# peekxc/primate

Measured on AMD Instinct MI355X. Metric: probe-matvecs/sec, higher is better.
Workload: dtype f64

## Files before the change

include/slq.h:

```cpp
#ifndef SLQ_H
#define SLQ_H

#include <stddef.h>
#include <stdint.h>

#ifdef __cplusplus
extern "C" {
#endif

#define SLQ_VERSION 100

enum {
  SLQ_OK = 0,
  SLQ_EINVAL = -1,
  SLQ_ENOMEM = -2,
  SLQ_EHIP = -3,
  SLQ_ENODEV = -4,
  SLQ_ECALLBACK = -5,
  SLQ_ENOTCONV = -6
};

enum { SLQ_F32 = 0, SLQ_F64 = 1 };

enum {
// ... 20 lines not shown
typedef struct slq_diag slq_diag;
typedef struct slq_dmat slq_dmat;
typedef struct slq_density slq_density;
typedef struct slq_sddmm slq_sddmm;

typedef int (*slq_matvec_fn)(void *user, const void *x, void *y);
typedef int (*slq_matmat_device_fn)(void *user, const void *d_X, void *d_Y, int64_t n, int ncols, void *stream);

const char *slq_last_error(void);
int slq_version(void);
int slq_device_count(int *count);
int slq_context_create(int device, void *hip_stream, slq_context **out);
int slq_context_destroy(slq_context *ctx);
int slq_context_synchronize(slq_context *ctx);
int slq_context_meminfo(slq_context *ctx, size_t *free_bytes, size_t *total_bytes);
int slq_context_device(slq_context *ctx, int *device);

int slq_csr_create(slq_context *ctx, int dtype, int64_t n, int64_t nnz, const int32_t *rowptr,
                   const int32_t *colind, const void *vals, slq_operator **out);
int slq_csr_create_device(slq_context *ctx, int dtype, int64_t n, int64_t nnz,
                          const int32_t *d_rowptr, const int32_t *d_colind, const void *d_vals,
                          slq_operator **out);
int slq_csr_gram_create(slq_context *ctx, int dtype, int64_t mrows, int64_t ncols, int64_t nnz, const int32_t *rowptr,
                        const int32_t *colind, const void *vals, slq_operator **out);
int slq_csr_affine_create(slq_context *ctx, int dtype, int64_t n, int64_t nnz_a, const int32_t *rowptr_a, const int32_t *colind_a,
                          const void *vals_a, int64_t nnz_b, const int32_t *rowptr_b, const int32_t *colind_b, const void *vals_b,
                          slq_operator **out);
int slq_operator_set_parameter(slq_operator *op, double t);
enum { SLQ_KERNEL_RBF = 0, SLQ_KERNEL_MATERN12 = 1, SLQ_KERNEL_MATERN32 = 2, SLQ_KERNEL_MATERN52 = 3 };
int slq_kernel_create(slq_context *ctx, int dtype, int64_t n, int d, const void *points, int64_t ldp, int profile,
                      const double *lengthscales, int nls, double outputscale, double noise, slq_operator **out);
int slq_kernel_create_device(slq_context *ctx, int dtype, int64_t n, int d, const void *d_points, int64_t ldp, int profile,
                             const double *lengthscales, int nls, double outputscale, double noise, slq_operator **out);
int slq_kernel_set_parameters(slq_operator *op, const double *lengthscales, int nls, double outputscale, double noise);
int slq_kernel_get_parameters(const slq_operator *op, int *d, int *profile, double *lengthscales, int nls, double *outputscale, double *noise);
int slq_debug_kernel_points(slq_operator *op, void *zt, void *nrm, void *params);
int slq_debug_kernel_schedule(int64_t n, int panel_width, int panels, int num_cus, int64_t *out, int nout);
int slq_debug_operator_device_bytes(int64_t *live);
int slq_dense_create(slq_context *ctx, int dtype, int64_t n, const void *A, int64_t lda,
                     slq_operator **out);
int slq_device_callback_create(slq_context *ctx, int dtype, int64_t n, slq_matmat_device_fn fn, void *user,
                               slq_operator **out);
int slq_callback_create(slq_context *ctx, int dtype, int64_t n, slq_matvec_fn fn, void *user,
                        slq_operator **out);
int slq_operator_destroy(slq_operator *op);
int slq_operator_shape(const slq_operator *op, int64_t *nrows, int64_t *ncols, int64_t *nnz,
                       int *dtype);
int slq_operator_matmat(slq_operator *op, const void *X, int64_t ldx, void *Y, int64_t ldy,
                        int b);

int slq_plan_create(slq_context *ctx, slq_operator *op, int nprobes, int deg, int orth,
                    int keep_basis, slq_plan **out);
int slq_plan_create_recompute(slq_context *ctx, slq_operator *op, int nprobes, int deg, int orth, slq_plan **out);
int slq_plan_basis_mode(const slq_plan *plan, int *mode, int *ring_slots, int *acc_cols);
int slq_plan_action_columns(slq_plan *plan, uint64_t *read, uint64_t *offered, int reset);
int slq_plan_destroy(slq_plan *plan);
int slq_plan_workspace_bytes(const slq_plan *plan, size_t *bytes);
int slq_plan_query_bytes(int dtype, int64_t n, int nprobes, int deg, int orth, int keep_basis,
                         size_t *bytes);
int slq_plan_query_bytes_recompute(int dtype, int64_t n, int nprobes, int deg, int orth, size_t *bytes);
typedef struct {
  int panel_width;
  int panels;
  int ring_slots;
  int sequence;
  int pipelined;
  int reordered;
  int upper_alpha;
  double far_per_row;
  int tiles;
  int fused_alpha;
} slq_plan_info;
int slq_plan_describe(const slq_plan *plan, slq_plan_info *out);

int slq_plan_set_probes(slq_plan *plan, const void *X, int64_t ldx);
int slq_plan_set_probes_device(slq_plan *plan, const void *d_X, int64_t ldx);
int slq_plan_generate_probes(slq_plan *plan, int pdf, uint64_t seed, uint64_t probe_offset);
int slq_plan_get_probes(slq_plan *plan, void *X, int64_t ldx);

int slq_plan_run(slq_plan *plan, double rtol);
int slq_plan_run_steps(slq_plan *plan, double rtol, int upto);
int slq_plan_steps_done(const slq_plan *plan, int *cur);
int slq_plan_get_tridiag(slq_plan *plan, void *alpha, void *beta, int32_t *steps);
int slq_plan_quadrature(slq_plan *plan, int fun_id, const double *fun_params, double *quad,
                        double *nodes, double *weights);
int slq_plan_quadrature_at(slq_plan *plan, int m, int rule, double endpoint, int fun_id, const double *fun_params,
                           double *quad, double *nodes, double *weights, double *stage);
int slq_plan_get_basis(slq_plan *plan, int probe, void *Q, int64_t ldq);
int slq_plan_fun_action(slq_plan *plan, int fun_id, const double *fun_params, void *Y,
                        int64_t ldy);

int slq_quadrature_batch(slq_context *ctx, int nb, int deg, const double *d, const double *e,
                         int fun_id, const double *fun_params, double *quad, double *nodes,
                         double *weights);

int slq_quadrature_radau_batch(slq_context *ctx, int nb, int m, const double *d, const double *e, const double *beta_m,
                               double endpoint, int fun_id, const double *fun_params, double *quad, double *nodes,
                               double *weights);

int slq_eigh_tridiag_batch(slq_context *ctx, int nb, int deg, const double *d, const double *e, double *w, double *Z);

int slq_dmat_create(slq_context *ctx, int64_t n, int cols, slq_dmat **out);
int slq_dmat_destroy(slq_dmat *m);
int slq_dmat_set(slq_dmat *m, int c0, int nc, const double *host, int64_t ld);
int slq_dmat_get(slq_dmat *m, int c0, int nc, double *host, int64_t ld);
int slq_dmat_ptr(slq_dmat *m, int c0, void **dptr);
int slq_dmat_generate(slq_dmat *m, int c0, int nc, int pdf, uint64_t seed, uint64_t probe_offset);
int slq_dmat_copy(slq_dmat *dst, int d0, slq_dmat *src, int s0, int nc);
int slq_dmat_copy_rows(slq_dmat *dst, int d0, int64_t dr0, slq_dmat *src, int s0, int64_t sr0, int64_t nrows, int nc);
int slq_dmat_gemm_tn(slq_dmat *A, int a0, int ma, slq_dmat *B, int b0, int mb, double *C_host);
int slq_dmat_gemm_nn(slq_dmat *OUT, int o0, slq_dmat *A, int a0, int ma, const double *C_host, int mb,
                     double alpha, double beta);
int slq_plan_fun_action_dmat(slq_plan *plan, int fun_id, const double *fun_params, slq_dmat *OUT, int o0);
int slq_plan_get_probes_dmat(slq_plan *plan, slq_dmat *OUT, int o0);

int slq_measure_stream(slq_context *ctx, int mode, size_t bytes_per_stream, int reps, double *gbps);

int slq_fttr_batch(slq_context *ctx, int nb, int n, int k, const double *theta, const double *alpha,
                   const double *beta, double *weights);

int slq_diag_create(slq_context *ctx, int64_t n, slq_diag **out);
int slq_diag_destroy(slq_diag *d);
int slq_diag_update(slq_diag *d, slq_plan *plan, int fun_id, const double *fun_params);
int slq_diag_get(slq_diag *d, double *numer, double *denom, double *running_mean, int64_t *count);

int slq_density_create(slq_context *ctx, int kind, int ngrid, const double *grid, double bw, slq_density **out);
int slq_density_update(slq_density *d, slq_plan *plan);
int slq_density_get(slq_density *d, double *mean, double *m2, double *outside, int64_t *count);
int slq_density_destroy(slq_density *d);

int slq_plan_create_chebyshev(slq_context *ctx, slq_operator *op, int nprobes, int nsteps, slq_plan **out);
int slq_plan_run_chebyshev(slq_plan *plan, double center, double halfwidth, double outside_tol);
int slq_plan_get_moments(slq_plan *plan, double *mu, int *outside);
int slq_plan_moment_sum(slq_plan *plan, int ncoef, const double *coef, double *quad, double *stage);
int slq_density_update_moments(slq_density *d, slq_plan *plan, int nweights, const double *damp);

int slq_plan_create_chebyshev_action(slq_context *ctx, slq_operator *op, int nprobes, int nsteps, slq_plan **out);
int slq_plan_chebyshev_action(slq_plan *plan, double center, double halfwidth, double outside_tol, int ncoef, const double *coef,
                              void *Y, int64_t ldy);
int slq_plan_chebyshev_action_dmat(slq_plan *plan, double center, double halfwidth, double outside_tol, int ncoef, const double *coef,
                                   slq_dmat *OUT, int o0);

int slq_sddmm_create(slq_context *ctx, int64_t n, int64_t nnz, const int32_t *rowptr, const int32_t *colind, slq_sddmm **out);
int slq_sddmm_create_device(slq_context *ctx, int64_t n, int64_t nnz, const int32_t *d_rowptr, const int32_t *d_colind, slq_sddmm **out);
int slq_sddmm_update(slq_sddmm *s, slq_dmat *W, int w0, slq_dmat *Z, int z0, int m, double alpha, double beta, int symmetric);
int slq_sddmm_get(slq_sddmm *s, double *vals, int64_t *count);
int slq_sddmm_ptr(slq_sddmm *s, void **d_vals);
int slq_sddmm_reset(slq_sddmm *s);
int slq_sddmm_destroy(slq_sddmm *s);
int slq_debug_sddmm_schedule(int64_t n, const int32_t *rowptr, int32_t *row0, int32_t *nrows, int32_t *kind, int64_t *e0, int64_t *e1,
                             int64_t cap, int64_t *nitems, int64_t *info);

typedef struct slq_kernel_grad slq_kernel_grad;
int slq_kernel_grad_create(slq_context *ctx, slq_operator *op, slq_kernel_grad **out);
int slq_kernel_grad_update(slq_kernel_grad *g, slq_dmat *Z, int z0, slq_dmat *W, int w0, int m, double alpha, double beta);
int slq_kernel_grad_get(slq_kernel_grad *g, double *vals, int nvals, int64_t *count);
int slq_kernel_grad_reset(slq_kernel_grad *g);
int slq_kernel_grad_destroy(slq_kernel_grad *g);
int slq_debug_kernel_grad_schedule(int64_t n, int m, int num_cus, int64_t *out, int nout);

typedef struct slq_kernel_cross slq_kernel_cross;
int slq_kernel_cross_create(slq_context *ctx, slq_operator *op, int64_t m, const void *points, int64_t ldp, slq_kernel_cross **out);
int slq_kernel_cross_create_device(slq_context *ctx, slq_operator *op, int64_t m, const void *d_points, int64_t ldp, slq_kernel_cross **out);
int slq_kernel_cross_matmat(slq_kernel_cross *cross, int trans, const void *X, int64_t ldx, void *Y, int64_t ldy, int b);
int slq_kernel_cross_dmat(slq_kernel_cross *cross, int trans, slq_dmat *IN, int i0, slq_dmat *OUT, int o0, int b);
int slq_kernel_cross_destroy(slq_kernel_cross *cross);
int slq_debug_kernel_cross_points(slq_kernel_cross *cross, void *zt, void *nrm);
int slq_debug_kernel_cross_schedule(int64_t nrows, int64_t nsum, int64_t b, int num_cus, int64_t *out, int nout);

typedef struct slq_kernel_feature slq_kernel_feature;
int slq_kernel_feature_create(slq_context *ctx, slq_operator *op, int64_t F2, const void *omega, int64_t ld, slq_kernel_feature **out);
int slq_kernel_feature_matmat(slq_kernel_feature *feat, slq_kernel_cross *cross, const void *W, int64_t ldw, void *Y, int64_t ldy, int b);
int slq_kernel_feature_dmat(slq_kernel_feature *feat, slq_kernel_cross *cross, slq_dmat *IN, int i0, slq_dmat *OUT, int o0, int b);
int slq_kernel_feature_destroy(slq_kernel_feature *feat);
int slq_debug_kernel_feature_frequencies(slq_kernel_feature *feat, void *omega_t);
int slq_debug_kernel_feature_schedule(int64_t nrows, int64_t F2, int64_t b, int num_cus, int is_f64, int64_t *out, int nout);
int slq_kernel_feature_rmatmat(slq_kernel_feature *feat, slq_kernel_cross *cross, const void *U, int64_t ldu, void *Z, int64_t ldz, int b);
int slq_kernel_feature_rdmat(slq_kernel_feature *feat, slq_kernel_cross *cross, slq_dmat *IN, int i0, slq_dmat *OUT, int o0, int b);
int slq_debug_kernel_feature_adjoint_schedule(int64_t F2, int64_t nrows, int64_t b, int num_cus, int is_f64, int64_t *out, int nout);

int slq_kernel_precond_create(slq_context *ctx, slq_operator *kernel_op, int rank_max, double tol, slq_operator **out);
int slq_kernel_precond_refresh(slq_operator *pre);
int slq_kernel_precond_info(const slq_operator *pre, int *rank_max, int *rank, double *logdet_p, double *residual_trace, double *t_max);
int slq_kernel_precond_get(slq_operator *pre, int32_t *pivots, double *L, int64_t ldl, double *G, double *eig);
int slq_kernel_precond_apply(slq_operator *pre, const void *X, int64_t ldx, void *Y, int64_t ldy, int b);
int slq_kernel_precond_apply_dmat(slq_operator *pre, slq_dmat *IN, int i0, slq_dmat *OUT, int o0, int b);
int slq_debug_kernel_precond_addresses(const slq_operator *pre, uint64_t *out4);
int slq_debug_kernel_precond_h(slq_operator *pre, double *H);
int slq_kernel_precond_columns(slq_operator *pre, int which, int c0, int nc, slq_dmat *OUT, int o0);
int slq_kernel_precond_trace_grad(slq_operator *pre, slq_kernel_grad *grad, double alpha, double beta);
int slq_debug_kernel_precond_timing(const slq_operator *pre, double *out2);

typedef struct slq_kernel_pointgrad slq_kernel_pointgrad;
int slq_kernel_pointgrad_create(slq_context *ctx, slq_operator *op, slq_kernel_pointgrad **out);
int slq_kernel_pointgrad_create_cross(slq_context *ctx, slq_kernel_cross *cross, slq_kernel_pointgrad **out);
int slq_kernel_pointgrad_update(slq_kernel_pointgrad *g, slq_dmat *Z_or_U, int c0, slq_dmat *W, int w0, int m, double alpha, double beta);
int slq_kernel_pointgrad_get(slq_kernel_pointgrad *g, double *vals, int64_t ld, int64_t *count);
int slq_kernel_pointgrad_reset(slq_kernel_pointgrad *g);
int slq_kernel_pointgrad_destroy(slq_kernel_pointgrad *g);
int slq_kernel_precond_trace_pointgrad(slq_operator *pre, slq_kernel_pointgrad *grad, double alpha, double beta);
int slq_debug_kernel_pointgrad_schedule(int64_t nrows, int64_t nsum, int num_cus, int64_t *out, int nout);

enum {
  SLQ_K_SPMM = 0,
  SLQ_K_AXPY_NORM,
  SLQ_K_REORTH_DOT,
  SLQ_K_REORTH_UPD,
  SLQ_K_FINALIZE,
  SLQ_K_PROBES,
  SLQ_K_QUADRATURE,
  SLQ_K_COMBINE,
  SLQ_K_COUNT
};
typedef struct {
  double ms[SLQ_K_COUNT];
  int64_t launches[SLQ_K_COUNT];
} slq_profile;
int slq_plan_profile_enable(slq_plan *plan, int enable);
int slq_plan_sweep_columns(slq_plan *plan, uint64_t *read, uint64_t *offered, int reset);
int slq_plan_window_columns(slq_plan *plan, int64_t out[5], int reset);
int slq_plan_dense_path(slq_plan *plan, int *kernel, int *ksplit);
int slq_plan_window_verify(slq_plan *plan, int *mode, double out[5]);
int slq_plan_window_census(slq_plan *plan, int32_t *out, int64_t len);
int slq_plan_window_flags(slq_plan *plan, int32_t *read, int32_t *rescue, int64_t len);
int slq_plan_profile_read(slq_plan *plan, slq_profile *out, int reset);

int slq_debug_ring_flag_status(int flag);
int slq_debug_plan_poke_ring_flag(slq_plan *plan, int value);
int slq_debug_plan_mark_stale(slq_plan *plan, int nstale);
int slq_debug_step_shape(const int *facts, int nfacts, int j, int prev_xt, int *out, int nout);
int slq_debug_cheb_step_shape(const int *facts, int nfacts, int j, int *out, int nout);
int slq_debug_cheb_action_schedule(int nsteps, int *t0, int *nc, int cap, int *npieces, int *ring_slots, int *acc_cols);
int slq_debug_csr_layout(int64_t n, int64_t nnz, const int32_t *rowptr, const int32_t *colind, int plain, int32_t *perm_out,
                         int32_t *tile_row_out, int64_t ntile_cap, int32_t *xcd_tile_out, double *info_out);
int slq_debug_plan_shape(const double *facts, int nfacts, double *out, int nout);
int slq_debug_plan_shape_of(const slq_plan *plan, double *facts_out, int nfacts, double *shape_out, int nout);

int slq_quad_batch(slq_context *ctx, slq_operator *op, const void *X, int64_t ldx, int pdf,
                   uint64_t seed, uint64_t probe_offset, int nprobes, int deg, double rtol,
                   int orth, int fun_id, const double *fun_params, double *quad_out,
                   double *nodes_out, double *weights_out);

int slq_fAv_batch(slq_context *ctx, slq_operator *op, const void *X, int64_t ldx, int nvec, int deg,
                  double rtol, int orth, int fun_id, const double *fun_params, void *Y, int64_t ldy);
int slq_fAv_batch_mode(slq_context *ctx, slq_operator *op, const void *X, int64_t ldx, int nvec, int deg, double rtol, int orth,
                       int fun_id, const double *fun_params, int basis_mode, void *Y, int64_t ldy, int *basis_used);

int slq_lanczos_f64(slq_context *ctx, slq_operator *op, double *v, int deg, double rtol, int orth,
                    double *alpha, double *beta, double *Q, size_t ncv);
int slq_lanczos_f32(slq_context *ctx, slq_operator *op, float *v, int deg, float rtol, int orth,
                    float *alpha, float *beta, float *Q, size_t ncv);

#ifdef __cplusplus
}
#endif
#endif
```

primate_amd/_capi.py:

```python

from __future__ import annotations

import ctypes as C
import os
from pathlib import Path

import numpy as np

_HERE = Path(__file__).resolve().parent
LIB_PATH = Path(os.environ["PRIMATE_AMD_LIBSLQ"]) if os.environ.get("PRIMATE_AMD_LIBSLQ") else _HERE / "_libslq.so"

SLQ_OK, SLQ_EINVAL, SLQ_ENOMEM, SLQ_EHIP, SLQ_ENODEV, SLQ_ECALLBACK, SLQ_ENOTCONV = 0, -1, -2, -3, -4, -5, -6
SLQ_F32, SLQ_F64 = 0, 1
FUN_NONE = -1
FUN_IDS = {
	"identity": 0, "abs": 1, "sqrt": 2, "log": 3, "inv": 4, "exp": 5, "smoothstep": 6, "step": 7, "numrank": 7,
	"softsign": 8,
}
PDF_IDS = {"rademacher": 0, "signs": 0, "normal": 1, "gaussian": 1, "sphere": 2}
DENSITY_KINDS = {"gaussian": 0, "lorentzian": 1, "histogram": 2, "cdf": 3, "chebyshev": 4}
KERNEL_PROFILES = {"rbf": 0, "matern12": 1, "matern32": 2, "matern52": 3}
OP_KERNEL_PRECOND = 6
KERNEL_CLASSES = ["spmm_3term", "axpy_norm", "reorth_dot", "reorth_update", "finalize", "probes", "quadrature", "fun_combine"]

# ... 74 lines not shown
	"slq_device_callback_create": (C.c_int, [_P, C.c_int, C.c_int64, _P, _P, _P]),
	"slq_dmat_generate": (C.c_int, [_P, C.c_int, C.c_int, C.c_int, C.c_uint64, C.c_uint64]),
	"slq_dmat_copy": (C.c_int, [_P, C.c_int, _P, C.c_int, C.c_int]),
	"slq_dmat_copy_rows": (C.c_int, [_P, C.c_int, C.c_int64, _P, C.c_int, C.c_int64, C.c_int64, C.c_int]),
	"slq_measure_stream": (C.c_int, [_P, C.c_int, C.c_size_t, C.c_int, C.POINTER(C.c_double)]),
	"slq_plan_set_probes_device": (C.c_int, [_P, _P, C.c_int64]),
	"slq_fttr_batch": (C.c_int, [_P, C.c_int, C.c_int, C.c_int, _P, _P, _P, _P]),
	"slq_diag_create": (C.c_int, [_P, C.c_int64, _PP]),
	"slq_diag_destroy": (C.c_int, [_P]),
	"slq_diag_update": (C.c_int, [_P, _P, C.c_int, _P]),
	"slq_diag_get": (C.c_int, [_P, _P, _P, _P, C.POINTER(C.c_int64)]),
	"slq_density_create": (C.c_int, [_P, C.c_int, C.c_int, _P, C.c_double, _PP]),
	"slq_density_destroy": (C.c_int, [_P]),
	"slq_density_update": (C.c_int, [_P, _P]),
	"slq_density_get": (C.c_int, [_P, _P, _P, _P, C.POINTER(C.c_int64)]),
	"slq_sddmm_create": (C.c_int, [_P, C.c_int64, C.c_int64, _P, _P, _PP]),
	"slq_sddmm_create_device": (C.c_int, [_P, C.c_int64, C.c_int64, _P, _P, _PP]),
	"slq_sddmm_update": (C.c_int, [_P, _P, C.c_int, _P, C.c_int, C.c_int, C.c_double, C.c_double, C.c_int]),
	"slq_sddmm_get": (C.c_int, [_P, _P, C.POINTER(C.c_int64)]),
	"slq_sddmm_ptr": (C.c_int, [_P, _PP]),
	"slq_sddmm_reset": (C.c_int, [_P]),
	"slq_sddmm_destroy": (C.c_int, [_P]),
	"slq_debug_sddmm_schedule": (C.c_int, [C.c_int64, _P, _P, _P, _P, _P, _P, C.c_int64, C.POINTER(C.c_int64), _P]),
	"slq_kernel_grad_create": (C.c_int, [_P, _P, _PP]),
	"slq_kernel_grad_update": (C.c_int, [_P, _P, C.c_int, _P, C.c_int, C.c_int, C.c_double, C.c_double]),
	"slq_kernel_grad_get": (C.c_int, [_P, _P, C.c_int, C.POINTER(C.c_int64)]),
	"slq_kernel_grad_reset": (C.c_int, [_P]),
	"slq_kernel_grad_destroy": (C.c_int, [_P]),
	"slq_debug_kernel_grad_schedule": (C.c_int, [C.c_int64, C.c_int, C.c_int, C.POINTER(C.c_int64), C.c_int]),
	"slq_kernel_cross_create": (C.c_int, [_P, _P, C.c_int64, _P, C.c_int64, _PP]),
	"slq_kernel_cross_create_device": (C.c_int, [_P, _P, C.c_int64, _P, C.c_int64, _PP]),
	"slq_kernel_cross_matmat": (C.c_int, [_P, C.c_int, _P, C.c_int64, _P, C.c_int64, C.c_int]),
	"slq_kernel_cross_dmat": (C.c_int, [_P, C.c_int, _P, C.c_int, _P, C.c_int, C.c_int]),
	"slq_kernel_cross_destroy": (C.c_int, [_P]),
	"slq_debug_kernel_cross_points": (C.c_int, [_P, _P, _P]),
	"slq_debug_kernel_cross_schedule": (C.c_int, [C.c_int64, C.c_int64, C.c_int64, C.c_int, C.POINTER(C.c_int64), C.c_int]),
	"slq_kernel_feature_create": (C.c_int, [_P, _P, C.c_int64, _P, C.c_int64, _PP]),
	"slq_kernel_feature_matmat": (C.c_int, [_P, _P, _P, C.c_int64, _P, C.c_int64, C.c_int]),
	"slq_kernel_feature_dmat": (C.c_int, [_P, _P, _P, C.c_int, _P, C.c_int, C.c_int]),
	"slq_kernel_feature_destroy": (C.c_int, [_P]),
	"slq_debug_kernel_feature_frequencies": (C.c_int, [_P, _P]),
	"slq_debug_kernel_feature_schedule": (C.c_int, [C.c_int64, C.c_int64, C.c_int64, C.c_int, C.c_int, C.POINTER(C.c_int64), C.c_int]),
	"slq_kernel_feature_rmatmat": (C.c_int, [_P, _P, _P, C.c_int64, _P, C.c_int64, C.c_int]),
	"slq_kernel_feature_rdmat": (C.c_int, [_P, _P, _P, C.c_int, _P, C.c_int, C.c_int]),
	"slq_debug_kernel_feature_adjoint_schedule": (C.c_int, [C.c_int64, C.c_int64, C.c_int64, C.c_int, C.c_int, C.POINTER(C.c_int64), C.c_int]),
	"slq_kernel_precond_create": (C.c_int, [_P, _P, C.c_int, C.c_double, _PP]),
	"slq_kernel_precond_refresh": (C.c_int, [_P]),
	"slq_kernel_precond_info": (C.c_int, [_P, C.POINTER(C.c_int), C.POINTER(C.c_int), C.POINTER(C.c_double), C.POINTER(C.c_double), C.POINTER(C.c_double)]),
	"slq_kernel_precond_get": (C.c_int, [_P, _P, _P, C.c_int64, _P, _P]),
	"slq_kernel_precond_apply": (C.c_int, [_P, _P, C.c_int64, _P, C.c_int64, C.c_int]),
	"slq_kernel_precond_apply_dmat": (C.c_int, [_P, _P, C.c_int, _P, C.c_int, C.c_int]),
	"slq_debug_kernel_precond_addresses": (C.c_int, [_P, C.POINTER(C.c_uint64)]),
	"slq_debug_kernel_precond_timing": (C.c_int, [_P, C.POINTER(C.c_double)]),
	"slq_debug_kernel_precond_h": (C.c_int, [_P, _P]),
	"slq_kernel_precond_columns": (C.c_int, [_P, C.c_int, C.c_int, C.c_int, _P, C.c_int]),
	"slq_kernel_precond_trace_grad": (C.c_int, [_P, _P, C.c_double, C.c_double]),
	"slq_kernel_pointgrad_create": (C.c_int, [_P, _P, _PP]),
	"slq_kernel_pointgrad_create_cross": (C.c_int, [_P, _P, _PP]),
	"slq_kernel_pointgrad_update": (C.c_int, [_P, _P, C.c_int, _P, C.c_int, C.c_int, C.c_double, C.c_double]),
	"slq_kernel_pointgrad_get": (C.c_int, [_P, _P, C.c_int64, C.POINTER(C.c_int64)]),
	"slq_kernel_pointgrad_reset": (C.c_int, [_P]),
	"slq_kernel_pointgrad_destroy": (C.c_int, [_P]),
	"slq_kernel_precond_trace_pointgrad": (C.c_int, [_P, _P, C.c_double, C.c_double]),
	"slq_debug_kernel_pointgrad_schedule": (C.c_int, [C.c_int64, C.c_int64, C.c_int, C.POINTER(C.c_int64), C.c_int]),
	"slq_plan_profile_enable": (C.c_int, [_P, C.c_int]),
	"slq_plan_action_columns": (C.c_int, [_P, C.POINTER(C.c_uint64), C.POINTER(C.c_uint64), C.c_int]),
	"slq_plan_sweep_columns": (C.c_int, [_P, C.POINTER(C.c_uint64), C.POINTER(C.c_uint64), C.c_int]),
	"slq_plan_window_columns": (C.c_int, [_P, C.POINTER(C.c_int64), C.c_int]),
	"slq_plan_dense_path": (C.c_int, [_P, C.POINTER(C.c_int), C.POINTER(C.c_int)]),
	"slq_plan_window_verify": (C.c_int, [_P, C.POINTER(C.c_int), C.POINTER(C.c_double)]),
	"slq_plan_window_census": (C.c_int, [_P, C.POINTER(C.c_int32), C.c_int64]),
	"slq_plan_window_flags": (C.c_int, [_P, C.POINTER(C.c_int32), C.POINTER(C.c_int32), C.c_int64]),
	"slq_plan_profile_read": (C.c_int, [_P, C.POINTER(SlqProfile), C.c_int]),
	"slq_quad_batch": (C.c_int, [_P, _P, _P, C.c_int64, C.c_int, C.c_uint64, C.c_uint64, C.c_int, C.c_int, C.c_double, C.c_int, C.c_int, _P, _P, _P, _P]),
	"slq_eigh_tridiag_batch": (C.c_int, [_P, C.c_int, C.c_int, _P, _P, _P, _P]),
	"slq_fAv_batch": (C.c_int, [_P, _P, _P, C.c_int64, C.c_int, C.c_int, C.c_double, C.c_int, C.c_int, _P, _P, C.c_int64]),
	"slq_fAv_batch_mode": (C.c_int, [_P, _P, _P, C.c_int64, C.c_int, C.c_int, C.c_double, C.c_int, C.c_int, _P, C.c_int, _P, C.c_int64, C.POINTER(C.c_int)]),
	"slq_lanczos_f64": (C.c_int, [_P, _P, _P, C.c_int, C.c_double, C.c_int, _P, _P, _P, C.c_size_t]),
	"slq_lanczos_f32": (C.c_int, [_P, _P, _P, C.c_int, C.c_float, C.c_int, _P, _P, _P, C.c_size_t]),
	"slq_debug_ring_flag_status": (C.c_int, [C.c_int]),
	"slq_debug_plan_poke_ring_flag": (C.c_int, [_P, C.c_int]),
	"slq_debug_step_shape": (C.c_int, [C.POINTER(C.c_int), C.c_int, C.c_int, C.c_int, C.POINTER(C.c_int), C.c_int]),
	"slq_debug_cheb_step_shape": (C.c_int, [C.POINTER(C.c_int), C.c_int, C.c_int, C.POINTER(C.c_int), C.c_int]),
	"slq_debug_csr_layout": (C.c_int, [C.c_int64, C.c_int64, _P, _P, C.c_int, _P, _P, C.c_int64, _P, _P]),
	"slq_debug_plan_shape": (C.c_int, [C.POINTER(C.c_double), C.c_int, C.POINTER(C.c_double), C.c_int]),
	"slq_debug_plan_shape_of": (C.c_int, [_P, C.POINTER(C.c_double), C.c_int, C.POINTER(C.c_double), C.c_int]),
	"slq_plan_create_chebyshev": (C.c_int, [_P, _P, C.c_int, C.c_int, _PP]),
	"slq_plan_run_chebyshev": (C.c_int, [_P, C.c_double, C.c_double, C.c_double]),
	"slq_plan_get_moments": (C.c_int, [_P, _P, _P]),
	"slq_plan_moment_sum": (C.c_int, [_P, C.c_int, _P, _P, _P]),
	"slq_density_update_moments": (C.c_int, [_P, _P, C.c_int, _P]),
	"slq_plan_create_chebyshev_action": (C.c_int, [_P, _P, C.c_int, C.c_int, _PP]),
	"slq_plan_chebyshev_action": (C.c_int, [_P, C.c_double, C.c_double, C.c_double, C.c_int, _P, _P, C.c_int64]),
	"slq_plan_chebyshev_action_dmat": (C.c_int, [_P, C.c_double, C.c_double, C.c_double, C.c_int, _P, _P, C.c_int]),
	"slq_debug_cheb_action_schedule": (C.c_int, [C.c_int, C.POINTER(C.c_int), C.POINTER(C.c_int), C.c_int, C.POINTER(C.c_int), C.POINTER(C.c_int), C.POINTER(C.c_int)]),
}
DEVICE_MATMAT_FN = C.CFUNCTYPE(C.c_int, C.c_void_p, C.c_void_p, C.c_void_p, C.c_int64, C.c_int, C.c_void_p)
class PlanInfo(C.Structure):

	_fields_ = [("panel_width", C.c_int), ("panels", C.c_int), ("ring_slots", C.c_int), ("sequence", C.c_int), ("pipelined", C.c_int),
				("reordered", C.c_int), ("upper_alpha", C.c_int), ("far_per_row", C.c_double), ("tiles", C.c_int), ("fused_alpha", C.c_int)]


EXPORTED_SYMBOLS = tuple(_SIGNATURES)


def _preload_hip_runtime() -> None:
	import importlib.util
	import sys

	if "torch" in sys.modules:
		return
	try:
		spec = importlib.util.find_spec("torch")
	except (ImportError, ValueError):
		spec = None
	if spec is None or not spec.origin:
		return
	cand = Path(spec.origin).parent / "lib" / "libamdhip64.so"
	if cand.exists():
		try:
			C.CDLL(str(cand), mode=getattr(os, "RTLD_NOW", 2) | getattr(os, "RTLD_GLOBAL", 0x100))
		except OSError:
			pass


def lib() -> C.CDLL:
	global _lib
	if _lib is None:
		_preload_hip_runtime()
		if not LIB_PATH.exists():
			raise ImportError(
				f"{LIB_PATH} is missing: build it with `python -c 'import __graft_entry__ as g; g.build()'` "
				"(hipcc --offload-arch=gfx950). primate_amd has no CPU fallback."
			)
		L = C.CDLL(str(LIB_PATH), mode=getattr(os, "RTLD_NOW", 2))
		for name, (res, args) in _SIGNATURES.items():
			fn = getattr(L, name)
			fn.restype, fn.argtypes = res, args
		_lib = L
	return _lib


def check(rc: int) -> int:
	if rc < 0:
		msg = lib().slq_last_error().decode(errors="replace")
		if rc == SLQ_EINVAL:
			raise ValueError(msg)
		if rc == SLQ_ENOMEM:
			raise MemoryError(msg)
		raise SlqError(rc, msg)
	return rc


def ptr(a) -> C.c_void_p:
	return None if a is None else a.ctypes.data_as(C.c_void_p)


def dtype_id(dt) -> int:
	dt = np.dtype(dt)
	if dt == np.float64:
		return SLQ_F64
	if dt == np.float32:
		return SLQ_F32
	raise AssertionError("Only 32- or 64-bit floats are supported.")
```

primate_amd/csrc/slq.hip:

```cpp
#include "../../include/slq.h"

#include <hip/hip_runtime.h>

#include <algorithm>
#include <chrono>
#include <cmath>
#include <cstdarg>
#include <cstdio>
#include <cstdlib>
#include <cstring>
#include <limits>
#include <memory>
#include <atomic>
#include <mutex>
#include <new>
#include <string>
#include <system_error>
#include <thread>
#include <type_traits>
#include <utility>
#include <vector>

#include "slq_kernels.hpp"
#include "slq_ring_api.h"
// ... 42 lines not shown
    if (_rc != SLQ_OK) return _rc; \
  } while (0)

extern "C" const char *slq_last_error(void) { return g_err; }
extern "C" int slq_version(void) { return SLQ_VERSION; }

struct slq_context {
  int device;
  hipStream_t stream;
  bool own_stream;
  int num_cus;
  int refs = 0;
  bool dead = false;
  void *pin[2] = {nullptr, nullptr};
  hipEvent_t pin_ev[2] = {nullptr, nullptr};
  bool pin_busy[2] = {false, false};
  size_t pin_bytes = 0;
};
static void ctx_retain(slq_context *ctx) { ++ctx->refs; }
static void ctx_free(slq_context *ctx) {
  hipSetDevice(ctx->device);
  for (int b = 0; b < 2; ++b) {
    if (ctx->pin[b]) hipHostFree(ctx->pin[b]);
    if (ctx->pin_ev[b]) hipEventDestroy(ctx->pin_ev[b]);
  }
  if (ctx->own_stream) hipStreamDestroy(ctx->stream);
  delete ctx;
}
static void ctx_release(slq_context *ctx) {
  if (--ctx->refs == 0 && ctx->dead) ctx_free(ctx);
}

static_assert(kF32 == SLQ_F32 && kF64 == SLQ_F64, "slq_plan_shape.hpp: the dtype codes of include/slq.h");


struct ProfEvent {
  hipEvent_t a, b;
  int kind;
};

struct slq_plan {
  slq_context *ctx;
  slq_operator *op;
  int dtype, n, nprobes, deg, orth, keep_basis;
  int LPR, PW, NP, bpad, S;
  size_t esz;
  int64_t slot_stride;
  void *ring;
  void *T;
  void *T2;
  void *stage;
  int stage_cols;
  StepState st;
  double *scal;
  double *part;
  int nblkA, nblkS, nblkU, nblkT;
  int nblkF;
  size_t alpha_pad;
  double *quad_d, *nodes_d, *weights_d;
  int *fail_d;
  int *ring_fail_d;
  int rule_src = 0;
  int rule_fail_h = 0;
  int rmax;
  bool probes_ready, ran;
  int pdf_sphere;
  bool prof;
  std::vector<ProfEvent> events;
  std::vector<ProfEvent> pool;
  slq_profile acc;
  std::vector<char> hbuf;
  int nstale;
  struct GraphEntry {
    int j0, j1;
    double rtol;
    unsigned variant;
    hipGraphExec_t exec;
    bool xt_out;
  };
  std::vector<GraphEntry> graphs;
  int cur = 0;
  double run_rtol = 0.0;
  bool prev_xt = false;
  double *at_d = nullptr;
  int *at_flags = nullptr;
  PlanSwitches sw;
  bool pipelined;
  int dense_ks;
  int ringR;
  bool ring_gen;
  bool ring_deep;
  bool gram;
  bool gram_csr;
  const TileStream *rs_full = nullptr, *rs_upper = nullptr;
  bool ring_staged;
  int part_maxblk = 0;
  bool launch_error = false;
  bool sweep_skip = true;
  unsigned long long *sweep_cols_d = nullptr;
  bool omega_on = false;
  double *om_buf = nullptr;
  int *om_flags = nullptr;
  unsigned long long *om_cnt = nullptr;
  int *om_ticket = nullptr;
  int *om_census = nullptr;
  double om_norm = 0.0;
  bool last_nostore = true;
  int basis_mode = 0;
  int acc_cols = 0;
  int v_slot = 0, y_slot = 0;
  double *acc_coef = nullptr;
  bool stash_ready = false;
  bool stash_unit = false;
  bool acc_skip = true;
  hipGraphExec_t replay_exec = nullptr;
  double replay_rtol = 0.0;
  unsigned replay_variant = 0;
  bool replay_xt_out = false;
  bool cheb = false;
  bool cheb_ran = false;
  double cheb_c = 0.0, cheb_h = 0.0;
  double *cheb_mu = nullptr;
  int *cheb_out = nullptr;
  double *cheb_coef = nullptr;
  bool cheb_action = false;
  PlanFacts facts;
  PlanShape shape;
  void *ws[kNumRegions] = {};
  uint64_t cheb_cols_read = 0, cheb_cols_offered = 0;
};

static int need_lanczos(const slq_plan *p, const char *who) {
  if (p->cheb) return fail(SLQ_EINVAL, "%s: a Chebyshev plan has no Lanczos run (slq_plan_run_chebyshev, _get_moments, _moment_sum)", who);
  return SLQ_OK;
}
static int need_chebyshev(const slq_plan *p, const char *who) {
  if (!p->cheb) return fail(SLQ_EINVAL, "%s: not a Chebyshev plan (slq_plan_create_chebyshev)", who);
  return SLQ_OK;
}

static_assert(OperatorSwitches{}.tiles == 2 && OperatorSwitches{}.tile_rows == kTileRows && OperatorSwitches{}.tile_cols == kTileCols, "slq_switches.hpp: tile defaults");
static_assert(seq::kMaxFusedR == kFusedMaxR && seq::kMaxRingR == kRingMaxR, "slq_sequence.hpp: the constants of slq_common.hpp");
static_assert(PlanSwitches{}.debug_pass == PASS_ADOTS, "slq_switches.hpp: SLQ_DEBUG_PASS");
constexpr double kOmegaC = 3.5;
constexpr double kOmegaKappa = 4.0;
static_assert(PlanSwitches{}.ring_alpha_max_x100 == (int)(100 * kTileAlphaColsPerRow), "slq_switches.hpp: SLQ_RING_ALPHA_MAX_X100");

struct UploadQueue {
  struct Job { void *dst; const void *src; size_t bytes; };
  int device;
  std::vector<std::thread> th;
  std::mutex m;
  hipError_t err = hipSuccess;
  explicit UploadQueue(int dev) : device(dev) {}
  void push(std::vector<Job> jobs) {
    auto run = [this](const std::vector<Job> &js) {
      hipError_t e = hipSetDevice(device);
      for (const Job &j : js)
        if (e == hipSuccess && j.bytes) e = hipMemcpy(j.dst, j.src, j.bytes, hipMemcpyHostToDevice);
      if (e != hipSuccess) {
        std::lock_guard<std::mutex> g(m);
        if (err == hipSuccess) err = e;
      }
    };
    try {
      th.emplace_back([run, jobs]() { run(jobs); });
    } catch (const std::system_error &) {
      run(jobs);
    }
  }
  hipError_t wait() {
    for (auto &t : th)
      if (t.joinable()) t.join();
    th.clear();
    return err;
  }
  ~UploadQueue() { wait(); }
};

extern "C" int slq_device_count(int *count) {
  if (!count) return fail(SLQ_EINVAL, "count is NULL");
  int c = 0;
  hipError_t e = hipGetDeviceCount(&c);
  if (e != hipSuccess) {
    *count = 0;
    return fail(SLQ_ENODEV, "hipGetDeviceCount: %s", hipGetErrorString(e));
  }
  *count = c;
  return SLQ_OK;
}

extern "C" int slq_context_create(int device, void *hip_stream, slq_context **out) {
  if (!out) return fail(SLQ_EINVAL, "out is NULL");
  *out = nullptr;
  int count = 0;
  if (hipGetDeviceCount(&count) != hipSuccess || count <= 0)
    return fail(SLQ_ENODEV, "no HIP device visible: the SLQ engine has no CPU fallback");
  if (device < 0) HIP_TRY(hipGetDevice(&device));
  if (device >= count) return fail(SLQ_EINVAL, "device %d out of range (%d visible)", device, count);
  HIP_TRY(hipSetDevice(device));
  hipDeviceProp_t prop;
  HIP_TRY(hipGetDeviceProperties(&prop, device));
  if (strncmp(prop.gcnArchName, "gfx950", 6) != 0)
    return fail(SLQ_ENODEV, "device %d is %s; libslq is built for gfx950 only", device,
                prop.gcnArchName);
  slq_context *ctx = new (std::nothrow) slq_context();
  if (!ctx) return fail(SLQ_ENOMEM, "host allocation failed");
  ctx->device = device;
  ctx->num_cus = prop.multiProcessorCount;
  if (hip_stream) {
    ctx->stream = (hipStream_t)hip_stream;
    ctx->own_stream = false;
  } else {
    hipError_t e = hipStreamCreateWithFlags(&ctx->stream, hipStreamNonBlocking);
    if (e != hipSuccess) {
      delete ctx;
      return fail(SLQ_EHIP, "hipStreamCreate: %s", hipGetErrorString(e));
    }
    ctx->own_stream = true;
  }
  *out = ctx;
  return SLQ_OK;
}
// ... 1072 lines not shown
      if (op->dtype == SLQ_F64) k_norm_inf<double><<<grid, 256, 0, st>>>((int)op->n, op->csr.rp(), op->csr.vals.as<const double>(), d);
      else k_norm_inf<float><<<grid, 256, 0, st>>>((int)op->n, op->csr.rp(), op->csr.vals.as<const float>(), d);
      e = hipGetLastError();
    }
    if (e == hipSuccess) e = hipMemcpyAsync(&h, d, 8, hipMemcpyDeviceToHost, st);
    if (e == hipSuccess) e = hipStreamSynchronize(st);
    hipFree(d);
    if (e != hipSuccess) return fail(SLQ_EHIP, "||A||_inf: %s", hipGetErrorString(e));
    double v;
    memcpy(&v, &h, 8);
    op->norm_inf = v;
  }
  *out = op->norm_inf;
  return SLQ_OK;
}

static PlanFacts plan_facts_of(const slq_operator *op, int nprobes, int deg, int orth, PlanKind kind) {
  PlanFacts f;
  const TileStream &upper_stream = op->streams[0].upper;
  f.kind = op->kind, f.dtype = op->dtype, f.n = op->n, f.nnz = op->nnz, f.nnz_u = op->upper.nnz, f.upper = (bool)op->upper;
  f.mrows = op->kind == OP_KERNEL_PRECOND ? op->pre->rpad : op->mrows, f.lda = op->lda;
  f.has_tiles = (bool)op->tiles.tile_ptr, f.tiles_ringed = op->tiles_ringed, f.tiles_max_cols = op->tiles.max_cols;
  f.upper_per_row = op->upper_per_row, f.upper_stream = (bool)upper_stream, f.upper_padded = upper_stream.padded;
  f.far_per_row = op->far_per_row, f.affine = (bool)op->vals_b;
  std::copy(op->tiles.xcd_tile, op->tiles.xcd_tile + 9, f.xcd_tile);
  std::copy(upper_stream.xcd_tile, upper_stream.xcd_tile + 9, f.xcd_tile_u);
  {
    std::unique_lock<std::mutex> guard;
    if (op->tiles_ringed) guard = std::unique_lock<std::mutex>(op->merged_lock);
    for (int i = 0; i < 2; ++i) {
      const TileStreamPair &m = op->streams[1 + i];
      f.merged[i].available = (bool)m.full, f.merged[i].upper = (bool)m.upper, f.merged[i].u_padded = m.upper.padded;
      std::copy(m.full.xcd_tile, m.full.xcd_tile + 9, f.merged[i].xcd_tile);
    }
  }
  f.num_cus = op->ctx->num_cus;
  f.nprobes = nprobes, f.deg = deg, f.orth = orth, f.plan = kind;
  return f;
}

static int check_query(int dtype, int64_t n, int nprobes, size_t *bytes) {
  if (!bytes) return fail(SLQ_EINVAL, "bytes is NULL");
  SLQ_TRY(check_dtype(dtype));
  if (n <= 0 || nprobes <= 0) return fail(SLQ_EINVAL, "n and nprobes must be positive");
  return SLQ_OK;
}
static size_t query_ring_bytes(int dtype, int64_t n, int nprobes, int deg, int orth, PlanKind kind) {
  PlanFacts f;
  f.dtype = dtype, f.n = n, f.nprobes = nprobes, f.deg = deg, f.orth = orth, f.plan = kind;
  return plan_shape(f, read_plan_switches()).ws[WS_RING].bytes;
}

extern "C" int slq_plan_query_bytes(int dtype, int64_t n, int nprobes, int deg, int orth,
                                    int keep_basis, size_t *bytes) {
  SLQ_TRY(check_query(dtype, n, nprobes, bytes));
  SLQ_TRY(normalise_params(n, &deg, &orth));
  *bytes = query_ring_bytes(dtype, n, nprobes, deg, orth, keep_basis ? PlanKind::KeepBasis : PlanKind::Ring);
  return SLQ_OK;
}

extern "C" int slq_plan_query_bytes_recompute(int dtype, int64_t n, int nprobes, int deg, int orth, size_t *bytes) {
  SLQ_TRY(check_query(dtype, n, nprobes, bytes));
  if (deg < 1) return fail(SLQ_EINVAL, "Number of steps must be positive!");
  if (deg > n) deg = (int)n;
  if (orth < 0 || orth > deg) orth = deg;
  *bytes = query_ring_bytes(dtype, n, nprobes, deg, orth, PlanKind::Recompute);
  return SLQ_OK;
}

static int plan_bytes_on_mode(const slq_operator *op, int nprobes, int deg, int orth, int mode, size_t *bytes) {
  SLQ_TRY(check_query(op->dtype, op->n, nprobes, bytes));
  SLQ_TRY(normalise_params(op->n, &deg, &orth));
  const PlanFacts f = plan_facts_of(op, nprobes, deg, orth, mode == 2 ? PlanKind::Recompute : (mode == 1 ? PlanKind::KeepBasis : PlanKind::Ring));
  *bytes = plan_estimate_bytes(plan_shape(f, read_plan_switches()), f);
  return SLQ_OK;
}
static int plan_bytes_on(const slq_operator *op, int nprobes, int deg, int orth, int keep_basis, size_t *bytes) {
  return plan_bytes_on_mode(op, nprobes, deg, orth, keep_basis ? 1 : 0, bytes);
}

extern "C" int slq_plan_destroy(slq_plan *p) {
  if (!p) return SLQ_OK;
  hipSetDevice(p->ctx->device);
  hipStreamSynchronize(p->ctx->stream);
  for (auto &ev : p->events) { hipEventDestroy(ev.a); hipEventDestroy(ev.b); }
  for (auto &ev : p->pool) { hipEventDestroy(ev.a); hipEventDestroy(ev.b); }
  for (auto &g : p->graphs) hipGraphExecDestroy(g.exec);
  if (p->replay_exec) hipGraphExecDestroy(p->replay_exec);
  if (p->at_d) hipFree(p->at_d);
  if (p->at_flags) hipFree(p->at_flags);
  if (p->om_ticket) hipFree(p->om_ticket);
  if (p->stage) hipFree(p->stage);
  for (void *q : p->ws)
    if (q) hipFree(q);
  ctx_release(p->ctx);
  delete p;
  return SLQ_OK;
}

static int set_kernel_attributes(slq_plan *p);
static seq::SequenceFacts sequence_facts(const slq_plan *p);

static int plan_create_mode(slq_context *ctx, slq_operator *op, int nprobes, int deg, int orth, PlanKind kind, slq_plan **out);

extern "C" int slq_plan_create(slq_context *ctx, slq_operator *op, int nprobes, int deg, int orth,
                               int keep_basis, slq_plan **out) {
  return plan_create_mode(ctx, op, nprobes, deg, orth, keep_basis != 0 ? PlanKind::KeepBasis : PlanKind::Ring, out);
}

extern "C" int slq_plan_create_recompute(slq_context *ctx, slq_operator *op, int nprobes, int deg, int orth, slq_plan **out) {
  return plan_create_mode(ctx, op, nprobes, deg, orth, PlanKind::Recompute, out);
}

extern "C" int slq_plan_basis_mode(const slq_plan *p, int *mode, int *ring_slots_out, int *acc_cols) {
  if (!p) return fail(SLQ_EINVAL, "plan is NULL");
  if (mode) *mode = p->basis_mode;
  if (ring_slots_out) *ring_slots_out = p->S;
  if (acc_cols) *acc_cols = p->acc_cols;
  return SLQ_OK;
}

static void plan_adopt_shape(slq_plan *p) {
  const PlanFacts &f = p->facts;
  const PlanShape &sh = p->shape;
  const slq_operator *op = p->op;
  p->cheb = is_cheb(f.plan);
  p->cheb_action = f.plan == PlanKind::ChebyshevAction;
  p->basis_mode = basis_mode_of(f.plan);
  p->keep_basis = f.plan == PlanKind::KeepBasis;
  p->dtype = op->dtype, p->n = (int)op->n, p->nprobes = f.nprobes, p->deg = f.deg, p->orth = f.orth;
  p->esz = esize(op->dtype);
  p->LPR = sh.LPR, p->PW = sh.PW, p->NP = sh.NP, p->bpad = sh.bpad, p->S = sh.S;
  p->acc_cols = sh.acc_cols, p->v_slot = sh.v_slot, p->y_slot = sh.y_slot;
  p->slot_stride = sh.slot_stride, p->rmax = sh.rmax;
  p->pipelined = sh.pipelined != 0;
  p->nblkA = sh.nblkA, p->nblkS = sh.nblkS, p->nblkU = sh.nblkU, p->nblkF = sh.nblkF, p->nblkT = sh.nblkT;
  p->alpha_pad = sh.alpha_pad, p->part_maxblk = sh.part_maxblk, p->dense_ks = sh.dense_ks;
  p->ringR = sh.ringR, p->ring_staged = sh.ring_staged != 0;
  p->rs_full = p->rs_upper = nullptr;
  if (sh.stream != STREAM_NONE) {
    const TileStreamPair &m = op->streams[sh.stream - STREAM_BASE];
    p->rs_full = &m.full;
    if (m.upper && (sh.stream != STREAM_BASE || sh.rs_upper)) p->rs_upper = &m.upper;
  }
  p->ring_gen = sh.seq.ring_gen, p->ring_deep = sh.seq.ring_deep, p->gram = sh.seq.gram, p->gram_csr = sh.seq.gram_csr, p->last_nostore = sh.seq.last_nostore;
  p->omega_on = sh.omega_on != 0;
  p->acc_skip = p->sw.acc_skip != 0;
  p->sweep_skip = p->sw.sweep_skip != 0;
  p->nstale = 0;
}

static int plan_materialise(slq_plan *p) {
  const PlanShape &sh = p->shape;
  hipError_t e = hipSuccess;
  for (const Region &r : sh.ws) {
    if (e != hipSuccess || !r.bytes) continue;
    e = hipMalloc(&p->ws[r.id], r.bytes);
    if (e == hipSuccess && r.zeroed == 1) e = hipMemset(p->ws[r.id], 0, r.bytes);
  }
  if (e != hipSuccess)
    return fail(e == hipErrorOutOfMemory ? SLQ_ENOMEM : SLQ_EHIP, "plan workspace (%zu bytes of Lanczos panels): %s", sh.ws[WS_RING].bytes, hipGetErrorString(e));
  p->ring = p->ws[WS_RING], p->scal = (double *)p->ws[WS_SCAL], p->part = (double *)p->ws[WS_PART], p->acc_coef = (double *)p->ws[WS_ACC_COEF];
  p->sweep_cols_d = (unsigned long long *)p->ws[WS_SWEEP_COLS];
  p->om_buf = (double *)p->ws[WS_OM_BUF], p->om_flags = (int *)p->ws[WS_OM_FLAGS], p->om_cnt = (unsigned long long *)p->ws[WS_OM_CNT];
  p->om_census = (int *)p->ws[WS_OM_CENSUS];
  p->quad_d = (double *)p->ws[WS_QUAD];
// ... 113 lines not shown
  };
  raise((const void *)k_reorth_update<F, L>);
  for_each_csr_pass<F, L>(raise);
  if constexpr (L == 64) {
    for_each_tiled_pass<F, false>(raise);
    for_each_tiled_pass<F, true>(raise);
  }
  return e;
}
static int set_kernel_attributes(slq_plan *p) {
  hipError_t ae = hipSuccess;
  DISPATCH(p->dtype, p->LPR, (ae = raise_lds_limits<F, L>()));
  HIP_TRY(ae);
  if (p->ring_gen || p->ring_deep) {
    hipError_t re = hipSuccess;
    const bool d = p->dtype == SLQ_F64;
    switch (p->LPR) {
      case 64: re = d ? slq_ring_prepare_f64_l64() : slq_ring_prepare_f32_l64(); break;
      case 32: re = d ? slq_ring_prepare_f64_l32() : slq_ring_prepare_f32_l32(); break;
      default: re = d ? slq_ring_prepare_f64_l16() : slq_ring_prepare_f32_l16(); break;
    }
    HIP_TRY(re);
  }
  HIP_TRY(hipFuncSetAttribute((const void *)k_dense_mfma_3term<16>, hipFuncAttributeMaxDynamicSharedMemorySize, 160 * 1024));
  HIP_TRY(hipFuncSetAttribute((const void *)k_dense_mfma_3term<32>, hipFuncAttributeMaxDynamicSharedMemorySize, 160 * 1024));
  HIP_TRY(hipFuncSetAttribute((const void *)k_dense_mfma_3term<64>, hipFuncAttributeMaxDynamicSharedMemorySize, 160 * 1024));

  return SLQ_OK;
}

static bool plan_tiled(const slq_plan *p) { return p->ringR > 0; }

static int ring_flag_status(int flag) {
  if (flag) return fail(SLQ_EHIP, "the ring-fed tile pass gave up waiting on a tile (SLQ_TILES=2): results are invalid");
  return SLQ_OK;
}
static int check_ring_flag(slq_plan *p) {
  int flag = 0;
  HIP_TRY(hipMemcpyAsync(&flag, p->ring_fail_d, sizeof(int), hipMemcpyDeviceToHost, p->ctx->stream));
  HIP_TRY(hipStreamSynchronize(p->ctx->stream));
  return ring_flag_status(flag);
}
extern "C" int slq_debug_ring_flag_status(int flag) { return ring_flag_status(flag); }
extern "C" int slq_debug_plan_poke_ring_flag(slq_plan *p, int value) {
  if (!p) return fail(SLQ_EINVAL, "plan is NULL");
  HIP_TRY(hipSetDevice(p->ctx->device));
  HIP_TRY(hipMemcpyAsync(p->ring_fail_d, &value, sizeof(int), hipMemcpyHostToDevice, p->ctx->stream));
  HIP_TRY(hipStreamSynchronize(p->ctx->stream));
  return SLQ_OK;
}

extern "C" int slq_plan_describe(const slq_plan *p, slq_plan_info *out) {
  if (!p || !out) return fail(SLQ_EINVAL, "plan/out is NULL");
  memset(out, 0, sizeof(*out));
  out->panel_width = p->PW;
  out->panels = p->NP;
  out->ring_slots = p->S;
  out->sequence = seq::plan_sequence_of(sequence_facts(p));
  out->pipelined = p->pipelined ? 1 : 0;
  out->reordered = p->op->perm_d ? 1 : 0;
  out->upper_alpha = p->op->upper ? 1 : 0;
  out->far_per_row = p->op->far_per_row;
  out->tiles = plan_tiled(p) ? (p->op->tiles_ringed ? 2 : 1) : 0;
  return SLQ_OK;
}

extern "C" int slq_plan_sweep_columns(slq_plan *p, uint64_t *read, uint64_t *offered, int reset) {
  if (!p) return fail(SLQ_EINVAL, "plan is NULL");
  HIP_TRY(hipSetDevice(p->ctx->device));
  unsigned long long h[2] = {0, 0};
  HIP_TRY(hipMemcpyAsync(h, p->sweep_cols_d, sizeof(h), hipMemcpyDeviceToHost, p->ctx->stream));
  if (reset) HIP_TRY(hipMemsetAsync(p->sweep_cols_d, 0, sizeof(h), p->ctx->stream));
  HIP_TRY(hipStreamSynchronize(p->ctx->stream));
  if (read) *read = h[0];
  if (offered) *offered = h[1];
  return SLQ_OK;
}

extern "C" int slq_plan_window_columns(slq_plan *p, int64_t out[5], int reset) {
  if (!p || !out) return fail(SLQ_EINVAL, "plan/out is NULL");
  for (int k = 0; k < 5; ++k) out[k] = 0;
  if (!p->omega_on) return SLQ_OK;
  HIP_TRY(hipSetDevice(p->ctx->device));
  unsigned long long h[8] = {0, 0, 0, 0, 0, 0, 0, 0};
  HIP_TRY(hipMemcpyAsync(h, p->om_cnt, sizeof(h), hipMemcpyDeviceToHost, p->ctx->stream));
  if (reset) HIP_TRY(hipMemsetAsync(p->om_cnt, 0, sizeof(h), p->ctx->stream));
  HIP_TRY(hipStreamSynchronize(p->ctx->stream));
  for (int k = 0; k < 5; ++k) out[k] = (int64_t)h[k];
  return SLQ_OK;
}

extern "C" int slq_plan_window_flags(slq_plan *p, int32_t *read, int32_t *rescue, int64_t len) {
  if (!p || !read || !rescue) return fail(SLQ_EINVAL, "plan/read/rescue is NULL");
  const int64_t words = (int64_t)(p->deg + 1) * p->NP;
  if (len != words) return fail(SLQ_EINVAL, "flag buffers: %lld words expected", (long long)words);
  memset(read, 0, (size_t)words * sizeof(int32_t));
  memset(rescue, 0, (size_t)words * sizeof(int32_t));
  if (!p->omega_on) return SLQ_OK;
  HIP_TRY(hipSetDevice(p->ctx->device));
  HIP_TRY(hipMemcpyAsync(read, p->om_flags, (size_t)words * sizeof(int), hipMemcpyDeviceToHost, p->ctx->stream));
  HIP_TRY(hipMemcpyAsync(rescue, p->om_flags + words, (size_t)words * sizeof(int), hipMemcpyDeviceToHost, p->ctx->stream));
  HIP_TRY(hipStreamSynchronize(p->ctx->stream));
  return SLQ_OK;
}

extern "C" int slq_plan_window_census(slq_plan *p, int32_t *out, int64_t len) {
  if (!p || !out) return fail(SLQ_EINVAL, "plan/out is NULL");
  const int64_t words = (int64_t)(p->deg + 1) * (kFusedMaxR + 1) * p->NP;
  if (!p->om_census) return fail(SLQ_EINVAL, "the plan keeps no census (ring-fed Gram sequence created under SLQ_OMEGA=2)");
  if (len != words) return fail(SLQ_EINVAL, "census buffer: %lld words expected", (long long)words);
  HIP_TRY(hipSetDevice(p->ctx->device));
  HIP_TRY(hipMemcpyAsync(out, p->om_census, (size_t)words * sizeof(int), hipMemcpyDeviceToHost, p->ctx->stream));
  HIP_TRY(hipStreamSynchronize(p->ctx->stream));
  return SLQ_OK;
}

extern "C" int slq_plan_window_verify(slq_plan *p, int *mode, double out[5]) {
  if (!p) return fail(SLQ_EINVAL, "plan is NULL");
  if (mode) *mode = p->omega_on ? p->sw.omega : 0;
  if (!out) return SLQ_OK;
  out[0] = 0.0, out[1] = std::numeric_limits<double>::infinity(), out[2] = kOmegaC, out[3] = kOmegaKappa, out[4] = p->om_norm;
  if (!p->omega_on) return SLQ_OK;
  HIP_TRY(hipSetDevice(p->ctx->device));
  unsigned long long h[8];
  HIP_TRY(hipMemcpyAsync(h, p->om_cnt, sizeof(h), hipMemcpyDeviceToHost, p->ctx->stream));
  HIP_TRY(hipStreamSynchronize(p->ctx->stream));
  double inv;
  memcpy(&out[0], &h[kOmCntInnov], 8);
  memcpy(&inv, &h[kOmCntMargin], 8);
  if (inv > 0.0) out[1] = 1.0 / inv;
  return SLQ_OK;
}

extern "C" int slq_plan_action_columns(slq_plan *p, uint64_t *read, uint64_t *offered, int reset) {
  if (!p) return fail(SLQ_EINVAL, "plan is NULL");
  HIP_TRY(hipSetDevice(p->ctx->device));
  if (p->cheb_action) {
    if (read) *read = p->cheb_cols_read;
    if (offered) *offered = p->cheb_cols_offered;
    if (reset) p->cheb_cols_read = p->cheb_cols_offered = 0;
    HIP_TRY(hipStreamSynchronize(p->ctx->stream));
    return SLQ_OK;
  }
  unsigned long long h[2] = {0, 0};
  HIP_TRY(hipMemcpyAsync(h, p->sweep_cols_d + 2, sizeof(h), hipMemcpyDeviceToHost, p->ctx->stream));
  if (reset) HIP_TRY(hipMemsetAsync(p->sweep_cols_d + 2, 0, sizeof(h), p->ctx->stream));
  HIP_TRY(hipStreamSynchronize(p->ctx->stream));
  if (read) *read = h[0];
  if (offered) *offered = h[1];
  return SLQ_OK;
}

extern "C" int slq_plan_workspace_bytes(const slq_plan *plan, size_t *bytes) {
  if (!plan || !bytes) return fail(SLQ_EINVAL, "plan/bytes is NULL");
  *bytes = plan_workspace_bytes(plan->shape);
  return SLQ_OK;
}

static int ensure_stage(slq_plan *p, int cols) {
  if (p->stage && p->stage_cols >= cols) return SLQ_OK;
  if (p->stage) { hipFree(p->stage); p->stage = nullptr; }
  HIP_TRY(hipMalloc(&p->stage, (size_t)cols * p->n * p->esz));
  p->stage_cols = cols;
  return SLQ_OK;
}

static int stage_chunk_cols(const slq_plan *p) {
  const size_t per_col = (size_t)p->n * p->esz;
  size_t c = std::max<size_t>(1, ((size_t)256 << 20) / per_col);
  return (int)std::min<size_t>(c, (size_t)p->bpad);
}

static int init_from_probes(slq_plan *p, int sphere, bool unit_entries = false, bool restoring = false) {
  hipStream_t st = p->ctx->stream;
  if (p->basis_mode == 2 && !restoring) {
    HIP_TRY(hipMemcpyAsync(slot_ptr(p, p->v_slot), slot_ptr(p, 0), (size_t)p->slot_stride * p->esz, hipMemcpyDeviceToDevice, st));
    p->stash_unit = unit_entries;
    p->stash_ready = true;
  }
  dim3 g(p->nblkS, p->NP);
  if (!unit_entries)
    PROFILED(p, SLQ_K_AXPY_NORM,
             DISPATCH(p->dtype, p->LPR,
                      (k_axpy_norm<F, L, 1><<<g, dim3(kBlock), 0, st>>>(p->n,
                                          (F *)slot_ptr(p, 0), (const F *)nullptr,
                                          (const double *)nullptr, p->part, p->bpad))));
  PROFILED(p, SLQ_K_FINALIZE,
           hipLaunchKernelGGL(k_fin_init, dim3((p->bpad + 63) / 64), dim3(kFinThreads), 0, st, p->st, p->part,
                              unit_entries ? 0 : p->nblkS, sphere, (double)p->n));
  HIP_TRY(hipGetLastError());
  p->probes_ready = true;
  p->ran = false;
  p->cur = 0;
  return SLQ_OK;
}

static bool ensure_pinned(slq_context *ctx, size_t bytes) {
  if (ctx->pin_bytes >= bytes && ctx->pin[0] && ctx->pin[1]) return true;
  for (int b = 0; b < 2; ++b) {
    if (ctx->pin[b]) hipHostFree(ctx->pin[b]);
    ctx->pin[b] = nullptr;
    ctx->pin_busy[b] = false;
  }
  ctx->pin_bytes = 0;
  for (int b = 0; b < 2; ++b) {
    if (hipHostMalloc(&ctx->pin[b], bytes, hipHostMallocDefault) != hipSuccess) { (void)hipGetLastError(); return false; }
    if (!ctx->pin_ev[b] && hipEventCreateWithFlags(&ctx->pin_ev[b], hipEventDisableTiming) != hipSuccess) return false;
  }
  ctx->pin_bytes = bytes;
  return true;
}

extern "C" int slq_plan_set_probes(slq_plan *p, const void *X, int64_t ldx) {
  if (!p || !X) return fail(SLQ_EINVAL, "plan/X is NULL");
  if (ldx < p->n) return fail(SLQ_EINVAL, "ldx (%lld) < n (%d)", (long long)ldx, p->n);
  HIP_TRY(hipSetDevice(p->ctx->device));
  hipStream_t st = p->ctx->stream;
  slq_context *ctx = p->ctx;
  const size_t col_bytes = (size_t)p->n * p->esz;
  const bool pinned = p->sw.pinned_upload != 0 && (size_t)p->nprobes * col_bytes >= ((size_t)4 << 20);
  int cc = stage_chunk_cols(p);
  if (pinned) cc = (int)std::max<size_t>(1, std::min<size_t>((size_t)cc, ((size_t)32 << 20) / col_bytes));
  const bool use_pin = pinned && ensure_pinned(ctx, (size_t)cc * col_bytes);
  if (!use_pin) cc = stage_chunk_cols(p);
  SLQ_TRY(ensure_stage(p, cc));
  if (p->nprobes < p->bpad)
    HIP_TRY(hipMemsetAsync(slot_ptr(p, 0), 0, (size_t)p->slot_stride * p->esz, st));
  int buf = 0;
  for (int c0 = 0; c0 < p->nprobes; c0 += cc) {
    const int nc = std::min(cc, p->nprobes - c0);
    const char *src = (const char *)X + (size_t)c0 * (size_t)ldx * p->esz;
    if (use_pin) {
      if (ctx->pin_busy[buf]) HIP_TRY(hipEventSynchronize(ctx->pin_ev[buf]));
      char *dst = (char *)ctx->pin[buf];
      if (!parallel_pieces(host_threads(), p->n, [&](int, int64_t r0, int64_t r1) {
            for (int c = 0; c < nc; ++c)
              memcpy(dst + (size_t)c * col_bytes + (size_t)r0 * p->esz, src + (size_t)c * (size_t)ldx * p->esz + (size_t)r0 * p->esz, (size_t)(r1 - r0) * p->esz);
          }))
        return fail(SLQ_ENOMEM, "host worker failed while staging the probes");
      HIP_TRY(hipMemcpyAsync(p->stage, dst, (size_t)nc * col_bytes, hipMemcpyHostToDevice, st));
      HIP_TRY(hipEventRecord(ctx->pin_ev[buf], st));
      ctx->pin_busy[buf] = true;
      buf ^= 1;
    } else {
      HIP_TRY(hipMemcpy2DAsync(p->stage, col_bytes, src, (size_t)ldx * p->esz, col_bytes, (size_t)nc, hipMemcpyHostToDevice, st));
    }
    dim3 g((p->n + 63) / 64, (nc + 63) / 64);
    PROFILED(p, SLQ_K_PROBES, {
      if (p->dtype == SLQ_F64)
        hipLaunchKernelGGL(k_cols_to_panel<double>, g, dim3(256), 0, st, p->n, (const double *)p->stage, c0, nc, (double *)slot_ptr(p, 0), p->PW, p->op->perm_d.as<int32_t>());
      else
        hipLaunchKernelGGL(k_cols_to_panel<float>, g, dim3(256), 0, st, p->n, (const float *)p->stage, c0, nc, (float *)slot_ptr(p, 0), p->PW, p->op->perm_d.as<int32_t>());
    });
    if (!use_pin) HIP_TRY(hipStreamSynchronize(st));
  }
  p->pdf_sphere = 0;
  return init_from_probes(p, 0);
}

extern "C" int slq_plan_generate_probes(slq_plan *p, int pdf, uint64_t seed, uint64_t probe_offset) {
  if (!p) return fail(SLQ_EINVAL, "plan is NULL");
  if (pdf < 0 || pdf > 2) return fail(SLQ_EINVAL, "Invalid distribution id %d supplied.", pdf);
  HIP_TRY(hipSetDevice(p->ctx->device));
  hipStream_t st = p->ctx->stream;
  const int RPW = 64 / p->LPR;
  const int items = (p->n + (pdf == 0 ? 127 : 1)) / (pdf == 0 ? 128 : 2);
  const int gx = std::max(1, std::min(p->ctx->num_cus * 8, (items + 4 * RPW - 1) / (4 * RPW)));
  dim3 g(gx, p->NP);
  PROFILED(p, SLQ_K_PROBES,
           DISPATCH(p->dtype, p->LPR,
                    (k_gen_probes<F, L><<<g, dim3(256), 0, st>>>(p->n,
                                        (F *)slot_ptr(p, 0), pdf, seed, probe_offset, p->nprobes, p->op->inv_perm_d.as<int32_t>()))));
  p->pdf_sphere = (pdf == SLQ_PDF_SPHERE);
  return init_from_probes(p, p->pdf_sphere, pdf == 0 && p->sw.known_norm != 0);
}

static int panel_to_host(slq_plan *p, int slot, int c0, int nc, void *X, int64_t ldx,
                         const double *d_scale) {
  hipStream_t st = p->ctx->stream;
  const int cc = stage_chunk_cols(p);
  SLQ_TRY(ensure_stage(p, cc));
  for (int o = 0; o < nc; o += cc) {
    const int m = std::min(cc, nc - o);
    dim3 g((p->n + 63) / 64, (m + 63) / 64);
    if (p->dtype == SLQ_F64)
      hipLaunchKernelGGL(k_panel_to_cols<double>, g, dim3(256), 0, st, p->n, (const double *)slot_ptr(p, slot), c0 + o, m, (double *)p->stage, p->PW, d_scale, p->op->perm_d.as<int32_t>());
    else
      hipLaunchKernelGGL(k_panel_to_cols<float>, g, dim3(256), 0, st, p->n, (const float *)slot_ptr(p, slot), c0 + o, m, (float *)p->stage, p->PW, d_scale, p->op->perm_d.as<int32_t>());
    HIP_TRY(hipMemcpy2DAsync((char *)X + (size_t)o * (size_t)ldx * p->esz, (size_t)ldx * p->esz, p->stage,
                             (size_t)p->n * p->esz, (size_t)p->n * p->esz, (size_t)m, hipMemcpyDeviceToHost, st));
    HIP_TRY(hipStreamSynchronize(st));
  }
  return SLQ_OK;
}

extern "C" int slq_plan_get_probes(slq_plan *p, void *X, int64_t ldx) {
  if (!p || !X) return fail(SLQ_EINVAL, "plan/X is NULL");
  if (!p->probes_ready) return fail(SLQ_EINVAL, "no probes set, or they were consumed by a run");
  if (ldx < p->n) return fail(SLQ_EINVAL, "ldx < n");
  HIP_TRY(hipSetDevice(p->ctx->device));
  return panel_to_host(p, 0, 0, p->nprobes, X, ldx, nullptr);
}


static int dense_kernel_of(const slq_plan *p) { return p->shape.dense_class; }

extern "C" int slq_plan_dense_path(slq_plan *p, int *kernel, int *ksplit) {
  if (!p) return fail(SLQ_EINVAL, "plan is NULL");
  if (kernel) *kernel = dense_kernel_of(p);
  if (ksplit) *ksplit = p->dense_ks;
  return SLQ_OK;
}

static seq::SequenceFacts sequence_facts(const slq_plan *p) {
  seq::SequenceFacts f = p->shape.seq;
  f.nstale = p->nstale;
  return f;
}

extern "C" int slq_debug_csr_layout(int64_t n, int64_t nnz, const int32_t *rowptr, const int32_t *colind, int plain, int32_t *perm_out,
                                    int32_t *tile_row_out, int64_t ntile_cap, int32_t *xcd_tile_out, double *info_out) {
  if (!perm_out || !tile_row_out || !xcd_tile_out || !info_out) return fail(SLQ_EINVAL, "slq_debug_csr_layout: an output is NULL");
  return create_guarded(nullptr, [&]() {
    SLQ_TRY(validate_csr(n, nnz, rowptr, colind));
    const OperatorSwitches osw = read_operator_switches();
    const CsrView A{n, nnz, rowptr, colind};
    const OperatorLayout L = decide_layout(A, osw, layout_prefilter(A, osw, plain != 0), nullptr);
    const int64_t ntiles = L.have_tiles ? (int64_t)L.tile_row.size() - 1 : 0;
    if ((int64_t)L.tile_row.size() > ntile_cap) return fail(SLQ_EINVAL, "slq_debug_csr_layout: %zu tile boundaries, room for %lld", L.tile_row.size(), (long long)ntile_cap);
    std::copy(L.perm.begin(), L.perm.end(), perm_out);
    std::copy(L.tile_row.begin(), L.tile_row.end(), tile_row_out);
    std::copy(L.xcd_tile, L.xcd_tile + 9, xcd_tile_out);
    info_out[0] = L.have_tiles ? 1.0 : 0.0, info_out[1] = (double)ntiles, info_out[2] = L.perm.empty() ? 0.0 : 1.0, info_out[3] = L.rms_dist;
    return (int)SLQ_OK;
  });
}

extern "C" int slq_debug_step_shape(const int *facts, int nfacts, int j, int prev_xt, int *out, int nout) {
  if (!facts || !out || nfacts != seq::kNumFacts || nout != seq::kNumShape + 1) return fail(SLQ_EINVAL, "slq_debug_step_shape: %d facts in, %d values out", seq::kNumFacts, seq::kNumShape + 1);
  const seq::SequenceFacts f = seq::facts_from_array(facts);
  seq::shape_to_array(seq::step_shape(f, j, prev_xt != 0), out);
  out[seq::kNumShape] = seq::plan_sequence_of(f);
  return SLQ_OK;
}

static int launch_dense_mfma(slq_plan *p, const void *Wc, const void *Wp, void *Wn, int first, int plain, int *nblk_out) {
// ... 298 lines not shown
  a.coefB = p->st.coefB;
  a.gamma = p->st.gamma;
  a.part = p->part;
  a.bpad = p->bpad;
  a.xt = xt;
  a.fail = p->ring_fail_d;
  a.wread = wread;
  a.dbg = pass == p->sw.debug_pass ? debug_times_buffer() : nullptr;
  const bool d = p->dtype == SLQ_F64;
  int rc_l = -1;
  switch (p->LPR) {
    case 64: rc_l = d ? slq_ring_launch_f64_l64(a) : slq_ring_launch_f32_l64(a); break;
    case 32: rc_l = d ? slq_ring_launch_f64_l32(a) : slq_ring_launch_f32_l32(a); break;
    case 16: rc_l = d ? slq_ring_launch_f64_l16(a) : slq_ring_launch_f32_l16(a); break;
    default: break;
  }
  if (rc_l != 0) return fail(SLQ_EINVAL, "no ring-fed kernel for pass %d with %d ring columns on %d lanes per row", pass, rc, p->LPR);
  return SLQ_OK;
}

struct RunFrame {
  slq_plan *p;
  hipStream_t st;
  bool nt;
  double eps, residual_tol, orth_tol;
  dim3 gA, gS, gU, gF, gAf, gT;
  size_t lds0;
  OmegaState om_off;
  int blocks(int blk) const {
    switch (blk) {
      case seq::BLK_A: return p->nblkA;
      case seq::BLK_U: return p->nblkU;
      case seq::BLK_T: return p->nblkT;
      case seq::BLK_F: return p->nblkF;
      default: return p->nblkS;
    }
  }
  size_t lds_alpha(const seq::StepShape &s) const { return lds0 + (s.alpha_tiled ? 0 : p->alpha_pad); }
  size_t lds_fused(const seq::StepShape &s) const {
    return lds0 + (s.tiled ? 0 : (size_t)(p->sw.fused_pad >= 0 ? p->sw.fused_pad : (p->pipelined ? 98304 : 65536)));
  }
  size_t lds_tile(const seq::StepShape &s) const {
    return lds0 + (s.tiled ? (size_t)(SLQ_TILE_DB ? 2 : 1) * p->op->tiles.max_cols * p->PW * p->esz : 0);
  }
};

#define CSR_PASS_RC(PASS, LP, RCT)                                                                   \
  do {                                                                                               \
    if (tl && s.gen)                                                                                 \
      SLQ_TRY(launch_ring_gen(p, PASS, RCT, c.gT, c.st, j, xt, upper));                              \
    else if (tl)                                                                                     \
      DISPATCH(p->dtype, p->LPR, (launch_tile_pass<F, L, PASS, LP, RCT>(p, c.gT, c.lds_tile(s), c.st, j, xt, upper))); \
    else                                                                                             \
      DISPATCH(p->dtype, p->LPR,                                                                     \
               (launch_csr_pass<F, L, PASS, LP, RCT>(s.pipe_on != 0, (PASS == PASS_ALPHA ? c.gAf : c.gU), lds, c.st, p->n, \
                   (half ? op->upper : op->csr).rp(), (half ? op->upper : op->csr).ci(),               \
                   (half ? op->upper : op->csr).vals.as<const F>(), (F *)p->ring, p->slot_stride, p->S, j, \
                   p->st.coefA, p->st.coefB, p->st.gamma, p->part, p->bpad, xt)));                   \
  } while (0)
#define CSR_PASS(PASS, LP)                                                                           \
  switch (PASS == PASS_ALPHA ? 0 : rc) {                                                             \
    case 0: CSR_PASS_RC(PASS, LP, ((PASS == PASS_DOTS || PASS == PASS_ADOTS) ? 1 : 0)); break;       \
    case 1: CSR_PASS_RC(PASS, LP, (PASS == PASS_ALPHA ? 0 : 1)); break;                              \
    case 2: CSR_PASS_RC(PASS, LP, (PASS == PASS_ALPHA ? 0 : 2)); break;                              \
    case 3: CSR_PASS_RC(PASS, LP, (PASS == PASS_ALPHA ? 0 : 3)); break;                              \
    case 4: CSR_PASS_RC(PASS, LP, (PASS == PASS_ALPHA ? 0 : 4)); break;                              \
    case 5: CSR_PASS_RC(PASS, LP, (PASS == PASS_ALPHA ? 0 : 5)); break;                              \
    case 6: CSR_PASS_RC(PASS, LP, (PASS == PASS_ALPHA ? 0 : 6)); break;                              \
    case 7: CSR_PASS_RC(PASS, LP, (PASS == PASS_ALPHA ? 0 : 7)); break;                              \
    default: CSR_PASS_RC(PASS, LP, (PASS == PASS_ALPHA ? 0 : 8)); break;                             \
  }
template <int PASS> static int launch_fused_pass(const RunFrame &c, const seq::StepShape &s, int j, int rc, size_t lds, int xt) {
  slq_plan *p = c.p;
  const slq_operator *op = p->op;
  const bool tl = PASS == PASS_ALPHA ? s.alpha_tiled : s.tiled;
  const bool half = PASS == PASS_ALPHA && s.half;
  const bool upper = PASS == PASS_ALPHA && s.alpha_upper;
  if (c.nt) CSR_PASS(PASS, 1) else CSR_PASS(PASS, 0)
  return SLQ_OK;
}
#undef CSR_PASS
#undef CSR_PASS_RC

static int launch_gram_ring(const RunFrame &c, const seq::StepShape &s, int j) {
  slq_plan *p = c.p;
  hipStream_t st = c.st;
  const int bp = p->bpad, r = s.r, S = p->S;
  PROFILED(p, SLQ_K_SPMM, SLQ_TRY(launch_fused_pass<PASS_ALPHA>(c, s, j, 0, c.lds_alpha(s), s.xt_alpha)));
  OmegaState om = c.om_off;
  om.census = p->om_census, om.PW = p->PW, om.NP = p->NP;
  if (s.omega) {
    om.mode = p->sw.omega;
    om.est_prev = s.est_prev;
    om.force = (j == p->sw.omega_trip ? 1 : 0) | (j == p->sw.omega_rescue ? 2 : 0);
    om.D = p->om_buf, om.rho = p->om_buf + bp, om.g3 = p->om_buf + 2 * (size_t)bp, om.Dm = p->om_buf + 3 * (size_t)bp;
    om.read = p->om_flags, om.rescue = p->om_flags + (size_t)(p->deg + 1) * p->NP;
    om.cnt = p->om_cnt;
    om.eps_norm = c.eps * p->om_norm;
    om.theta = kOmegaC * om.eps_norm;
    om.tol_k = c.orth_tol / kOmegaKappa;
  }
  PROFILED(p, SLQ_K_FINALIZE,
           hipLaunchKernelGGL(k_fin_gram, dim3((bp + 63) / 64, r), dim3(kFinThreads), 0, st, p->st, p->part, c.blocks(s.blk_alpha), j, r, c.orth_tol, om));
  if (om.mode == 1 && om.est_prev) {
    double *part_r = p->part + (size_t)p->part_maxblk * bp;
    PROFILED(p, SLQ_K_FINALIZE,
             DISPATCH(p->dtype, p->LPR, (k_omega_rescue_dot<F, L><<<c.gS, dim3(kBlock), 0, st>>>(p->n, (const F *)p->ring, p->slot_stride, S, j, r, part_r, p->om_ticket, p->st, c.orth_tol, om))));
  }
  PROFILED(p, SLQ_K_REORTH_UPD, SLQ_TRY(launch_ring_gen(p, PASS_UPDATEG, r, c.gT, st, j, s.xt_update, false, om.mode == 1 ? om.read + (size_t)j * p->NP : nullptr)));
  PROFILED(p, SLQ_K_FINALIZE,
           hipLaunchKernelGGL(k_fin_beta_gram, dim3((bp + 63) / 64, r + 1), dim3(kFinThreads), 0, st, p->st, p->part, c.blocks(s.blk_beta), j, r, c.residual_tol, om));
  return SLQ_OK;
}

static int launch_gram_csr(const RunFrame &c, const seq::StepShape &s, int j) {
  slq_plan *p = c.p;
  hipStream_t st = c.st;
  const int bp = p->bpad, r = s.r;
  PROFILED(p, SLQ_K_SPMM, SLQ_TRY(launch_fused_pass<PASS_ALPHA>(c, s, j, 0, c.lds_alpha(s), s.xt_alpha)));
  PROFILED(p, SLQ_K_FINALIZE,
           hipLaunchKernelGGL(k_fin_gram, dim3((bp + 63) / 64, r), dim3(kFinThreads), 0, st, p->st, p->part, c.blocks(s.blk_alpha), j, r, c.orth_tol, c.om_off));
  PROFILED(p, SLQ_K_REORTH_UPD, DISPATCH(p->dtype, p->LPR, (launch_csr_updateg<F, L>(p, r, s.pipe_on != 0, c.gU, c.lds_fused(s), st, j, s.xt_update))));
  PROFILED(p, SLQ_K_FINALIZE,
           hipLaunchKernelGGL(k_fin_beta_gram, dim3((bp + 63) / 64, r + 1), dim3(kFinThreads), 0, st, p->st, p->part, c.blocks(s.blk_beta), j, r, c.residual_tol, c.om_off));
  return SLQ_OK;
}

static int launch_merged(const RunFrame &c, const seq::StepShape &s, int j) {
  slq_plan *p = c.p;
  const int bp = p->bpad, r = s.r;
  PROFILED(p, SLQ_K_REORTH_DOT, SLQ_TRY(launch_fused_pass<PASS_ADOTS>(c, s, j, r, c.lds_fused(s), s.xt_dots)));
  PROFILED(p, SLQ_K_FINALIZE,
           hipLaunchKernelGGL(k_fin_adots, dim3((bp + 63) / 64, r), dim3(kFinThreads), 0, c.st, p->st, p->part, c.blocks(s.blk_dots), j, r, c.orth_tol));
  PROFILED(p, SLQ_K_REORTH_UPD, SLQ_TRY(launch_fused_pass<PASS_UPDATE>(c, s, j, r, c.lds_fused(s), s.xt_update)));
  return SLQ_OK;
}

static int launch_separate(const RunFrame &c, const seq::StepShape &s, int j) {
  slq_plan *p = c.p;
  const int bp = p->bpad, r = s.r;
  PROFILED(p, SLQ_K_SPMM, SLQ_TRY(launch_fused_pass<PASS_ALPHA>(c, s, j, 0, c.lds_alpha(s), s.xt_alpha)));
  PROFILED(p, SLQ_K_FINALIZE,
           hipLaunchKernelGGL(k_fin_alpha, c.gF, dim3(kFinThreads), 0, c.st, p->st, p->part, c.blocks(s.blk_alpha), j, s.xt_alpha & 1));
  if (r > 0) {
    PROFILED(p, SLQ_K_REORTH_DOT, SLQ_TRY(launch_fused_pass<PASS_DOTS>(c, s, j, r, c.lds_fused(s), s.xt_dots)));
    PROFILED(p, SLQ_K_FINALIZE,
             hipLaunchKernelGGL(k_fin_gamma, dim3((bp + 63) / 64, r), dim3(kFinThreads), 0, c.st, p->st, p->part, c.blocks(s.blk_dots), j, 0, c.orth_tol));
  }
  PROFILED(p, (r == 0 ? SLQ_K_AXPY_NORM : SLQ_K_REORTH_UPD), SLQ_TRY(launch_fused_pass<PASS_UPDATE>(c, s, j, r, c.lds_fused(s), s.xt_update)));
  return SLQ_OK;
}

static int launch_sweep_product(const RunFrame &c, const seq::StepShape &s, int j, bool cheb = false) {
  slq_plan *p = c.p;
  const slq_operator *op = p->op;
  hipStream_t st = c.st;
  const int bp = p->bpad, S = p->S;
  const int sc_ = j % S, sp_ = (j + S - 1) % S, sn_ = (j + 1) % S;
  const int first = (j == 0);
  int nblk = c.blocks(s.blk_alpha);
  switch (s.product) {
    case seq::PRODUCT_RING:
      PROFILED(p, SLQ_K_SPMM, {
        if (s.gen) SLQ_TRY(launch_ring_gen(p, PASS_SPMM, 0, c.gT, st, j, 0, false));
        else if (c.nt) DISPATCH(p->dtype, p->LPR, (launch_tile_pass<F, L, PASS_SPMM, 1, 0>(p, c.gT, 0, st, j, 0, false)));
        else DISPATCH(p->dtype, p->LPR, (launch_tile_pass<F, L, PASS_SPMM, 0, 0>(p, c.gT, 0, st, j, 0, false)));
      });
      break;
    case seq::PRODUCT_CSR: {
      const size_t spmm_pad = (size_t)p->sw.spmm_pad;
#define SPMM_LAUNCH(LP, SP)                                                                          \
  DISPATCH(p->dtype, p->LPR,                                                                         \
           (k_spmm_3term<F, L, LP, SP><<<c.gA, dim3(kBlock), spmm_pad, st>>>(                        \
               p->n, op->csr.rp(), op->csr.ci(), op->csr.vals.as<const F>(), (const F *)slot_ptr(p, sc_),       \
               (const F *)slot_ptr(p, sp_), (F *)slot_ptr(p, sn_), p->st.coefA, p->part, bp, first)))
      PROFILED(p, SLQ_K_SPMM, {
        switch (c.nt ? 11 : 0) {
          case 1: SPMM_LAUNCH(0, 1); break;
          case 2: SPMM_LAUNCH(0, 2); break;
          case 10: SPMM_LAUNCH(1, 0); break;
          case 11: SPMM_LAUNCH(1, 1); break;
          case 12: SPMM_LAUNCH(1, 2); break;
          default: SPMM_LAUNCH(0, 0); break;
        }
      });
#undef SPMM_LAUNCH
      break;
    }
    case seq::PRODUCT_DENSE:
      PROFILED(p, SLQ_K_SPMM, SLQ_TRY(launch_dense_mfma(p, slot_ptr(p, sc_), slot_ptr(p, sp_), slot_ptr(p, sn_), first, 0, &nblk)));
      break;
    default:
      SLQ_TRY(apply_operator_unfused(p, sc_));
      if (cheb)
        PROFILED(p, SLQ_K_AXPY_NORM,
                 DISPATCH(p->dtype, p->LPR,
                          (k_cheb_3term<F, L><<<c.gS, dim3(kBlock), 0, st>>>(p->n, (const F *)p->T, (const F *)slot_ptr(p, sc_), (const F *)slot_ptr(p, sp_),
                                                                             (F *)slot_ptr(p, sn_), p->st.coefA, p->st.coefB, p->part, bp, first))));
      else
      PROFILED(p, SLQ_K_AXPY_NORM,
               DISPATCH(p->dtype, p->LPR,
                        (k_3term<F, L><<<c.gS, dim3(kBlock), 0, st>>>(p->n, (const F *)p->T, (const F *)slot_ptr(p, sc_), (const F *)slot_ptr(p, sp_),
                                                                      (F *)slot_ptr(p, sn_), p->st.coefA, p->part, bp, first))));
      break;
  }
  if (cheb) return SLQ_OK;
  PROFILED(p, SLQ_K_FINALIZE, hipLaunchKernelGGL(k_fin_alpha, c.gF, dim3(kFinThreads), 0, st, p->st, p->part, nblk, j, 0));
  return SLQ_OK;
}

static int launch_sweeps(const RunFrame &c, const seq::StepShape &s, int j) {
  slq_plan *p = c.p;
  hipStream_t st = c.st;
  const int bp = p->bpad, S = p->S, r = s.r;
  SLQ_TRY(launch_sweep_product(c, s, j));
  if (s.seq == seq::SEQ_SWEEPS_PLAIN) {
    PROFILED(p, SLQ_K_AXPY_NORM,
             DISPATCH(p->dtype, p->LPR,
                      (k_axpy_norm<F, L, 0><<<c.gS, dim3(kBlock), 0, st>>>(p->n, (F *)slot_ptr(p, (j + 1) % S), (const F *)slot_ptr(p, j % S), p->st.coefB, p->part, bp))));
  } else if (s.seq == seq::SEQ_SWEEPS_MGS) {
    for (int i = 0; i < r; ++i) {
      PROFILED(p, SLQ_K_REORTH_DOT,
               DISPATCH(p->dtype, p->LPR,
                        (k_reorth_dot<F, L><<<c.gS, dim3(kBlock), 0, st>>>(p->n, (F *)p->ring, p->slot_stride, S, j, i, 1, (int)(i == 0), p->st.coefB, p->part, bp))));
      PROFILED(p, SLQ_K_FINALIZE,
               hipLaunchKernelGGL(k_fin_gamma, dim3((bp + 63) / 64, 1), dim3(kFinThreads), 0, st, p->st, p->part, p->nblkS, j, i, c.orth_tol));
      SLQ_TRY(launch_reorth_update_range(p, j, i, i + 1));
    }
  } else {
    for (int i0 = 0; i0 < r; i0 += kReorthChunk) {
      const int rc = std::min(kReorthChunk, r - i0);
      PROFILED(p, SLQ_K_REORTH_DOT, DISPATCH(p->dtype, p->LPR, (launch_reorth_dot<F, L>(p, c.gS, st, j, i0, rc))));
      PROFILED(p, SLQ_K_FINALIZE,
               hipLaunchKernelGGL(k_fin_gamma, dim3((bp + 63) / 64, rc), dim3(kFinThreads), 0, st, p->st, p->part, p->nblkS, j, i0, c.orth_tol));
    }
    SLQ_TRY(launch_reorth_update(p, j, r, 0, p->sw.defer_axpy));
  }
  return SLQ_OK;
}

static RunFrame run_frame(slq_plan *p, double rtol) {
  const int bp = p->bpad;
  RunFrame c;
  c.p = p, c.st = p->ctx->stream, c.nt = p->sw.nt != 0;
  c.eps = p->dtype == SLQ_F64 ? std::numeric_limits<double>::epsilon() : (double)std::numeric_limits<float>::epsilon();
  c.residual_tol = std::sqrt((double)p->n) * rtol;
  c.orth_tol = 2.0 * c.eps * std::sqrt((double)p->n);
  c.gA = dim3(p->nblkA, p->NP), c.gS = dim3(p->nblkS, p->NP), c.gU = dim3(p->nblkU, p->NP), c.gF = dim3((bp + 63) / 64);
  c.gAf = dim3(p->nblkF, p->NP), c.gT = dim3(p->nblkT, p->NP);
  c.lds0 = sizeof(double) * kWaves * 64 * (p->dtype == SLQ_F64 ? 2 : 4);
  memset(&c.om_off, 0, sizeof(c.om_off));
  return c;
}

static int enqueue_run(slq_plan *p, double rtol, int j0, int j1) {
  hipStream_t st = p->ctx->stream;
  const int bp = p->bpad, deg = p->deg;
  const RunFrame c = run_frame(p, rtol);
  if (j0 == 0) {
    HIP_TRY(hipMemsetAsync(p->st.alpha, 0, (size_t)(deg + 1) * bp * 8, st));
    HIP_TRY(hipMemsetAsync(p->st.nu + bp, 0, (size_t)deg * bp * 8, st));
    HIP_TRY(hipMemsetAsync(p->st.gram, 0, (size_t)2 * (kFusedMaxR + 1) * bp * 8, st));
    if (p->omega_on) {
      HIP_TRY(hipMemsetAsync(p->om_buf, 0, (size_t)4 * bp * 8, st));
      HIP_TRY(hipMemsetAsync(p->om_flags, 0, (size_t)2 * (deg + 1) * p->NP * sizeof(int), st));
    }
  }
  if (j0 == 0 && p->om_census) HIP_TRY(hipMemsetAsync(p->om_census, 0, (size_t)(deg + 1) * (kFusedMaxR + 1) * p->NP * sizeof(int), st));
  const seq::SequenceFacts facts = sequence_facts(p);
  bool prev_xt = j0 > 0 && p->prev_xt;
  for (int j = j0; j < j1; ++j) {
    const seq::StepShape s = seq::step_shape(facts, j, prev_xt);
    prev_xt = s.prev_xt != 0;
    switch (s.seq) {
      case seq::SEQ_GRAM_RING: SLQ_TRY(launch_gram_ring(c, s, j)); continue;
      case seq::SEQ_GRAM_CSR: SLQ_TRY(launch_gram_csr(c, s, j)); continue;
      case seq::SEQ_MERGED:
      case seq::SEQ_STORED_U: SLQ_TRY(launch_merged(c, s, j)); break;
      case seq::SEQ_SEPARATE: SLQ_TRY(launch_separate(c, s, j)); break;
      default: SLQ_TRY(launch_sweeps(c, s, j)); break;
    }
    PROFILED(p, SLQ_K_FINALIZE,
             hipLaunchKernelGGL(k_fin_beta, c.gF, dim3(kFinThreads), 0, st, p->st, p->part, c.blocks(s.blk_beta), j, c.residual_tol, prev_xt ? 1 : 0));
  }
  p->prev_xt = prev_xt;
  HIP_TRY(hipGetLastError());
  if (p->launch_error) {
    p->launch_error = false;
    return fail(SLQ_EINVAL, "internal: a pass of the launch sequence had no kernel for this plan's tiles");
  }
  return SLQ_OK;
}

extern "C" int slq_plan_create_chebyshev(slq_context *ctx, slq_operator *op, int nprobes, int nsteps, slq_plan **out) {
  return plan_create_mode(ctx, op, nprobes, nsteps, 0, PlanKind::Chebyshev, out);
}

extern "C" int slq_debug_cheb_step_shape(const int *facts, int nfacts, int j, int *out, int nout) {
  if (!facts || !out || nfacts != seq::kNumFacts || nout != seq::kNumChebShape) return fail(SLQ_EINVAL, "slq_debug_cheb_step_shape: %d facts in, %d values out", seq::kNumFacts, seq::kNumChebShape);
  seq::cheb_shape_to_array(seq::cheb_step_shape(seq::facts_from_array(facts), j), out);
  return SLQ_OK;
}

extern "C" int slq_debug_cheb_action_schedule(int nsteps, int *t0, int *nc, int cap, int *npieces, int *ring_slots_out, int *acc_cols) {
  if (nsteps < 1 || nsteps > kMaxChebSteps || cap < 0 || !npieces)
    return fail(SLQ_EINVAL, "slq_debug_cheb_action_schedule: nsteps = %d must lie in [1, %d], cap >= 0, npieces not NULL", nsteps, kMaxChebSteps);
  *npieces = seq::cheb_action_schedule(nsteps, kChebAccCols, t0, nc, nullptr, cap);
  if (ring_slots_out) *ring_slots_out = seq::cheb_action_ring_slots(nsteps, kChebAccCols);
  if (acc_cols) *acc_cols = kChebAccCols;
  return SLQ_OK;
}

static int launch_cheb_accumulate(slq_plan *p, int t0, int nc, const double *coef_h) {
  hipStream_t st = p->ctx->stream;
  const dim3 gS(p->nblkS, p->NP);
  unsigned live = 0;
  for (int i = 0; i < nc; ++i)
    if (!p->acc_skip || coef_h[t0 + i] != 0.0) live |= 1u << i;
  p->cheb_cols_read += (uint64_t)__builtin_popcount(live);
  p->cheb_cols_offered += (uint64_t)nc;
  PROFILED(p, SLQ_K_COMBINE,
           DISPATCH(p->dtype, p->LPR,
                    (k_cheb_accumulate<F, L><<<gS, dim3(kBlock), 0, st>>>(p->n, (const F *)p->ring, p->slot_stride, p->S, t0, nc, live,
                                                                        (const double *)p->cheb_coef, (F *)slot_ptr(p, p->y_slot), t0 == 0 ? 1 : 0))));
  return SLQ_OK;
}

static int cheb_run(slq_plan *p, const char *who, double center, double halfwidth, double outside_tol, const double *action_coef) {
  if (!p->probes_ready) return fail(SLQ_EINVAL, "%s: set or generate probes first", who);
  SLQ_TRY(precond_check_fresh(p->op, who));
  if (!std::isfinite(center) || !std::isfinite(halfwidth) || !(halfwidth > 0.0))
    return fail(SLQ_EINVAL, "%s: center = %g, halfwidth = %g (finite, halfwidth > 0)", who, center, halfwidth);
  HIP_TRY(hipSetDevice(p->ctx->device));
  hipStream_t st = p->ctx->stream;
  const int bp = p->bpad, S = p->S;
  const RunFrame c = run_frame(p, 0.0);
  const double tol = outside_tol > 0.0 ? outside_tol : kChebOutsideTol;
  const double inv_h = 1.0 / halfwidth, c_over_h = center / halfwidth;
  const int sphere = p->pdf_sphere ? 1 : 0;
  const seq::SequenceFacts facts = sequence_facts(p);
  PROFILED(p, SLQ_K_AXPY_NORM,
           DISPATCH(p->dtype, p->LPR,
                    (k_axpy_norm<F, L, 1><<<c.gS, dim3(kBlock), 0, st>>>(p->n, (F *)slot_ptr(p, 0), (const F *)nullptr, (const double *)nullptr, p->part, bp))));
  PROFILED(p, SLQ_K_FINALIZE,
           hipLaunchKernelGGL(k_fin_cheb, c.gF, dim3(kFinThreads), 0, st, p->st, p->part, p->nblkS, -1, p->cheb_mu, p->cheb_out, inv_h, c_over_h, tol, sphere));
  int c0 = 0;
  for (int j = 0; j < p->deg; ++j) {
    const seq::ChebStepShape s = seq::cheb_step_shape(facts, j);
    seq::StepShape l;
    l.tiled = s.tiled, l.gen = s.gen, l.pipe_on = s.pipe_on, l.product = s.product, l.blk_alpha = s.blk_product;
    int nblk = c.blocks(s.blk);
    if (!s.sweeps) {
      PROFILED(p, SLQ_K_AXPY_NORM, SLQ_TRY(launch_fused_pass<PASS_UPDATE>(c, l, j, 0, c.lds_fused(l), s.xt_update)));
    } else {
      SLQ_TRY(launch_sweep_product(c, l, j, true));
      if (s.product != seq::PRODUCT_UNFUSED)
        PROFILED(p, SLQ_K_AXPY_NORM,
                 DISPATCH(p->dtype, p->LPR,
                          (k_cheb_axpy<F, L><<<c.gS, dim3(kBlock), 0, st>>>(p->n, (F *)slot_ptr(p, (j + 1) % S), (const F *)slot_ptr(p, j % S), p->st.coefB, p->part, bp))));
      nblk = p->nblkS;
    }
    PROFILED(p, SLQ_K_FINALIZE,
             hipLaunchKernelGGL(k_fin_cheb, c.gF, dim3(kFinThreads), 0, st, p->st, p->part, nblk, j, p->cheb_mu, p->cheb_out, inv_h, c_over_h, tol, sphere));
    if (action_coef) {
      const int m = seq::cheb_action_piece_after(p->deg, p->acc_cols, j, c0);
      if (m) SLQ_TRY(launch_cheb_accumulate(p, c0, m, action_coef));
// ... 70 lines not shown
extern "C" int slq_plan_get_moments(slq_plan *p, double *mu, int *outside) {
  if (!p) return fail(SLQ_EINVAL, "plan is NULL");
  SLQ_TRY(need_chebyshev(p, "slq_plan_get_moments"));
  if (!p->cheb_ran) return fail(SLQ_EINVAL, "slq_plan_get_moments: no completed run");
  HIP_TRY(hipSetDevice(p->ctx->device));
  hipStream_t st = p->ctx->stream;
  const int bp = p->bpad, P = p->nprobes;
  const size_t K = (size_t)2 * p->deg + 1;
  std::vector<double> h;
  if (mu) {
    h.resize(K * bp);
    HIP_TRY(hipMemcpyAsync(h.data(), p->cheb_mu, h.size() * 8, hipMemcpyDeviceToHost, st));
  }
  std::vector<int> flags;
  int raised = 0;
  SLQ_TRY(cheb_flags(p, flags, &raised));
  if (mu)
    for (int i = 0; i < P; ++i)
      for (size_t k = 0; k < K; ++k) mu[(size_t)i * K + k] = h[k * bp + i];
  if (outside) memcpy(outside, flags.data(), (size_t)P * sizeof(int));
  return SLQ_OK;
}

extern "C" int slq_plan_moment_sum(slq_plan *p, int ncoef, const double *coef, double *quad, double *stage) {
  if (!p || !coef) return fail(SLQ_EINVAL, "plan/coef is NULL");
  SLQ_TRY(need_chebyshev(p, "slq_plan_moment_sum"));
  if (!p->cheb_ran) return fail(SLQ_EINVAL, "slq_plan_moment_sum: no completed run");
  const int K = 2 * p->deg + 1, P = p->nprobes;
  if (ncoef < 1 || ncoef > K) return fail(SLQ_EINVAL, "slq_plan_moment_sum: ncoef = %d must lie in [1, %d] (2 nsteps + 1 moments)", ncoef, K);
  HIP_TRY(hipSetDevice(p->ctx->device));
  hipStream_t st = p->ctx->stream;
  std::vector<int> flags;
  int raised = 0;
  SLQ_TRY(cheb_flags(p, flags, &raised));
  if (raised) return cheb_outside_error(p, "slq_plan_moment_sum", raised);
  double *stage_d = p->cheb_coef + K;
  HIP_TRY(hipMemcpyAsync(p->cheb_coef, coef, (size_t)ncoef * 8, hipMemcpyHostToDevice, st));
  PROFILED(p, SLQ_K_QUADRATURE,
           hipLaunchKernelGGL(k_moment_sum, dim3((P + 63) / 64), dim3(64), 0, st, P, p->bpad, ncoef, (const double *)p->cheb_coef, (const double *)p->cheb_mu, p->quad_d));
  if (stage)
    hipLaunchKernelGGL(k_stage_reduce, dim3(1), dim3(kStageThreads), 0, st, P, (const double *)p->quad_d, (const double *)nullptr, stage_d);
  HIP_TRY(hipGetLastError());
  if (quad) HIP_TRY(hipMemcpyAsync(quad, p->quad_d, (size_t)P * 8, hipMemcpyDeviceToHost, st));
  if (stage) HIP_TRY(hipMemcpyAsync(stage, stage_d, 4 * 8, hipMemcpyDeviceToHost, st));
  HIP_TRY(hipStreamSynchronize(st));
  return SLQ_OK;
}

static int run_range(slq_plan *p, double rtol, int j0, int j1);

extern "C" int slq_plan_run(slq_plan *p, double rtol) {
  if (!p) return fail(SLQ_EINVAL, "plan is NULL");
  SLQ_TRY(need_lanczos(p, "slq_plan_run"));
  if (!p->probes_ready) return fail(SLQ_EINVAL, "slq_plan_run: set or generate probes first");
  return run_range(p, rtol, 0, p->deg);
}

extern "C" int slq_plan_run_steps(slq_plan *p, double rtol, int upto) {
  if (!p) return fail(SLQ_EINVAL, "plan is NULL");
  SLQ_TRY(need_lanczos(p, "slq_plan_run_steps"));
  if (p->nstale > 0) return fail(SLQ_EINVAL, "slq_plan_run_steps: a plan with stale ring columns is not resumable");
  if (p->basis_mode == 2) return fail(SLQ_EINVAL, "slq_plan_run_steps: a recompute plan runs in one piece (a staged two-pass run is not supported)");
  const bool fresh = p->probes_ready;
  if (!fresh && !(p->ran && p->cur > 0)) return fail(SLQ_EINVAL, "slq_plan_run_steps: set or generate probes first");
  const int cur = fresh ? 0 : p->cur;
  if (upto <= cur || upto > p->deg) return fail(SLQ_EINVAL, "slq_plan_run_steps: upto = %d must lie in (%d, %d] (steps done, the plan's deg)", upto, cur, p->deg);
  if (!fresh && rtol != p->run_rtol) return fail(SLQ_EINVAL, "slq_plan_run_steps: rtol = %g differs from the %g this run began with", rtol, p->run_rtol);
  return run_range(p, rtol, cur, upto);
}

extern "C" int slq_plan_steps_done(const slq_plan *p, int *cur) {
  if (!p || !cur) return fail(SLQ_EINVAL, "plan/cur is NULL");
  *cur = p->probes_ready ? 0 : (p->ran ? p->cur : 0);
  return SLQ_OK;
}

constexpr size_t kGraphCacheMax = 16;

static int run_range(slq_plan *p, double rtol, int j0, int j1) {
  SLQ_TRY(precond_check_fresh(p->op, "slq_plan_run"));
  HIP_TRY(hipSetDevice(p->ctx->device));
  hipStream_t st = p->ctx->stream;
  const bool graph_ok = p->sw.graph && !p->prof && p->op->kind != OP_CALLBACK && p->op->kind != OP_DEVICE_CALLBACK;
  if (!graph_ok) {
    SLQ_TRY(enqueue_run(p, rtol, j0, j1));
  } else {
    const unsigned variant = (unsigned)p->nstale;
    size_t gi = 0;
    for (; gi < p->graphs.size(); ++gi) {
      const auto &g = p->graphs[gi];
      if (g.j0 == j0 && g.j1 == j1 && g.rtol == rtol && g.variant == variant) break;
    }
    if (gi == p->graphs.size()) {
      for (size_t k = 0; k < p->graphs.size();) {
        if (p->graphs[k].j0 == j0 && p->graphs[k].j1 == j1) {
          HIP_TRY(hipGraphExecDestroy(p->graphs[k].exec));
          p->graphs.erase(p->graphs.begin() + k);
        } else {
          ++k;
        }
      }
      if (p->graphs.size() >= kGraphCacheMax) {
        HIP_TRY(hipGraphExecDestroy(p->graphs.front().exec));
        p->graphs.erase(p->graphs.begin());
      }
      hipGraph_t graph = nullptr;
      const bool xt_in = p->prev_xt;
      HIP_TRY(hipStreamBeginCapture(st, hipStreamCaptureModeThreadLocal));
      const int rc = enqueue_run(p, rtol, j0, j1);
      hipError_t ce = hipStreamEndCapture(st, &graph);
      if (rc != SLQ_OK) {
        if (graph) hipGraphDestroy(graph);
        p->prev_xt = xt_in;
        return rc;
      }
      if (ce != hipSuccess) return fail(SLQ_EHIP, "hipStreamEndCapture: %s", hipGetErrorString(ce));
      hipGraphExec_t exec = nullptr;
      ce = hipGraphInstantiate(&exec, graph, nullptr, nullptr, 0);
      hipGraphDestroy(graph);
      if (ce != hipSuccess) {
        p->prev_xt = xt_in;
        return fail(SLQ_EHIP, "hipGraphInstantiate: %s", hipGetErrorString(ce));
      }
      p->graphs.push_back({j0, j1, rtol, variant, exec, p->prev_xt});
      gi = p->graphs.size() - 1;
    }
    HIP_TRY(hipGraphLaunch(p->graphs[gi].exec, st));
    p->prev_xt = p->graphs[gi].xt_out;
  }
  p->probes_ready = false;
  p->ran = true;
  p->cur = j1;
  p->run_rtol = rtol;
  p->rule_src = 0;
  return SLQ_OK;
}

static int need_finished_run(const slq_plan *p, const char *who) {
  if (!p->ran) return fail(SLQ_EINVAL, "%s: no completed run", who);
  if (p->cur < p->deg)
    return fail(SLQ_EINVAL, "%s: the run stands at step %d of %d (slq_plan_run_steps); use slq_plan_quadrature_at for a prefix, or run to deg", who, p->cur, p->deg);
  return SLQ_OK;
}

extern "C" int slq_plan_get_tridiag(slq_plan *p, void *alpha, void *beta, int32_t *steps) {
  if (!p) return fail(SLQ_EINVAL, "plan is NULL");
  SLQ_TRY(need_lanczos(p, "slq_plan_get_tridiag"));
  if (!p->ran) return fail(SLQ_EINVAL, "slq_plan_get_tridiag: no completed run");
  HIP_TRY(hipSetDevice(p->ctx->device));
  hipStream_t st = p->ctx->stream;
  const int bp = p->bpad, deg = p->deg, P = p->nprobes;
  std::vector<double> ha((size_t)(deg + 1) * bp), hn((size_t)(deg + 1) * bp);
  std::vector<int> hs(bp);
  HIP_TRY(hipMemcpyAsync(ha.data(), p->st.alpha, ha.size() * 8, hipMemcpyDeviceToHost, st));
  HIP_TRY(hipMemcpyAsync(hn.data(), p->st.nu, hn.size() * 8, hipMemcpyDeviceToHost, st));
  HIP_TRY(hipMemcpyAsync(hs.data(), p->st.steps, (size_t)bp * 4, hipMemcpyDeviceToHost, st));
  int ring_bad = 0;
  HIP_TRY(hipMemcpyAsync(&ring_bad, p->ring_fail_d, sizeof(int), hipMemcpyDeviceToHost, st));
  HIP_TRY(hipStreamSynchronize(st));
  SLQ_TRY(ring_flag_status(ring_bad));
  for (int i = 0; i < P; ++i) {
    for (int t = 0; t <= deg; ++t) {
      const double a = ha[(size_t)t * bp + i];
      const double b = (t == 0) ? 0.0 : hn[(size_t)t * bp + i];
      if (p->dtype == SLQ_F64) {
        if (alpha) ((double *)alpha)[(size_t)i * (deg + 1) + t] = a;
        if (beta) ((double *)beta)[(size_t)i * (deg + 1) + t] = b;
      } else {
        if (alpha) ((float *)alpha)[(size_t)i * (deg + 1) + t] = (float)a;
        if (beta) ((float *)beta)[(size_t)i * (deg + 1) + t] = (float)b;
      }
    }
    if (steps) steps[i] = hs[i];
  }
  return SLQ_OK;
}

extern "C" int slq_plan_quadrature(slq_plan *p, int fun_id, const double *fun_params, double *quad,
                                   double *nodes, double *weights) {
  if (!p) return fail(SLQ_EINVAL, "plan is NULL");
  SLQ_TRY(need_lanczos(p, "slq_plan_quadrature"));
  SLQ_TRY(need_finished_run(p, "slq_plan_quadrature"));
  if (fun_id < SLQ_FUN_NONE || fun_id > SLQ_FUN_SOFTSIGN) return fail(SLQ_EINVAL, "Unknown function id %d.", fun_id);
  HIP_TRY(hipSetDevice(p->ctx->device));
  hipStream_t st = p->ctx->stream;
  const int deg = p->deg, P = p->nprobes;
  const double p0 = fun_params ? fun_params[0] : 0.0, p1 = fun_params ? fun_params[1] : 0.0;
  if (p->rule_src == 2) {
    hipLaunchKernelGGL(k_rule_reduce, dim3((P + 63) / 64), dim3(64), 0, st, P, deg, p->nodes_d, p->weights_d, p->st.vnorm2, fun_id, p0,
                       p1, p->quad_d);
  } else {
    const QuadShape q = quadrature_shape(deg, P);
    if (q.lds > 48 * 1024)
      HIP_TRY(hipFuncSetAttribute((const void *)k_quadrature, hipFuncAttributeMaxDynamicSharedMemorySize, 160 * 1024));
    HIP_TRY(hipMemsetAsync(p->fail_d, 0, sizeof(int), st));
    PROFILED(p, SLQ_K_QUADRATURE,
             hipLaunchKernelGGL(k_quadrature, dim3(q.grid), dim3(64), q.lds, st, p->st, q.lanes, fun_id, p0, p1,
                                p->quad_d, p->nodes_d, p->weights_d, p->fail_d));
  }
  HIP_TRY(hipGetLastError());
  int bad3[3] = {0, 0, 0};
  HIP_TRY(hipMemcpyAsync(bad3, p->fail_d, 3 * sizeof(int), hipMemcpyDeviceToHost, st));
  if (quad) HIP_TRY(hipMemcpyAsync(quad, p->quad_d, (size_t)P * 8, hipMemcpyDeviceToHost, st));
  if (nodes) HIP_TRY(hipMemcpyAsync(nodes, p->nodes_d, (size_t)P * deg * 8, hipMemcpyDeviceToHost, st));
  if (weights) HIP_TRY(hipMemcpyAsync(weights, p->weights_d, (size_t)P * deg * 8, hipMemcpyDeviceToHost, st));
  HIP_TRY(hipStreamSynchronize(st));
  const int bad = p->rule_src == 2 ? bad3[2] : bad3[0];
  if (p->rule_src != 2) {
    p->rule_src = 1;
    p->rule_fail_h = bad ? 1 : 0;
  }
  SLQ_TRY(ring_flag_status(bad3[1]));
  if (bad) return fail(SLQ_ENOTCONV, "tridiagonal QL did not converge for at least one probe");
  return SLQ_OK;
}

extern "C" int slq_plan_quadrature_at(slq_plan *p, int m, int rule, double endpoint, int fun_id, const double *fun_params,
                                      double *quad, double *nodes, double *weights, double *stage) {
  if (!p) return fail(SLQ_EINVAL, "plan is NULL");
  SLQ_TRY(need_lanczos(p, "slq_plan_quadrature_at"));
  if (!p->ran || p->cur < 1) return fail(SLQ_EINVAL, "slq_plan_quadrature_at: no steps done");
  if (m < 1 || m > p->cur) return fail(SLQ_EINVAL, "slq_plan_quadrature_at: m = %d must lie in [1, %d] (steps done)", m, p->cur);
  if (rule != 0 && rule != 1) return fail(SLQ_EINVAL, "slq_plan_quadrature_at: rule %d (0 Gauss, 1 Gauss-Radau)", rule);
  if (rule == 1 && !std::isfinite(endpoint)) return fail(SLQ_EINVAL, "slq_plan_quadrature_at: the Gauss-Radau rule needs a finite endpoint");
  if (fun_id < SLQ_FUN_NONE || fun_id > SLQ_FUN_SOFTSIGN) return fail(SLQ_EINVAL, "Unknown function id %d.", fun_id);
  HIP_TRY(hipSetDevice(p->ctx->device));
  hipStream_t st = p->ctx->stream;
  const int deg = p->deg, P = p->nprobes, kout = m + rule;
  const size_t rule_sz = (size_t)P * (deg + 1);
  if (!p->at_d) {
    hipError_t e = hipMalloc((void **)&p->at_d, (2 * (size_t)P + 4 + 2 * rule_sz) * 8);
    if (e == hipSuccess) e = hipMalloc((void **)&p->at_flags, 2 * sizeof(int));
    if (e != hipSuccess) {
      if (p->at_d) hipFree(p->at_d);
      p->at_d = nullptr;
      return fail(SLQ_ENOMEM, "slq_plan_quadrature_at: scratch: %s", hipGetErrorString(e));
    }
  }
  double *quad_d = p->at_d, *gauss_d = quad_d + P, *stage_d = gauss_d + P, *nodes_d = stage_d + 4, *weights_d = nodes_d + rule_sz;
  const double p0 = fun_params ? fun_params[0] : 0.0, p1 = fun_params ? fun_params[1] : 0.0;
  const int lanes = quadrature_lanes(m + 1);
  const size_t lds = (size_t)3 * (m + 1) * lanes * 8;
  if (lds > 48 * 1024)
    HIP_TRY(hipFuncSetAttribute((const void *)k_quadrature_at, hipFuncAttributeMaxDynamicSharedMemorySize, 160 * 1024));
  HIP_TRY(hipMemsetAsync(p->at_flags, 0, 2 * sizeof(int), st));
  const double residual_tol = std::sqrt((double)p->n) * p->run_rtol;
  PROFILED(p, SLQ_K_QUADRATURE,
           hipLaunchKernelGGL(k_quadrature_at, dim3((P + lanes - 1) / lanes), dim3(64), lds, st, p->st, m, rule, endpoint, residual_tol, lanes,
                              fun_id, p0, p1, quad_d, gauss_d, nodes_d, weights_d, p->at_flags));
  if (stage)
    hipLaunchKernelGGL(k_stage_reduce, dim3(1), dim3(kStageThreads), 0, st, P, (const double *)quad_d,
                       rule ? (const double *)gauss_d : (const double *)nullptr, stage_d);
  HIP_TRY(hipGetLastError());
  int flags[2] = {0, 0}, ring_bad = 0;
  HIP_TRY(hipMemcpyAsync(flags, p->at_flags, 2 * sizeof(int), hipMemcpyDeviceToHost, st));
  HIP_TRY(hipMemcpyAsync(&ring_bad, p->ring_fail_d, sizeof(int), hipMemcpyDeviceToHost, st));
  if (quad) HIP_TRY(hipMemcpyAsync(quad, quad_d, (size_t)P * 8, hipMemcpyDeviceToHost, st));
  if (nodes) HIP_TRY(hipMemcpyAsync(nodes, nodes_d, (size_t)P * kout * 8, hipMemcpyDeviceToHost, st));
  if (weights) HIP_TRY(hipMemcpyAsync(weights, weights_d, (size_t)P * kout * 8, hipMemcpyDeviceToHost, st));
  if (stage) HIP_TRY(hipMemcpyAsync(stage, stage_d, 4 * 8, hipMemcpyDeviceToHost, st));
  HIP_TRY(hipStreamSynchronize(st));
  SLQ_TRY(ring_flag_status(ring_bad));
  if (flags[1]) return fail(SLQ_EINVAL, "slq_plan_quadrature_at: endpoint = %g is not below the smallest Ritz value of every probe", endpoint);
  if (flags[0]) return fail(SLQ_ENOTCONV, "tridiagonal QL did not converge for at least one probe");
  return SLQ_OK;
}

extern "C" int slq_debug_plan_mark_stale(slq_plan *p, int nstale) {
  if (!p || nstale < 0) return fail(SLQ_EINVAL, "plan is NULL or nstale < 0");
  SLQ_TRY(need_lanczos(p, "slq_debug_plan_mark_stale"));
  p->nstale = nstale;
  return SLQ_OK;
}

extern "C" int slq_plan_get_basis(slq_plan *p, int probe, void *Q, int64_t ldq) {
  if (!p || !Q) return fail(SLQ_EINVAL, "plan/Q is NULL");
  SLQ_TRY(need_lanczos(p, "slq_plan_get_basis"));
  if (!p->keep_basis) return fail(SLQ_EINVAL, "plan was created without keep_basis");
  SLQ_TRY(need_finished_run(p, "slq_plan_get_basis"));
  if (probe < 0 || probe >= p->nprobes || ldq < p->n) return fail(SLQ_EINVAL, "bad probe index or ldq");
  HIP_TRY(hipSetDevice(p->ctx->device));
  hipStream_t st = p->ctx->stream;
  const int bp = p->bpad, deg = p->deg;
  std::vector<double> hn((size_t)(deg + 1) * bp), hscale((size_t)deg * bp, 0.0);
  HIP_TRY(hipMemcpyAsync(hn.data(), p->st.nu, hn.size() * 8, hipMemcpyDeviceToHost, st));
  SLQ_TRY(check_ring_flag(p));
  for (int t = 0; t < deg; ++t) {
    const double nu = hn[(size_t)t * bp + probe];
    hscale[(size_t)t * bp + probe] = nu > 0.0 ? 1.0 / nu : 0.0;
  }
  double *dscale = nullptr;
  HIP_TRY(hipMalloc((void **)&dscale, hscale.size() * 8));
  hipError_t e = hipMemcpyAsync(dscale, hscale.data(), hscale.size() * 8, hipMemcpyHostToDevice, st);
  int rc = e == hipSuccess ? SLQ_OK : fail(SLQ_EHIP, "scale upload: %s", hipGetErrorString(e));
  for (int t = 0; t < deg && rc == SLQ_OK; ++t)
    rc = panel_to_host(p, t, probe, 1, (char *)Q + (size_t)t * (size_t)ldq * p->esz, ldq, dscale + (size_t)t * bp);
  hipFree(dscale);
  return rc;
}

static int update_chunk_cols(const slq_plan *p) {
  const int V = p->dtype == SLQ_F64 ? 2 : 4;
  return std::min(192, (int)((150 * 1024 - sizeof(double) * kWaves * 64 * V) / ((size_t)p->PW * p->esz + sizeof(int))));
}

static int launch_reorth_update_range(slq_plan *p, int j, int istart, int r, bool axpy, int klass) {
  if (axpy && (istart != 0 || r < 1)) return fail(SLQ_EINVAL, "internal: the deferred axpy rides on column 0 of the first update chunk");
  hipStream_t st = p->ctx->stream;
  const int V = p->dtype == SLQ_F64 ? 2 : 4;
  const int kUpdChunk = update_chunk_cols(p);
  const dim3 gS(p->nblkS, p->NP);
  for (int i0 = istart; i0 < r; i0 += kUpdChunk) {
    const int rc = std::min(kUpdChunk, r - i0);
    const size_t lds = sizeof(double) * kWaves * 64 * V + (size_t)rc * p->PW * p->esz + (size_t)rc * sizeof(int);
    PROFILED(p, klass,
             DISPATCH(p->dtype, p->LPR,
                      (launch_reorth_update_kernel<F, L>(p, gS, lds, st, j, i0, rc, axpy && i0 == 0))));
  }
  return SLQ_OK;
}

static int launch_reorth_update(slq_plan *p, int j, int r, int istart, bool axpy, int klass) { return launch_reorth_update_range(p, j, istart, r, axpy, klass); }

static int launch_action_accumulate(slq_plan *p, int t0, int nc, bool init) {
  hipStream_t st = p->ctx->stream;
  const dim3 gS(p->nblkS, p->NP);
  PROFILED(p, SLQ_K_COMBINE,
           DISPATCH(p->dtype, p->LPR,
                    (k_action_accumulate<F, L><<<gS, dim3(kBlock), 0, st>>>(p->n, (const F *)p->ring, p->slot_stride, p->S, t0, nc,
// ... 1581 lines not shown
  SLQ_TRY(precond_grow(pc.cols, 2 * n * kPrecondChunkCols * 8, "slq_kernel_precond_trace_pointgrad"));
  slq_dmat Z{op->ctx, op->n, kPrecondChunkCols, pc.cols.as<double>()}, W{op->ctx, op->n, kPrecondChunkCols, pc.cols.as<double>() + n * kPrecondChunkCols};
  const double sigma2 = pc.base->k_noise;
  const int64_t count = g->count;
  bool first = true;
  for (int c0 = 0; c0 < pc.rank; c0 += kPrecondChunkCols) {
    const int nc = std::min(kPrecondChunkCols, pc.rank - c0);
    SLQ_TRY(precond_columns_device(op, 1, c0, nc, Z.d, "slq_kernel_precond_trace_pointgrad"));
    SLQ_TRY(precond_columns_device(op, 0, c0, nc, W.d, "slq_kernel_precond_trace_pointgrad"));
    SLQ_TRY(slq_kernel_pointgrad_update(g, &Z, 0, &W, 0, nc, -alpha / sigma2, first ? beta : 1.0));
    first = false;
  }
  g->count = count;
  return SLQ_OK;
}

extern "C" int slq_debug_kernel_precond_addresses(const slq_operator *op, uint64_t *out4) {
  SLQ_TRY(precond_handle(op, "slq_debug_kernel_precond_addresses"));
  if (!out4) return fail(SLQ_EINVAL, "slq_debug_kernel_precond_addresses: out is NULL");
  const KernelPrecond &pc = *op->pre;
  out4[0] = (uint64_t)(uintptr_t)pc.L.p, out4[1] = (uint64_t)(uintptr_t)pc.G.p, out4[2] = (uint64_t)(uintptr_t)pc.pivots, out4[3] = (uint64_t)(uintptr_t)pc.dres.p;
  return SLQ_OK;
}
extern "C" int slq_debug_kernel_precond_h(slq_operator *op, double *H) {
  SLQ_TRY(precond_handle(op, "slq_debug_kernel_precond_h"));
  if (!H) return fail(SLQ_EINVAL, "slq_debug_kernel_precond_h: H is NULL");
  const KernelPrecond &pc = *op->pre;
  HIP_TRY(hipSetDevice(op->ctx->device));
  HIP_TRY(hipStreamSynchronize(op->ctx->stream));
  return create_guarded(nullptr, [&]() {
    const size_t r = (size_t)pc.rank_max, rpad = (size_t)pc.rpad;
    std::vector<double> h(rpad * rpad);
    HIP_TRY(hipMemcpy(h.data(), pc.H.p, h.size() * 8, hipMemcpyDeviceToHost));
    for (size_t i = 0; i < r; ++i) std::copy(h.begin() + i * rpad, h.begin() + i * rpad + r, H + i * r);
    return (int)SLQ_OK;
  });
}
extern "C" int slq_debug_kernel_precond_timing(const slq_operator *op, double *out2) {
  SLQ_TRY(precond_handle(op, "slq_debug_kernel_precond_timing"));
  if (!out2) return fail(SLQ_EINVAL, "slq_debug_kernel_precond_timing: out is NULL");
  out2[0] = op->pre->device_ms, out2[1] = op->pre->host_ms;
  return SLQ_OK;
}

extern "C" int slq_measure_stream(slq_context *ctx, int mode, size_t bytes_per_stream, int reps, double *gbps) {
  if (!ctx || !gbps || mode < 0 || mode > 2 || reps < 1 || bytes_per_stream < (1u << 20))
    return fail(SLQ_EINVAL, "bad arguments");
  HIP_TRY(hipSetDevice(ctx->device));
  hipStream_t st = ctx->stream;
  const int64_t nvec = (int64_t)(bytes_per_stream / 16);
  double *buf = nullptr;
  HIP_TRY(hipMalloc((void **)&buf, (size_t)nvec * 32 + 64));
  double *w = buf, *q = buf + nvec * 2, *sink = q + nvec * 2;
  hipEvent_t a = nullptr, b = nullptr;
  hipError_t e = hipMemsetAsync(buf, 0, (size_t)nvec * 32 + 64, st);
  if (e == hipSuccess) e = hipEventCreate(&a);
  if (e == hipSuccess) e = hipEventCreate(&b);
  const int blocks = ctx->num_cus * 2;
  float ms = 0.f;
  if (e == hipSuccess) {
    for (int i = 0; i < 2; ++i) k_stream_probe<<<dim3(blocks), dim3(kBlock), 0, st>>>(w, q, nvec, mode, 1e-9, sink);
    e = hipEventRecord(a, st);
    for (int i = 0; i < reps; ++i) k_stream_probe<<<dim3(blocks), dim3(kBlock), 0, st>>>(w, q, nvec, mode, 1e-9, sink);
    if (e == hipSuccess) e = hipEventRecord(b, st);
    if (e == hipSuccess) e = hipEventSynchronize(b);
    if (e == hipSuccess) e = hipEventElapsedTime(&ms, a, b);
    if (e == hipSuccess) e = hipGetLastError();
  }
  if (a) hipEventDestroy(a);
  if (b) hipEventDestroy(b);
  hipFree(buf);
  if (e != hipSuccess) return fail(SLQ_EHIP, "slq_measure_stream: %s", hipGetErrorString(e));
  const double streams = mode == 1 ? 3.0 : 2.0;
  *gbps = streams * (double)nvec * 16.0 * reps / (ms * 1e-3) / 1e9;
  return SLQ_OK;
}

extern "C" int slq_plan_set_probes_device(slq_plan *p, const void *d_X, int64_t ldx) {
  if (!p || !d_X) return fail(SLQ_EINVAL, "plan/X is NULL");
  if (ldx < p->n) return fail(SLQ_EINVAL, "ldx (%lld) < n (%d)", (long long)ldx, p->n);
  HIP_TRY(hipSetDevice(p->ctx->device));
  hipStream_t st = p->ctx->stream;
  if (ldx != p->n) return fail(SLQ_EINVAL, "device probes must be contiguous columns (ldx == n)");
  if (p->nprobes < p->bpad) HIP_TRY(hipMemsetAsync(slot_ptr(p, 0), 0, (size_t)p->slot_stride * p->esz, st));
  dim3 g((p->n + 63) / 64, (p->nprobes + 63) / 64);
  PROFILED(p, SLQ_K_PROBES, {
    if (p->dtype == SLQ_F64)
      hipLaunchKernelGGL(k_cols_to_panel<double>, g, dim3(256), 0, st, p->n, (const double *)d_X, 0, p->nprobes, (double *)slot_ptr(p, 0), p->PW, p->op->perm_d.as<int32_t>());
    else
      hipLaunchKernelGGL(k_cols_to_panel<float>, g, dim3(256), 0, st, p->n, (const float *)d_X, 0, p->nprobes, (float *)slot_ptr(p, 0), p->PW, p->op->perm_d.as<int32_t>());
  });
  p->pdf_sphere = 0;
  return init_from_probes(p, 0);
}

extern "C" int slq_fttr_batch(slq_context *ctx, int nb, int n, int k, const double *theta, const double *alpha,
                              const double *beta, double *weights) {
  if (!ctx || !theta || !alpha || !beta || !weights) return fail(SLQ_EINVAL, "NULL argument");
  if (nb <= 0 || n <= 0 || k <= 0) return fail(SLQ_EINVAL, "bad sizes");
  HIP_TRY(hipSetDevice(ctx->device));
  hipStream_t st = ctx->stream;
  double *buf = nullptr;
  const size_t nth = (size_t)nb * k, nab = (size_t)nb * n;
  HIP_TRY(hipMalloc((void **)&buf, (2 * nth + 2 * nab) * 8));
  double *dth = buf, *dw = buf + nth, *da = dw + nth, *db = da + nab;
  hipError_t e = hipMemcpyAsync(dth, theta, nth * 8, hipMemcpyHostToDevice, st);
  if (e == hipSuccess) e = hipMemcpyAsync(da, alpha, nab * 8, hipMemcpyHostToDevice, st);
  if (e == hipSuccess) e = hipMemcpyAsync(db, beta, nab * 8, hipMemcpyHostToDevice, st);
  if (e == hipSuccess) {
    k_fttr<<<dim3((unsigned)((nth + 127) / 128)), dim3(128), 0, st>>>(nb, n, k, dth, da, db, dw);
    e = hipGetLastError();
  }
  if (e == hipSuccess) e = hipMemcpyAsync(weights, dw, nth * 8, hipMemcpyDeviceToHost, st);
  if (e == hipSuccess) e = hipStreamSynchronize(st);
  hipFree(buf);
  if (e != hipSuccess) return fail(SLQ_EHIP, "slq_fttr_batch: %s", hipGetErrorString(e));
  return SLQ_OK;
}

extern "C" int slq_eigh_tridiag_batch(slq_context *ctx, int nb, int deg, const double *d, const double *e, double *w,
                                      double *Z) {
  if (!ctx || !d || !e || !w) return fail(SLQ_EINVAL, "ctx/d/e/w is NULL");
  if (nb <= 0 || deg <= 0 || deg > kMaxDeg) return fail(SLQ_EINVAL, "bad batch size or degree (deg <= %d)", kMaxDeg);
  const size_t lds_onchip = ((size_t)2 * deg + (size_t)deg * (deg + 1)) * 8 + (size_t)deg * sizeof(int);
  const bool zg = lds_onchip > 160 * 1024;
  const size_t lds = zg ? (size_t)2 * deg * 8 + (size_t)deg * sizeof(int) : lds_onchip;
  HIP_TRY(hipSetDevice(ctx->device));
  hipStream_t st = ctx->stream;
  const size_t in = (size_t)nb * deg, zz = Z ? in * deg : 0, zs = zg ? in * (deg + 1) : 0;
  double *buf = nullptr;
  HIP_TRY(hipMalloc((void **)&buf, (3 * in + zz + zs + 1) * 8));
  double *dd = buf, *de = dd + in, *dw = de + in, *dz = Z ? dw + in : nullptr, *dscr = zg ? dw + in + zz : nullptr;
  int *dfail = (int *)(dw + in + zz + zs);
  hipError_t err = hipMemcpyAsync(dd, d, in * 8, hipMemcpyHostToDevice, st);
  if (err == hipSuccess) err = hipMemcpyAsync(de, e, in * 8, hipMemcpyHostToDevice, st);
  if (err == hipSuccess) err = hipMemsetAsync(dfail, 0, sizeof(int), st);
  if (err == hipSuccess && lds > 48 * 1024)
    err = hipFuncSetAttribute((const void *)k_eigh_tridiag<false>, hipFuncAttributeMaxDynamicSharedMemorySize, 160 * 1024);
  if (err == hipSuccess) {
    if (zg)
      k_eigh_tridiag<true><<<dim3(nb), dim3(64), lds, st>>>(deg, dd, de, dw, dz, dscr, dfail);
    else
      k_eigh_tridiag<false><<<dim3(nb), dim3(64), lds, st>>>(deg, dd, de, dw, dz, nullptr, dfail);
    err = hipGetLastError();
  }
  int bad = 0;
  if (err == hipSuccess) err = hipMemcpyAsync(&bad, dfail, sizeof(int), hipMemcpyDeviceToHost, st);
  if (err == hipSuccess) err = hipMemcpyAsync(w, dw, in * 8, hipMemcpyDeviceToHost, st);
  if (err == hipSuccess && Z) err = hipMemcpyAsync(Z, dz, zz * 8, hipMemcpyDeviceToHost, st);
  if (err == hipSuccess) err = hipStreamSynchronize(st);
  hipFree(buf);
  if (err != hipSuccess) return fail(SLQ_EHIP, "slq_eigh_tridiag_batch: %s", hipGetErrorString(err));
  if (bad) return fail(SLQ_ENOTCONV, "tridiagonal QL did not converge for at least one matrix");
  return SLQ_OK;
}

extern "C" int slq_quadrature_batch(slq_context *ctx, int nb, int deg, const double *d, const double *e,
                                    int fun_id, const double *fun_params, double *quad, double *nodes,
                                    double *weights) {
  if (!ctx || !d || !e) return fail(SLQ_EINVAL, "ctx/d/e is NULL");
  if (nb <= 0 || deg <= 0 || deg > kMaxDeg) return fail(SLQ_EINVAL, "bad batch size or degree");
  if (fun_id < SLQ_FUN_NONE || fun_id > SLQ_FUN_SOFTSIGN) return fail(SLQ_EINVAL, "Unknown function id %d.", fun_id);
  const QuadShape qs = quadrature_shape(deg, nb);
  HIP_TRY(hipSetDevice(ctx->device));
  hipStream_t st = ctx->stream;
  const int bp = (nb + 63) / 64 * 64;
// ... 315 lines not shown
```

primate_amd/csrc/slq_kernels.hpp:

```cpp
#pragma once
#include <hip/hip_runtime.h>
#include <stdint.h>

#include "slq_common.hpp"

namespace slq {

#ifdef SLQ_DEBUG_TIMES
__device__ unsigned long long *g_dbg_times = nullptr;
#endif

typedef int32_t csr_i8 __attribute__((ext_vector_type(8), aligned(4)));
typedef float csr_f8 __attribute__((ext_vector_type(8), aligned(4)));
typedef double csr_d8 __attribute__((ext_vector_type(8), aligned(8)));
template <typename F> struct CsrVals;
template <> struct CsrVals<float> { typedef csr_f8 type; };
template <> struct CsrVals<double> { typedef csr_d8 type; };

template <typename F, int PW>
__device__ __forceinline__ typename VecT<F>::type gather_row_uniform(const int32_t *__restrict__ colind,
                                                                      const F *__restrict__ vals, int p0, int p1,
                                                                      const F *xbase ,
                                                                      unsigned lane_off ) {
  using VF = typename VecT<F>::type;
// ... 1509 lines not shown
  double *gram;
  int *active;
  int *steps;
  int bpad, nprobes, deg;
};

struct OmegaState {
  int mode;
  int est_prev;
  int force;
  int PW, NP;
  double *D;
  double *rho;
  double *g3;
  double *Dm;
  int *read;
  int *rescue;
  int *census;
  unsigned long long *cnt;
  double theta;
  double tol_k;
  double eps_norm;
};
constexpr int kOmCntOffered = 0, kOmCntRead = 1, kOmCntRescue = 2, kOmCntViol = 3, kOmCntTrans = 4, kOmCntInnov = 5, kOmCntMargin = 6;

constexpr int kFinSlices = 16;
constexpr int kFinThreads = 64 * kFinSlices;
__device__ __forceinline__ double sum_partials_slice(const double *part, int nblk, int bpad, int col, int s) {
  double a0 = 0.0, a1 = 0.0, a2 = 0.0, a3 = 0.0;
  if (col < bpad) {
    int b = s;
    for (; b + 3 * kFinSlices < nblk; b += 4 * kFinSlices) {
      a0 += part[(int64_t)b * bpad + col];
      a1 += part[(int64_t)(b + kFinSlices) * bpad + col];
      a2 += part[(int64_t)(b + 2 * kFinSlices) * bpad + col];
      a3 += part[(int64_t)(b + 3 * kFinSlices) * bpad + col];
    }
    for (; b < nblk; b += kFinSlices) a0 += part[(int64_t)b * bpad + col];
  }
  return (a0 + a1) + (a2 + a3);
}
__device__ __forceinline__ double sum_partials(const double *__restrict__ part, int nblk, int bpad,
                                               int col, double *red ) {
  const int c = threadIdx.x & 63, s = threadIdx.x >> 6;
  red[s * 64 + c] = sum_partials_slice(part, nblk, bpad, col, s);
  __syncthreads();
  double tot = 0.0;
#pragma unroll
  for (int k = 0; k < kFinSlices; ++k) tot += red[k * 64 + c];
  __syncthreads();
  return tot;
}
__device__ __forceinline__ double sum_partials_kblock(const double *part, int nblk, int bpad, int col, double *red ) {
  static_assert(kBlock * 2 == kFinThreads, "a thread of the sweep workgroup walks two slices");
  const int c = threadIdx.x & 63, s = threadIdx.x >> 6;
  red[s * 64 + c] = sum_partials_slice(part, nblk, bpad, col, s);
  red[(s + kFinSlices / 2) * 64 + c] = sum_partials_slice(part, nblk, bpad, col, s + kFinSlices / 2);
  __syncthreads();
  double tot = 0.0;
#pragma unroll
  for (int k = 0; k < kFinSlices; ++k) tot += red[k * 64 + c];
  __syncthreads();
  return tot;
}

__global__ __launch_bounds__(kFinThreads) void k_fin_init(StepState st, const double *__restrict__ partN,
                                                  int nblk, int sphere, double n_as_double) {
  __shared__ double red4[kFinThreads];
  const int col = blockIdx.x * 64 + (threadIdx.x & 63);
  const double s = nblk > 0 ? sum_partials(partN, nblk, st.bpad, col, red4) : (col < st.nprobes ? n_as_double : 0.0);
  if ((threadIdx.x >> 6) == 0 && col < st.bpad) {
    const double nu0 = sqrt(s);
    const int act = (col < st.nprobes) && (nu0 > 0.0);
    st.nu[col] = nu0;
    st.vnorm2[col] = sphere ? n_as_double : s;
    st.active[col] = act;
    st.steps[col] = 0;
    st.coefA[col] = act ? 1.0 / nu0 : 0.0;
    st.coefA[st.bpad + col] = 0.0;
  }
}

__global__ __launch_bounds__(kFinThreads) void k_fin_alpha(StepState st, const double *__restrict__ partA,
                                                   int nblk, int j, int xt) {
  __shared__ double red4[kFinThreads];
  const int col = blockIdx.x * 64 + (threadIdx.x & 63);
  double a = sum_partials(partA, nblk, st.bpad, col, red4);
  if ((threadIdx.x >> 6) == 0 && col < st.bpad) {
    const int act = st.active[col];
    if (xt) a -= st.coefA[col] * st.coefA[st.bpad + col] * st.cross[col];
    if (act) st.alpha[(int64_t)j * st.bpad + col] = a;
    st.coefB[col] = act ? a / st.nu[(int64_t)j * st.bpad + col] : 0.0;
  }
}

__global__ __launch_bounds__(kFinThreads) void k_fin_beta(StepState st, const double *__restrict__ partN,
                                                  int nblk, int j, double residual_tol, int xt) {
  __shared__ double red4[kFinThreads];
  const int col = blockIdx.x * 64 + (threadIdx.x & 63);
  const double s = sum_partials(partN, nblk, st.bpad, col, red4);
  if (xt) {
    const double x = sum_partials(partN + (int64_t)nblk * st.bpad, nblk, st.bpad, col, red4);
    if ((threadIdx.x >> 6) == 0 && col < st.bpad) st.cross[col] = x;
  }
  if ((threadIdx.x >> 6) == 0 && col < st.bpad) {
    double sc = 0.0, cp = 0.0;
    if (st.active[col]) {
      const double beta = sqrt(s);
      st.nu[(int64_t)(j + 1) * st.bpad + col] = beta;
      st.steps[col] = j + 1;
      if (beta < residual_tol || (j + 1) == st.deg || !(beta == beta)) {
        st.active[col] = 0;
      } else {
        sc = 1.0 / beta;
        cp = beta / st.nu[(int64_t)j * st.bpad + col];
      }
    }
    st.coefA[col] = sc;
    st.coefA[st.bpad + col] = cp;
  }
}

__global__ __launch_bounds__(kFinThreads) void k_fin_adots(StepState st, const double *__restrict__ part, int nblk,
                                                   int j, int RC, double orth_tol) {
  __shared__ double red4[kFinThreads];
  const int i = blockIdx.y;
  const int col = blockIdx.x * 64 + (threadIdx.x & 63);
  const int64_t slab = (int64_t)nblk * st.bpad;
  const double a = sum_partials(part, nblk, st.bpad, col, red4);
  double d = 0.0, g = 0.0;
  if (i > 0) {
    d = sum_partials(part + i * slab, nblk, st.bpad, col, red4);
    g = sum_partials(part + (RC - 1 + i) * slab, nblk, st.bpad, col, red4);
  }
  if ((threadIdx.x >> 6) == 0 && col < st.bpad) {
    const int act = st.active[col];
    const double nuj = st.nu[(int64_t)j * st.bpad + col];
    const double cb = (act && nuj > 0.0) ? a / nuj : 0.0;
    if (i == 0) {
      if (act) st.alpha[(int64_t)j * st.bpad + col] = a;
      st.coefB[col] = cb;
      st.gamma[col] = 0.0;
    } else {
      const double nu = st.nu[(int64_t)(j - i) * st.bpad + col];
      double gm = 0.0;
      if (act && nu > 0.0) {
        const double sproj = (d - cb * g) / nu;
        if (fabs(sproj) > orth_tol) gm = sproj / nu;
      }
      st.gamma[(int64_t)i * st.bpad + col] = gm;
    }
  }
}

__device__ __forceinline__ double gram_sproj(const StepState &st, int j, int i, int col, double cb, double hi, double *nut_out) {
  constexpr int R1 = kFusedMaxR + 1;
  const int64_t bp = st.bpad;
  const double *Gc = st.gram + (int64_t)(j & 1) * R1 * bp + col;
  const double *Gp = st.gram + (int64_t)((j + 1) & 1) * R1 * bp + col;
  const double sc = st.coefA[col], cp = st.coefA[bp + col];
  const int t = j - i;
  const double nut = st.nu[(int64_t)t * bp + col];
  *nut_out = nut;
  const double g1 = Gc[(int64_t)(i - 1) * bp], g0 = Gc[(int64_t)i * bp];
  const double alt = st.alpha[(int64_t)t * bp + col];
  double s = g1 + (alt / nut) * g0;
  if (t >= 1 && i + 1 <= kFusedMaxR) {
    const double nutm = st.nu[(int64_t)(t - 1) * bp + col];
    if (nutm > 0.0) s += (nut / nutm) * hi;
  }
  const double nujm = st.nu[(int64_t)(j - 1) * bp + col];
  const double wt_wjm = i == 1 ? nujm * nujm : Gp[(int64_t)(i - 1) * bp];
  const double d = sc * (nut * s) - cp * wt_wjm;
  return (d - cb * g0) / nut;
}

__device__ __forceinline__ void om_max_bits(unsigned long long *w, double x) { atomicMax(w, (unsigned long long)__double_as_longlong(x > 0.0 ? x : 0.0)); }

__device__ __forceinline__ double omega_edge(const StepState &st, const OmegaState &om, int j, int i, int col, double cb, double orth_tol, bool measured_only) {
  constexpr int R1 = kFusedMaxR + 1;
  const int64_t bp = st.bpad;
  const int panel = col / om.PW;
  const int t = j - i;
  const double ghi = st.gram[((int64_t)(j & 1) * R1 + (i + 1)) * bp + col];
  const double nut0 = st.nu[(int64_t)t * bp + col];
  if (!(st.active[col] && nut0 > 0.0)) {
    om.D[col] = 0.0;
    om.rho[col] = 0.0;
    if (om.mode == 2) om.Dm[col] = 0.0;
    return 0.0;
  }
  int *read_j = om.read + (int64_t)j * om.NP + panel, *resc_j = om.rescue + (int64_t)j * om.NP + panel;
  const bool est_in = !measured_only && om.est_prev && t >= 1 && om.read[(int64_t)(j - 1) * om.NP + panel] == 0;
  const double sc = st.coefA[col];
  double nut;
  const double sproj_m = gram_sproj(st, j, i, col, cb, ghi, &nut);
  double gm = 0.0;
  bool need_read = (om.force & 1) != 0;
  if (om.mode == 1) {
    const double rho = (est_in ? sc * nut * om.rho[col] : 0.0) + om.theta;
    const bool cert = fabs(sproj_m) + rho <= om.tol_k;
    const bool soon = fabs(sproj_m) + rho + om.theta > om.tol_k;
    om.D[col] = sproj_m * nut;
    om.rho[col] = rho;
    if (est_in) {
      if (!cert) atomicOr(resc_j, 1);
      else need_read = need_read || soon;
    } else {
      if (fabs(sproj_m) > orth_tol) gm = sproj_m / nut;
      need_read = need_read || gm != 0.0 || soon;
    }
    if ((om.force & 2) && t >= 1 && !measured_only) atomicOr(resc_j, 1);
  } else {
    if (fabs(sproj_m) > orth_tol) gm = sproj_m / nut;
    double rho = om.theta, sproj_e = sproj_m;
    if (est_in) {
      double nut2;
      sproj_e = gram_sproj(st, j, i, col, cb, om.g3[col], &nut2);
      rho = sc * nut * om.rho[col] + om.theta;
      const double nutm = st.nu[(int64_t)(t - 1) * bp + col];
      if (nutm > 0.0) om_max_bits(om.cnt + kOmCntInnov, fabs(ghi - om.Dm[col]) / nutm / om.eps_norm);
      {
        const double room = orth_tol - fabs(sproj_m);
        om_max_bits(om.cnt + kOmCntMargin, room > 0.0 ? rho / room : __longlong_as_double(0x7ff0000000000000ll));
      }
      const bool says_zero = fabs(sproj_e) + rho <= om.tol_k;
      if ((says_zero && fabs(sproj_m) > orth_tol) || fabs(sproj_e - sproj_m) > rho) atomicAdd(om.cnt + kOmCntViol, 1ull);
      if (!says_zero) {
        atomicOr(resc_j, 1);
        sproj_e = sproj_m;
        rho = om.theta;
      }
    }
    need_read = need_read || gm != 0.0 || fabs(sproj_e) + rho + om.theta > om.tol_k;
    om.D[col] = sproj_e * nut;
    om.rho[col] = rho;
    om.Dm[col] = sproj_m * nut;
  }
  if (need_read) atomicOr(read_j, 1);
  return gm;
}

__global__ __launch_bounds__(kFinThreads) void k_fin_gram(StepState st, const double *__restrict__ part, int nblk, int j, int RC, double orth_tol, OmegaState om) {
  __shared__ double red4[kFinThreads];
  const int i = blockIdx.y;
  const int col = blockIdx.x * 64 + (threadIdx.x & 63);
  const double a_raw = sum_partials(part, nblk, st.bpad, col, red4);
  if ((threadIdx.x >> 6) == 0 && col < st.bpad) {
    constexpr int R1 = kFusedMaxR + 1;
    const int64_t bp = st.bpad;
    const double *Gc = st.gram + (int64_t)(j & 1) * R1 * bp + col;
    const int act = st.active[col];
    const double nuj = st.nu[(int64_t)j * bp + col];
    const double sc = st.coefA[col], cp = st.coefA[bp + col];
    const double a = a_raw - (j > 0 ? sc * cp * Gc[bp] : 0.0);
    const double cb = (act && nuj > 0.0) ? a / nuj : 0.0;
    if (i == 0) {
      if (act) st.alpha[(int64_t)j * bp + col] = a;
      st.coefB[col] = cb;
      st.gamma[col] = 0.0;
    } else if (om.mode != 0 && i == RC - 1) {
      const double gm = omega_edge(st, om, j, i, col, cb, orth_tol, false);
      st.gamma[(int64_t)i * bp + col] = gm;
      if (om.census && gm != 0.0) atomicAdd(om.census + ((int64_t)j * R1 + i) * om.NP + col / om.PW, 1);
    } else {
      const int t = j - i;
      const double nut0 = st.nu[(int64_t)t * bp + col];
      double gm = 0.0;
      if (act && nut0 > 0.0) {
        double nut;
        const double sproj = gram_sproj(st, j, i, col, cb, i + 1 <= kFusedMaxR ? Gc[(int64_t)(i + 1) * bp] : 0.0, &nut);
        if (fabs(sproj) > orth_tol) gm = sproj / nut;
      }
      st.gamma[(int64_t)i * bp + col] = gm;
      if (om.mode != 0 && gm != 0.0) atomicOr(om.read + (int64_t)j * om.NP + col / om.PW, 1);
      if (om.census && gm != 0.0) atomicAdd(om.census + ((int64_t)j * R1 + i) * om.NP + col / om.PW, 1);
    }
  }
}

template <typename F, int LPR>
__global__ __launch_bounds__(kBlock) void k_omega_rescue_dot(int n, const F *__restrict__ ring, int64_t slot_stride, int S, int j, int back,
                                                             double *partD, int *ticket , StepState st,
                                                             double orth_tol, OmegaState om) {
  using VF = typename VecT<F>::type;
  constexpr int V = Geo<F, LPR>::V, PW = Geo<F, LPR>::PW, RPW = Geo<F, LPR>::RPW;
  __shared__ double red[kWaves * 64 * V];
  __shared__ double red4[kFinThreads];
  __shared__ int last;
  const int panel = blockIdx.y;
  if (om.rescue[(int64_t)j * om.NP + panel] == 0) return;
  const int bpad = st.bpad, nblk = gridDim.x;
  const int lane = threadIdx.x & 63, wave = threadIdx.x >> 6;
  const int g = lane / LPR, cl = lane % LPR;
  const int64_t poff = (int64_t)panel * n * PW + cl * V;
  const F *A = ring + (int64_t)ring_slot(j, S) * slot_stride + poff;
  const F *B = ring + (int64_t)ring_slot(j - back, S) * slot_stride + poff;
  VF acc = (VF)(F)0;
  const int stride = gridDim.x * kWaves * RPW;
  for (int row = (blockIdx.x * kWaves + wave) * RPW + g; row < n; row += stride) {
    const int64_t ro = (int64_t)row * PW;
    acc += *(const VF *)(A + ro) * *(const VF *)(B + ro);
  }
  block_reduce_columns<F, LPR>(acc, red, partD + (int64_t)blockIdx.x * bpad + panel * PW);
  __threadfence();
  __syncthreads();
  if (threadIdx.x == 0) {
    const int drawn = __hip_atomic_fetch_add(ticket + panel, 1, __ATOMIC_ACQ_REL, __HIP_MEMORY_SCOPE_AGENT);
    last = drawn == nblk - 1;
  }
  __syncthreads();
  if (!last) return;
  __builtin_amdgcn_fence(__ATOMIC_ACQUIRE, "agent");
  if (threadIdx.x == 0) __hip_atomic_store(ticket + panel, 0, __ATOMIC_RELAXED, __HIP_MEMORY_SCOPE_AGENT);
  const int RC = back;
  const int cend = min((panel + 1) * PW, bpad);
  for (int c0 = panel * PW; c0 < cend; c0 += 64) {
    const int col = c0 + lane;
    const double m = sum_partials_kblock(partD, nblk, bpad, col < cend ? col : bpad, red4);
    if (wave == 0 && col < cend) {
      constexpr int R1 = kFusedMaxR + 1;
      st.gram[((int64_t)(j & 1) * R1 + RC) * bpad + col] = m;
      st.gamma[(int64_t)(RC - 1) * bpad + col] = omega_edge(st, om, j, RC - 1, col, st.coefB[col], orth_tol, true);
    }
  }
}

__global__ __launch_bounds__(kFinThreads) void k_fin_beta_gram(StepState st, const double *__restrict__ part, int nblk, int j, int RC,
                                                       double residual_tol, OmegaState om) {
  __shared__ double red4[kFinThreads];
  constexpr int R1 = kFusedMaxR + 1;
  const int q = blockIdx.y;
  const int col = blockIdx.x * 64 + (threadIdx.x & 63);
  double s = 0.0;
  if (q <= RC) s = sum_partials(part + (int64_t)q * nblk * st.bpad, nblk, st.bpad, col, red4);
  if (om.mode != 0 && q == RC) {
    const int *read_j = om.read + (int64_t)j * om.NP;
    if ((threadIdx.x >> 6) == 0 && col < st.bpad) {
      const bool skipped = read_j[min(col / om.PW, om.NP - 1)] == 0;
      if (om.mode == 2) om.g3[col] = skipped ? om.D[col] : s;
      else if (skipped) s = om.D[col];
    }
    if (blockIdx.x == 0 && threadIdx.x == 0) {
// ... 763 lines not shown
```

primate_amd/csrc/slq_plan_shape.hpp:

```cpp
#pragma once

#include <stddef.h>
#include <stdint.h>

#include <algorithm>
#include <cmath>

#include "slq_format.hpp"
#include "slq_kernelop.hpp"
#include "slq_kernelprecond.hpp"
#include "slq_sequence.hpp"
#include "slq_switches.hpp"

namespace slq {

enum { OP_CSR = 0, OP_DENSE = 1, OP_CALLBACK = 2, OP_DEVICE_CALLBACK = 3, OP_GRAM = 4, OP_KERNEL = 5, OP_KERNEL_PRECOND = 6 };
inline bool is_kernel_kind(int kind) { return kind == OP_KERNEL || kind == OP_KERNEL_PRECOND; }
constexpr int kF32 = 0, kF64 = 1;

enum class PlanKind { Ring = 0, KeepBasis = 1, Recompute = 2, Chebyshev = 3, ChebyshevAction = 4 };
inline bool is_cheb(PlanKind k) { return k == PlanKind::Chebyshev || k == PlanKind::ChebyshevAction; }
inline int basis_mode_of(PlanKind k) { return k == PlanKind::KeepBasis ? 1 : (k == PlanKind::Recompute ? 2 : 0); }

struct PlanFacts {
// ... 205 lines not shown
    s.acc_cols = kChebAccCols;
    s.y_slot = s.S;
  }
  s.slot_stride = (int64_t)s.NP * f.n * s.PW;
  s.rmax = std::max(keep_basis ? deg : orth, 1);
  s.pipelined = f.kind == OP_CSR && s.LPR == 64 && (sw.pipe >= 0 ? sw.pipe != 0 : (double)f.nnz / (double)std::max<int64_t>(f.n, 1) > 5.5);
  grid_sizes(sw, f.n, s.LPR, s.NP, f.num_cus, &s.nblkA, &s.nblkS, &s.nblkU, s.pipelined != 0);
  {
    const double gathers = f.kind != OP_CSR ? 0.0 : (double)(f.upper ? f.nnz_u : f.nnz) / (double)std::max<int64_t>(f.n, 1);
    const int local = f.kind == OP_CSR && gathers <= 3.2;
    const int per_cu_env = sw.blocks_per_cu_alpha;
    const int rows_per_block = kWaves * (64 / s.LPR);
    const int64_t chunk = (f.n + 7) / 8;
    const int per_panel = per_cu_env > 0 ? std::max(8, f.num_cus * per_cu_env / s.NP)
                                         : (local ? std::max(8, f.num_cus * 4 / s.NP) : f.num_cus * 2);
    const int per_xcd = (int)std::min<int64_t>(per_panel / 8, (chunk + rows_per_block - 1) / rows_per_block);
    s.nblkF = 8 * std::max(per_xcd, 1);
    s.alpha_pad = (size_t)or_auto(sw.alpha_lds_pad, (per_cu_env > 0 || local) ? 0 : 65536);
  }
  {
    for (int x = 0; x < 9; ++x) s.rs_xcd[x] = f.xcd_tile[x], s.rs_xcd_u[x] = f.xcd_tile_u[x];
    if (f.kind == OP_CSR && f.has_tiles && sw.tiles) {
      const int R = wants_merged_stream(f, sw);
      if (s.LPR == 64) {
        s.ringR = 1;
        if (f.tiles_ringed) {
          s.stream = STREAM_BASE;
          if (f.upper_stream && f.upper_per_row <= (double)sw.ring_alpha_max_x100 / 100.0)
            s.rs_upper = 1, s.rs_u_padded = f.upper_padded;
        }
      } else if (R && f.merged[R == 2 ? 0 : 1].available) {
        const PlanFacts::Merged &m = f.merged[R == 2 ? 0 : 1];
        s.ringR = R;
        s.stream = R == 2 ? STREAM_MERGED2 : STREAM_MERGED4;
        s.rs_upper = m.upper, s.rs_u_padded = m.u_padded;
        for (int x = 0; x < 9; ++x) s.rs_xcd[x] = m.xcd_tile[x], s.rs_xcd_u[x] = m.xcd_tile[x];
      }
      s.ring_staged = sw.ring_staged != 0;
    }
  }
  {
    const int img_kib = f.has_tiles ? (f.tiles_max_cols + 16) * (SLQ_TILE_DB ? 2 : 1) : 160;
    const int per_cu_t = f.tiles_ringed ? 1 : std::max(1, or_auto(sw.blocks_per_cu_tiled, std::max(1, std::min(4, 160 / std::max(img_kib, 1)))));
    int per_xcd_t = std::max(1, f.num_cus * per_cu_t / 8);
    per_xcd_t = std::max(1, std::min(per_xcd_t, or_auto(sw.tiled_wgs_per_xcd, per_xcd_t)));
    if (f.has_tiles) {
      int mn = 1 << 30;
      for (int x = 0; x < 8; ++x) mn = std::min(mn, std::max(1, s.rs_xcd[x + 1] - s.rs_xcd[x]));
      per_xcd_t = std::min(per_xcd_t, mn);
    }
    s.nblkT = 8 * per_xcd_t;
  }
  s.part_maxblk = std::max(std::max(std::max(std::max(s.nblkA, s.nblkF), s.nblkU), s.nblkS), s.nblkT);
  s.dense_ks = 0;
  const bool dense32 = f.kind == OP_DENSE && f.dtype == kF32 && sw.dense_mfma;
  if (dense32 || (f.kind == OP_DENSE && f.dtype == kF64 && sw.dense_mfma && s.PW >= 32 && !sw.dense_tile16)) {
    const int rw = dense32 ? kDense32BM : 32 * (kWaves / (s.PW >= 64 ? 2 : 1));
    const double wgs = (double)((f.n + rw - 1) / rw) * s.NP;
    double best = 1e30;
    const int forced = sw.dense_ksplit;
    for (int ks = 1; ks <= 16; ++ks) {
      const double cost = std::ceil(wgs * ks / f.num_cus) / ks + 0.005 * ks;
      if ((forced > 0 && ks == forced) || (forced <= 0 && cost < best - 1e-12)) { best = cost; s.dense_ks = ks; }
    }
  }
  if (is_kernel_kind(f.kind)) {
    const int slabs = kernel_schedule(f.n, s.PW, s.NP, f.num_cus).nslabs;
    s.dense_ks = slabs > 1 ? slabs : 0;
  }
  s.t_slabs_bound = f.kind == OP_CSR ? 0 : 1 + (((f.kind == OP_DENSE && (f.dtype == kF32 || s.PW >= 32)) || is_kernel_kind(f.kind)) ? 16 : 0);
  if (f.kind != OP_DENSE) s.dense_class = DENSE_K_NONE;
  else if (!sw.dense_mfma || (f.dtype != kF64 && s.dense_ks <= 0)) s.dense_class = DENSE_K_PANEL;
  else if (s.dense_ks <= 0) s.dense_class = DENSE_K_3TERM;
  else if (f.dtype == kF32) s.dense_class = DENSE_K_LDS32;
  else s.dense_class = sw.dense_lds && f.lda % 2 == 0 && s.PW >= 64 ? DENSE_K_LDS : DENSE_K_TILE;
  {
    seq::SequenceFacts &q = s.seq;
    q.csr = f.kind == OP_CSR, q.far_le4 = f.far_per_row <= 4.0, q.tiles_ringed = f.tiles_ringed, q.upper = f.upper;
    q.ringR = s.ringR, q.rs_desc_u = s.rs_upper, q.rs_u_padded = s.rs_u_padded;
    q.deg = deg, q.orth = orth, q.nstale = 0, q.basis_mode = basis_mode_of(f.plan);
    q.dense_class = s.dense_class, q.pipelined = s.pipelined;
    q.fused = sw.fused, q.merged = sw.merged, q.mgs = sw.mgs, q.stored_u = sw.stored_u, q.nt = sw.nt, q.cross = sw.cross, q.sw_gram = sw.gram;
    q.sw_gram_csr = sw.gram_csr, q.sw_ring_gen = sw.ring_gen, q.sw_ring_deep = sw.ring_deep;
    q.last_store = (sw.last_store || action) ? 1 : 0;
    q.ring_alpha = sw.ring_alpha, q.ring_rev = sw.ring_rev;
    seq::derive_plan_flags(q);
    s.omega_on = q.gram && sw.omega != 0 && orth == 3 && s.S >= 4 && !f.affine && s.PW >= 32;
    q.omega_on = s.omega_on;
  }

  const size_t bp = (size_t)s.bpad, hist = (size_t)s.hist;
  const size_t slot_bytes = (size_t)s.slot_stride * esz;
  for (int r = 0; r < kNumRegions; ++r) s.ws[r].id = r;
  auto region = [&s](int id, size_t bytes, int zeroed, int counted) { s.ws[id].bytes = bytes, s.ws[id].zeroed = zeroed, s.ws[id].counted = counted; };
  region(WS_RING, (size_t)(s.S + (recompute ? 2 : (action ? 1 : 0))) * slot_bytes, 0, 1);
  {
    ScalOffsets &o = s.scal;
    size_t at = 0;
    o.alpha = at, at += (hist + 1) * bp;
    o.nu_margin = at, at += (size_t)orth * bp;
    o.nu = at, at += (hist + 1) * bp;
    o.vnorm2 = at, at += bp;
    o.coefA = at, at += 2 * bp;
    o.coefB = at, at += bp;
    o.cross = at, at += bp;
    o.gram = at, at += (size_t)2 * (kFusedMaxR + 1) * bp;
    o.gamma = at, at += (size_t)s.rmax * bp;
    o.end = at;
    region(WS_SCAL, o.end * 8, 2, 1);
  }
  region(WS_PART, (size_t)kReorthChunk * s.part_maxblk * bp * 8, 0, 1);
  region(WS_ACC_COEF, recompute ? (size_t)deg * bp * 8 : 0, 0, 1);
  region(WS_SWEEP_COLS, 4 * sizeof(unsigned long long), 1, 0);
  region(WS_OM_BUF, s.omega_on ? 4 * bp * 8 : 0, 1, 0);
  region(WS_OM_FLAGS, s.omega_on ? (size_t)2 * (deg + 1) * s.NP * sizeof(int) : 0, 1, 0);
  region(WS_OM_CNT, s.omega_on ? 8 * sizeof(unsigned long long) : 0, 1, 0);
  region(WS_OM_CENSUS, (s.seq.gram && sw.omega == 2 && !cheb) ? (size_t)(deg + 1) * (kFusedMaxR + 1) * s.NP * sizeof(int) : 0, 1, 0);
  {
    ActiveOffsets &o = s.active;
    o.steps = bp, o.fail = 2 * bp, o.ring_fail = o.fail + 1, o.fail2 = o.fail + 2, o.end = o.fail + 4;
    region(WS_ACTIVE, o.end * sizeof(int), 0, 0);
  }
  region(WS_QUAD, (bp + 2 * bp * hist) * 8, 0, 1);
  const size_t nmom = cheb ? (size_t)(2 * deg + 1) : 0;
  region(WS_CHEB_MU, nmom * bp * 8, 1, 1);
  region(WS_CHEB_OUT, cheb ? bp * sizeof(int) : 0, 1, 0);
  region(WS_CHEB_COEF, cheb ? (nmom + 4) * 8 : 0, 0, 0);
  region(WS_T, f.kind == OP_CSR ? 0 : (size_t)(1 + s.dense_ks) * slot_bytes, 0, 1);
  region(WS_T2, f.kind == OP_GRAM             ? (size_t)s.NP * (size_t)f.mrows * s.PW * esz
                : f.kind == OP_KERNEL_PRECOND ? slot_bytes + precond_scratch_words(f.n, s.bpad, (int)f.mrows, f.num_cus) * 8
                                              : 0, 0, 1);
  return s;
}

inline size_t plan_workspace_bytes(const PlanShape &s) {
  size_t b = 0;
  for (const Region &r : s.ws)
    if (r.counted) b += r.bytes;
  return b;
}

inline size_t plan_estimate_bytes(const PlanShape &s, const PlanFacts &f) {
  return s.ws[WS_RING].bytes + (size_t)s.t_slabs_bound * (size_t)s.slot_stride * esize_of(f.dtype) + s.ws[WS_T2].bytes;
}

}
```

primate_amd/csrc/slq_sequence.hpp:

```cpp
#pragma once

#include <algorithm>

namespace slq {
namespace seq {

constexpr int kMaxFusedR = 8;
constexpr int kMaxRingR = 3;

struct SequenceFacts {
  int csr = 0;
  int far_le4 = 0;
  int tiles_ringed = 0;
  int upper = 0;
  int ringR = 0;
  int rs_desc_u = 0;
  int rs_u_padded = 0;
  int deg = 0, orth = 0, nstale = 0;
  int basis_mode = 0;
  int dense_class = 0;
  int pipelined = 0;
  int omega_on = 0;
  int fused = 1, merged = 1, mgs = 0, stored_u = 1, nt = 1, cross = 1, sw_gram = 1, sw_gram_csr = 1, sw_ring_gen = 1, sw_ring_deep = 1,
      last_store = 0, ring_alpha = 2, ring_rev = 1;
// ... 45 lines not shown
  int gen = 0;
  int alpha_tiled = 0;
  int alpha_upper = 0;
  int half = 0;
  int pipe_on = 0;
  int xt_alpha = 0;
  int xt_dots = 0;
  int xt_update = 0;
  int omega = 0;
  int est_prev = 0;
  int product = PRODUCT_UNFUSED;
  int blk_alpha = BLK_S;
  int blk_dots = BLK_S;
  int blk_beta = BLK_S;
  int prev_xt = 0;
};
constexpr int kNumShape = 18;

inline void shape_to_array(const StepShape &s, int *out) {
  const int v[kNumShape] = {s.seq, s.r, s.tiled, s.gen, s.alpha_tiled, s.alpha_upper, s.half, s.pipe_on, s.xt_alpha, s.xt_dots, s.xt_update, s.omega,
                            s.est_prev, s.product, s.blk_alpha, s.blk_dots, s.blk_beta, s.prev_xt};
  for (int i = 0; i < kNumShape; ++i) out[i] = v[i];
}

inline StepShape step_shape(const SequenceFacts &f, int j, bool prev_xt) {
  StepShape s;
  s.r = f.orth > 0 ? std::min(j + 1 + f.nstale, f.orth) : 0;
  const int r = s.r;
  const bool mgs = f.nstale > 0 || f.mgs;
  const bool gathers_cached = f.fused == 2 || f.far_le4;
  const bool plan_tiled = f.ringR > 0;
  const bool stored_u = f.csr && f.fused != 0 && !gathers_cached && r >= 1 && r <= kMaxFusedR && !mgs && f.stored_u && f.merged && !plan_tiled;
  if (!(f.csr && f.fused != 0 && (gathers_cached || stored_u) && r <= kMaxFusedR && !mgs)) {
    s.seq = r == 0 ? SEQ_SWEEPS_PLAIN : (mgs ? SEQ_SWEEPS_MGS : SEQ_SWEEPS_CGS);
    if (f.csr && plan_tiled && f.tiles_ringed) s.product = PRODUCT_RING, s.gen = f.ring_gen, s.blk_alpha = BLK_T;
    else if (f.csr) s.product = PRODUCT_CSR, s.blk_alpha = BLK_A;
    else if (f.dense_class >= 2) s.product = PRODUCT_DENSE, s.blk_alpha = BLK_DENSE;
    else s.product = PRODUCT_UNFUSED, s.blk_alpha = BLK_S;
    return s;
  }
  const bool tiled = plan_tiled && !stored_u && (!f.tiles_ringed || r <= kMaxRingR || f.ring_deep);
  const bool gen = tiled && f.tiles_ringed && (f.ring_gen || r > kMaxRingR);
  const bool alpha_tiled = tiled && !(f.tiles_ringed && f.upper && (f.ring_alpha == 0 || (f.ring_alpha == 2 && !f.rs_desc_u)));
  s.tiled = tiled, s.gen = gen, s.alpha_tiled = alpha_tiled;
  s.alpha_upper = alpha_tiled && f.tiles_ringed && f.rs_desc_u && f.ring_alpha == 2;
  s.half = !alpha_tiled && f.upper;
  s.pipe_on = f.pipelined && !tiled;
  const int blk_tu = tiled ? BLK_T : BLK_U;
  s.blk_alpha = alpha_tiled ? BLK_T : BLK_F;
  s.blk_dots = s.blk_beta = blk_tu;
  const int pad_bit = (alpha_tiled && gen && s.alpha_upper && f.rs_u_padded) ? 8 : 0;
  const int rev_bit = (tiled && f.tiles_ringed && f.ring_rev) ? 4 : 0;
  const int nostore_bit = (j == f.deg - 1 && f.basis_mode != 1 && f.last_nostore && !stored_u && (!tiled || gen)) ? 16 : 0;
  const bool merged = r > 0 && (tiled || f.merged);
  const bool gram_ring = gen && f.gram && r >= 1;
  const bool gram_csr = f.gram_csr && !tiled && gathers_cached && !stored_u && r >= 1;
  if (gram_ring || gram_csr) {
    s.seq = gram_ring ? SEQ_GRAM_RING : SEQ_GRAM_CSR;
    s.xt_alpha = (j > 0 ? 1 : 0) | pad_bit;
    s.xt_update = rev_bit | nostore_bit;
    s.omega = gram_ring && f.omega_on && r == 3 && f.orth == 3;
    s.est_prev = s.omega && j >= 3;
    return s;
  }
  const int su = stored_u ? 2 : 0;
  const int cross_bit = (!merged && f.cross) ? 1 : 0;
  s.seq = stored_u ? SEQ_STORED_U : (merged ? SEQ_MERGED : SEQ_SEPARATE);
  s.xt_alpha = ((prev_xt && j > 0) ? 1 : 0) | pad_bit;
  s.xt_dots = merged ? su : 0;
  s.xt_update = cross_bit | su | rev_bit | nostore_bit;
  s.prev_xt = cross_bit;
  return s;
}

inline int plan_sequence_of(const SequenceFacts &f) {
  switch (step_shape(f, 0, false).seq) {
    case SEQ_GRAM_RING: case SEQ_GRAM_CSR: return 4;
    case SEQ_MERGED: case SEQ_SEPARATE: return 1;
    case SEQ_STORED_U: return 2;
    default: return 0;
  }
}

struct ChebStepShape {
  int sweeps = 1;
  int tiled = 0;
  int gen = 0;
  int pipe_on = 0;
  int xt_update = 1;
  int product = PRODUCT_UNFUSED;
  int blk_product = BLK_S;
  int blk = BLK_S;
  int alpha_pass = 0;
};
constexpr int kNumChebShape = 9;

inline void cheb_shape_to_array(const ChebStepShape &s, int *out) {
  const int v[kNumChebShape] = {s.sweeps, s.tiled, s.gen, s.pipe_on, s.xt_update, s.product, s.blk_product, s.blk, s.alpha_pass};
  for (int i = 0; i < kNumChebShape; ++i) out[i] = v[i];
}

inline ChebStepShape cheb_step_shape(const SequenceFacts &facts, int j) {
  SequenceFacts f = facts;
  f.orth = 0, f.nstale = 0;
  const StepShape l = step_shape(f, j, false);
  ChebStepShape s;
  if (l.seq == SEQ_SWEEPS_PLAIN) {
    s.sweeps = 1, s.gen = l.gen, s.product = l.product, s.blk_product = l.blk_alpha;
    s.blk = BLK_S;
    s.xt_update = 1;
    return s;
  }
  s.sweeps = 0, s.tiled = l.tiled, s.gen = l.gen, s.pipe_on = l.pipe_on, s.blk = l.blk_beta;
  s.xt_update = l.xt_update | 1;
  return s;
}

inline int cheb_action_ring_slots(int nsteps, int acc) { return std::max(2, std::min(acc, nsteps + 1)); }

inline int cheb_action_piece_after(int nsteps, int acc, int j, int c0) {
  const int unconsumed = j + 2 - c0;
  return (unconsumed >= acc || j == nsteps - 1) ? unconsumed : 0;
}

inline int cheb_action_schedule(int nsteps, int acc, int *t0, int *nc, int *after, int cap) {
  int np = 0, c0 = 0;
  for (int j = 0; j < nsteps; ++j) {
    const int m = cheb_action_piece_after(nsteps, acc, j, c0);
    if (!m) continue;
    if (np < cap) {
      if (t0) t0[np] = c0;
      if (nc) nc[np] = m;
      if (after) after[np] = j;
    }
    ++np;
    c0 += m;
  }
  return np;
}

}
}
```

primate_amd/csrc/slq_switches.hpp:

```cpp
#pragma once

#include <climits>
#include <cstdlib>

namespace slq {

constexpr int kAuto = INT_MIN;

#define SLQ_SWITCH_TABLE(OP, PLAN, BOTH, USE)                                                                                                            \
  BOTH(tiles, "SLQ_TILES", 2, "LDS workgroup tiles: 0 none, 1 landed behind barriers, 2 fed through a ring of LDS slots; operator: rows regrouped, plan: passes use them") \
  OP(debug, "SLQ_DEBUG", 0, "print the phases and findings of an operator's creation on stderr")                                                      \
  OP(reorder, "SLQ_REORDER", -1, "XCD-aware RCM row order: 0 never, 1 n >= 65536, 2 always, -1 automatic")                                            \
  OP(rcm_sub, "SLQ_RCM_SUB", 0, "second reordering level: runs of Cuthill-McKee levels per XCD chunk (0: 1, and what the tile sweep finds)")           \
  OP(sym_alpha, "SLQ_SYM_ALPHA", 1, "alpha pass on the upper triangle of an exactly symmetric CSR")                                                  \
  OP(tile_rows, "SLQ_TILE_ROWS", 24, "tile caps of the barrier tiles: rows")                                                                         \
  OP(tile_cols, "SLQ_TILE_COLS", 72, "... distinct panel rows")                                                                                      \
  OP(device_build, "SLQ_DEVICE_BUILD", 1, "operators with ring tiles built on the device (0: on the host; 2: both, compared byte for byte)")          \
  OP(ring_order, "SLQ_RING_ORDER", 0, "order of a tile's lines (1: own rows first; experiments)")                                                    \
  OP(ring_upper_regroup, "SLQ_RING_UPPER_REGROUP", 1, "upper-triangle tiles regrouped into runs of the base tiles")                                  \
  OP(ring_pad_rows, "SLQ_RING_PAD_ROWS", 1, "upper-triangle tile streams with every row padded to whole chunks of four entries")                     \
  USE(host_threads, "SLQ_HOST_THREADS", kAuto, "host threads of operator creation and of the pinned probe upload (auto: min(16, hardware threads))")  \
  PLAN(fused, "SLQ_FUSED", 1, "1: recompute-SpMM passes where they pay, 0: store-and-revisit sweeps, 2: passes always")                               \
  PLAN(nt, "SLQ_NT", 1, "nontemporal hints on streamed-once rows")                                                                                   \
  PLAN(graph, "SLQ_GRAPH", 1, "capture the launch sequence into a hipGraph")                                                                         \
  PLAN(mgs, "SLQ_MGS", 0, "exact modified-Gram-Schmidt order")                                                                                       \
  PLAN(stored_u, "SLQ_STORED_U", 1, "non-local operators: merged pass stores u, update pass reads it back")                                          \
  PLAN(merged, "SLQ_MERGED", 1, "alpha from the merged alpha+dots pass")                                                                             \
  PLAN(cross, "SLQ_CROSS", 1, "q_c.q_p from the update pass's cross term")                                                                           \
  PLAN(gram, "SLQ_GRAM", 1, "Gram sequence: projections from Gram rows of the update passes")                                                        \
  PLAN(gram_csr, "SLQ_GRAM_CSR", 1, "... also on the generic passes (plans without ring-fed tiles)")                                                 \
  PLAN(ring_gen, "SLQ_RING_GEN", 1, "wide-panel ring-fed passes through k_ring_pass (0: k_csr_ring_pass)")                                           \
  PLAN(ring_deep, "SLQ_RING_DEEP", 1, "steps with 4..8 ring columns on the 8-wave form of k_ring_pass (0: generic passes)")                          \
  PLAN(ring_narrow, "SLQ_RING_NARROW", 1, "panels of 32 / 16 lanes per row on merged tiles (0: generic passes on the tiles' row order)")             \
  PLAN(ring_staged, "SLQ_RING_STAGED", 0, "alpha-only pass: loader waves through registers instead of LDS-DMA")                                      \
  PLAN(ring_alpha, "SLQ_RING_ALPHA", 2, "alpha-only pass of a tiled symmetric operator: 2 ring over the upper-triangle stream, 1 over full rows, 0 generic") \
  PLAN(ring_alpha_max_x100, "SLQ_RING_ALPHA_MAX_X100", 260, "... takes the upper-triangle stream up to this many (x100) landed rows per row")        \
  PLAN(ring_rev, "SLQ_RING_REV", 1, "the ring-fed update pass sweeps panels and tiles in reverse")                                                   \
  PLAN(last_store, "SLQ_LAST_STORE", 0, "1: the update pass of a run's last step stores W_deg although it is never read")                            \
  PLAN(sweep_skip, "SLQ_SWEEP_SKIP", 1, "the update sweep skips ring columns whose coefficient is zero for the whole panel")                         \
  PLAN(acc_skip, "SLQ_ACC_SKIP", 1, "the accumulation of a recompute plan's replay skips such columns")                                              \
  PLAN(defer_axpy, "SLQ_DEFER_AXPY", 1, "block-CGS sweeps: the dots sweeps are read-only, the update sweep applies the three-term axpy")             \
  PLAN(omega, "SLQ_OMEGA", 1, "edge recurrence: 1 on, 0 every column read, 2 verify (clamped to 0..2)")                                              \
  PLAN(omega_trip, "SLQ_OMEGA_TRIP", -1, "tests: the step at which every panel reads (-1: none)")                                                    \
  PLAN(omega_rescue, "SLQ_OMEGA_RESCUE", -1, "tests: the step at which every panel takes the rescue (-1: none)")                                     \
  PLAN(dense_mfma, "SLQ_DENSE_MFMA", 1, "dense operator on the matrix cores (0: k_dense_panel)")                                                     \
  PLAN(dense_tile16, "SLQ_DENSE_TILE16", 0, "keep the 16-row dense kernel also for wide panels")                                                     \
  PLAN(dense_lds, "SLQ_DENSE_LDS", 1, "fp64 dense product with the operands staged in LDS (0: k_dense_mfma_tile)")                                   \
  PLAN(dense_ksplit, "SLQ_DENSE_KSPLIT", 0, "K split of the big-tile dense kernels (0: fewest workgroup rounds)")                                    \
  PLAN(pipe, "SLQ_PIPE", -1, "pipelined row loop in the dots/update passes (-1: by operator)")                                                       \
  PLAN(lpr, "SLQ_LPR", 0, "lanes per row, 8/16/32/64 (0: by the number of probes)")                                                                  \
  PLAN(blocks_per_cu, "SLQ_BLOCKS_PER_CU", kAuto, "resident workgroups per CU: SpMM and streaming sweeps (auto: 4 / 2)")                             \
  PLAN(blocks_per_cu_spmm, "SLQ_BLOCKS_PER_CU_SPMM", kAuto, "... of k_spmm_3term alone")                                                            \
  PLAN(blocks_per_cu_stream, "SLQ_BLOCKS_PER_CU_STREAM", kAuto, "... of the streaming sweeps alone")                                                \
  PLAN(blocks_per_cu_fused, "SLQ_BLOCKS_PER_CU_FUSED", kAuto, "... of the dots/update passes, per panel (auto: 2; 1 with the pipelined loop)")       \
  PLAN(blocks_per_cu_alpha, "SLQ_BLOCKS_PER_CU_ALPHA", 0, "... of the alpha pass, total over the panels (0: by gathers per row)")                    \
  PLAN(blocks_per_cu_tiled, "SLQ_BLOCKS_PER_CU_TILED", kAuto, "... of the barrier-tile passes (auto: what their LDS images admit)")                  \
  PLAN(tiled_wgs_per_xcd, "SLQ_TILED_WGS_PER_XCD", kAuto, "experiments: fewer workgroups sweeping each XCD chunk in the tiled passes")               \
  PLAN(alpha_lds_pad, "SLQ_ALPHA_LDS_PAD", kAuto, "LDS padding (bytes) that caps the alpha pass's residency (auto: 0 or 65536)")                     \
  PLAN(fused_pad, "SLQ_FUSED_LDS_PAD", -1, "... of the dots/update passes (-1: by row loop)")                                                        \
  PLAN(spmm_pad, "SLQ_SPMM_LDS_PAD", 57344, "... of k_spmm_3term")                                                                                   \
  PLAN(known_norm, "SLQ_KNOWN_NORM", 1, "Rademacher probes drawn on the device skip the norm sweep (it is n)")                                       \
  PLAN(pinned_upload, "SLQ_PINNED_UPLOAD", 1, "slq_plan_set_probes through two pinned buffers (0: direct copy)")                                     \
  PLAN(debug_pass, "SLQ_DEBUG_PASS", 3, "diagnostic builds: the pass (PASS_* code) whose time line is stamped")

inline int env_int(const char *name, int dflt, bool *present = nullptr) {
  const char *s = getenv(name);
  if (present) *present = s != nullptr;
  return (s && *s) ? atoi(s) : dflt;
}
inline int or_auto(int v, int dflt) { return v != kAuto ? v : dflt; }

#define SLQ_SW_FIELD(field, name, dflt, meaning) int field = dflt;
#define SLQ_SW_READ(field, name, dflt, meaning) s.field = env_int(name, dflt);
#define SLQ_SW_NONE(field, name, dflt, meaning)

struct OperatorSwitches {
  SLQ_SWITCH_TABLE(SLQ_SW_FIELD, SLQ_SW_NONE, SLQ_SW_FIELD, SLQ_SW_NONE)
  bool tiles_forced = false;
};
struct PlanSwitches {
  SLQ_SWITCH_TABLE(SLQ_SW_NONE, SLQ_SW_FIELD, SLQ_SW_FIELD, SLQ_SW_NONE)
};

#define SLQ_SW_TILES_FORCED(field, name, dflt, meaning) env_int(name, dflt, &s.tiles_forced);
inline OperatorSwitches read_operator_switches() {
  OperatorSwitches s;
  SLQ_SWITCH_TABLE(SLQ_SW_READ, SLQ_SW_NONE, SLQ_SW_READ, SLQ_SW_NONE)
  SLQ_SWITCH_TABLE(SLQ_SW_NONE, SLQ_SW_NONE, SLQ_SW_TILES_FORCED, SLQ_SW_NONE)
  return s;
}
inline PlanSwitches read_plan_switches() {
  PlanSwitches s;
  SLQ_SWITCH_TABLE(SLQ_SW_NONE, SLQ_SW_READ, SLQ_SW_READ, SLQ_SW_NONE)
  s.omega = s.omega < 0 ? 0 : (s.omega > 2 ? 2 : s.omega);
  return s;
}
#define SLQ_SW_USE(field, name, dflt, meaning) inline int read_##field() { return env_int(name, dflt); }
SLQ_SWITCH_TABLE(SLQ_SW_NONE, SLQ_SW_NONE, SLQ_SW_NONE, SLQ_SW_USE)

#undef SLQ_SW_FIELD
#undef SLQ_SW_READ
#undef SLQ_SW_NONE
#undef SLQ_SW_TILES_FORCED
#undef SLQ_SW_USE

}
```

primate_amd/engine.py:

```python

from __future__ import annotations

import ctypes as C
import os
from typing import Optional

import numpy as np

from . import _capi
from ._capi import check, ptr


def fun_spec(fun, **kwargs) -> tuple:
	if fun is None:
		fun = "identity"
	if not isinstance(fun, str):
		return None, None
	assert fun in _capi.FUN_IDS, "If given as a string, matrix_function be one of the builtin functions."
	p = np.zeros(4)
	if fun == "exp":
		p[0] = kwargs.get("t", 1.0)
	elif fun == "smoothstep":
		p[0], p[1] = kwargs.get("a", 0.0), kwargs.get("b", 1.0)
	elif fun == "numrank":
# ... 346 lines not shown
	def basis_info(self) -> dict:
		m, s, a = C.c_int(), C.c_int(), C.c_int()
		check(_capi.lib().slq_plan_basis_mode(self._h, C.byref(m), C.byref(s), C.byref(a)))
		return {"mode": int(m.value), "ring_slots": int(s.value), "acc_cols": int(a.value)}

	@property
	def workspace_bytes(self) -> int:
		b = C.c_size_t()
		check(_capi.lib().slq_plan_workspace_bytes(self._h, C.byref(b)))
		return b.value

	def describe(self) -> dict:
		info = _capi.PlanInfo()
		check(_capi.lib().slq_plan_describe(self._h, C.byref(info)))
		d = {k: getattr(info, k) for k, _ in _capi.PlanInfo._fields_}
		d["sequence"] = {0: "sweeps", 1: "fused", 2: "fused_stored_u", 4: "fused_gram"}[d["sequence"]]
		mode = C.c_int()
		check(_capi.lib().slq_plan_window_verify(self._h, C.byref(mode), None))
		d["omega"] = int(mode.value)
		kernel, ksplit = C.c_int(), C.c_int()
		check(_capi.lib().slq_plan_dense_path(self._h, C.byref(kernel), C.byref(ksplit)))
		d["dense_kernel"], d["dense_ksplit"] = int(kernel.value), int(ksplit.value)
		return d

	def set_probes(self, X: np.ndarray):
		X = np.asarray(X)
		X = X.reshape(-1, 1) if X.ndim == 1 else X
		assert X.shape == (self.op.shape[1], self.nprobes), f"probes must be {(self.op.shape[1], self.nprobes)}"
		X = np.asfortranarray(X, dtype=self.op.dtype)
		check(_capi.lib().slq_plan_set_probes(self._h, ptr(X), X.shape[0]))

	def set_probes_device(self, dptr: int):
		check(_capi.lib().slq_plan_set_probes_device(self._h, C.c_void_p(int(dptr)), self.op.shape[0]))

	def generate_probes(self, pdf: str = "rademacher", seed: int = 0, probe_offset: int = 0):
		assert pdf in _capi.PDF_IDS, f"Invalid distribution '{pdf}' supplied."
		check(_capi.lib().slq_plan_generate_probes(self._h, _capi.PDF_IDS[pdf], int(seed), int(probe_offset)))

	def get_probes(self) -> np.ndarray:
		X = np.empty((self.op.shape[0], self.nprobes), dtype=self.op.dtype, order="F")
		check(_capi.lib().slq_plan_get_probes(self._h, ptr(X), X.shape[0]))
		return X

	def get_probes_into(self, out: "DeviceMatrix", o0: int):
		check(_capi.lib().slq_plan_get_probes_dmat(self._h, out._h, int(o0)))

	def run(self, rtol: float = 1e-8, upto: Optional[int] = None):
		if upto is None:
			rc = _capi.lib().slq_plan_run(self._h, float(rtol))
		else:
			rc = _capi.lib().slq_plan_run_steps(self._h, float(rtol), int(upto))
		if rc == _capi.SLQ_ECALLBACK and getattr(self.op, "error", None) is not None:
			raise self.op.error
		check(rc)

	@property
	def steps_done(self) -> int:
		c = C.c_int()
		check(_capi.lib().slq_plan_steps_done(self._h, C.byref(c)))
		return int(c.value)

	def quadrature_at(self, m: Optional[int] = None, fun="identity", rule: str = "gauss", endpoint: Optional[float] = None,
					  return_rule: bool = False, return_stage: bool = False, **fun_kwargs):
		rid, endpoint = _rule_args(rule, endpoint)
		fid, params = fun_spec(fun, **fun_kwargs)
		if fid is None and return_stage:
			raise ValueError("the stage statistics are reduced on the device: built-in function names only")
		host_fun = fid is None
		m = self.steps_done if m is None else int(m)
		want_rule = return_rule or host_fun
		k = m + rid
		quad = np.zeros(self.nprobes)
		nodes = np.zeros((self.nprobes, k)) if want_rule and k > 0 else None
		weights = np.zeros((self.nprobes, k)) if want_rule and k > 0 else None
		stage = np.zeros(4) if return_stage else None
		check(_capi.lib().slq_plan_quadrature_at(self._h, m, rid, endpoint, 0 if host_fun else fid, ptr(params), ptr(quad), ptr(nodes),
												 ptr(weights), ptr(stage)))
		if host_fun:
			ident = np.sum(nodes * weights, axis=1)
			vn2 = np.divide(quad, ident, out=np.zeros_like(quad), where=ident != 0)
			quad = np.array([np.sum(fun(nodes[i]) * weights[i]) for i in range(self.nprobes)]) * vn2
		out = (quad,) + ((nodes, weights) if return_rule else ()) + ((stage,) if return_stage else ())
		return out[0] if len(out) == 1 else out

	def tridiag(self) -> tuple:
		a = np.zeros((self.nprobes, self.deg + 1), dtype=self.op.dtype)
		b = np.zeros((self.nprobes, self.deg + 1), dtype=self.op.dtype)
		s = np.zeros(self.nprobes, dtype=np.int32)
		check(_capi.lib().slq_plan_get_tridiag(self._h, ptr(a), ptr(b), ptr(s)))
		return a, b, s

	def quadrature(self, fun="identity", return_rule: bool = False, **fun_kwargs):
		fid, params = fun_spec(fun, **fun_kwargs)
		host_fun = fid is None
		want_rule = return_rule or host_fun
		quad = np.zeros(self.nprobes)
		nodes = np.zeros((self.nprobes, self.deg)) if want_rule else None
		weights = np.zeros((self.nprobes, self.deg)) if want_rule else None
		check(
			_capi.lib().slq_plan_quadrature(
				self._h, 0 if host_fun else fid, ptr(params), ptr(quad), ptr(nodes), ptr(weights)
			)
		)
		if host_fun:
			ident = np.sum(nodes * weights, axis=1)
			vn2 = np.divide(quad, ident, out=np.zeros_like(quad), where=ident != 0)
			self._vnorm2 = vn2
			quad = np.array([np.sum(fun(nodes[i]) * weights[i]) for i in range(self.nprobes)]) * vn2
		return (quad, nodes, weights) if return_rule else quad

	def fun_action(self, fun="identity", **fun_kwargs) -> np.ndarray:
		fid, params = fun_spec(fun, **fun_kwargs)
		assert fid is not None, "fun_action evaluates built-in function names on the device"
		Y = np.zeros((self.op.shape[0], self.nprobes), dtype=self.op.dtype, order="F")
		check(_capi.lib().slq_plan_fun_action(self._h, fid, ptr(params), ptr(Y), Y.shape[0]))
		return Y

	def fun_action_into(self, out: "DeviceMatrix", o0: int, fun="identity", **fun_kwargs):
		fid, params = fun_spec(fun, **fun_kwargs)
		assert fid is not None
		check(_capi.lib().slq_plan_fun_action_dmat(self._h, fid, ptr(params), out._h, int(o0)))

	def basis(self, probe: int = 0) -> np.ndarray:
		if getattr(self, "basis_kind", None) == "recompute":
			raise ValueError("a recompute plan holds no basis: create the plan with basis='keep'")
		Q = np.zeros((self.op.shape[0], self.deg), dtype=self.op.dtype, order="F")
		check(_capi.lib().slq_plan_get_basis(self._h, int(probe), ptr(Q), Q.shape[0]))
		return Q

	def profile_enable(self, enable: bool = True):
		check(_capi.lib().slq_plan_profile_enable(self._h, int(enable)))

	def profile_read(self, reset: bool = True) -> dict:
		pr = _capi.SlqProfile()
		check(_capi.lib().slq_plan_profile_read(self._h, C.byref(pr), int(reset)))
		return {k: {"ms": pr.ms[i], "launches": pr.launches[i]} for i, k in enumerate(_capi.KERNEL_CLASSES)}

	def sweep_columns(self, reset: bool = True) -> tuple:
		a, b = C.c_uint64(), C.c_uint64()
		check(_capi.lib().slq_plan_sweep_columns(self._h, C.byref(a), C.byref(b), int(reset)))
		return int(a.value), int(b.value)

	def window_columns(self, reset: bool = False) -> dict:
		out = (C.c_int64 * 5)()
		check(_capi.lib().slq_plan_window_columns(self._h, out, int(reset)))
		return dict(zip(("offered", "read", "rescues", "violations", "transitions"), (int(v) for v in out)))

	def window_verify(self) -> dict:
		out = (C.c_double * 5)()
		check(_capi.lib().slq_plan_window_verify(self._h, None, out))
		return dict(zip(("innovation", "margin", "c", "kappa", "norm_inf"), (float(v) for v in out)))

	def window_flags(self) -> tuple:
		panels = self.describe()["panels"]
		rd = np.zeros((self.deg + 1, panels), dtype=np.int32)
		rs = np.zeros((self.deg + 1, panels), dtype=np.int32)
		i32 = C.POINTER(C.c_int32)
		check(_capi.lib().slq_plan_window_flags(self._h, rd.ctypes.data_as(i32), rs.ctypes.data_as(i32), rd.size))
		return rd, rs

	def window_census(self) -> np.ndarray:
		panels = self.describe()["panels"]
		out = np.zeros((self.deg + 1, 9, panels), dtype=np.int32)
		check(_capi.lib().slq_plan_window_census(self._h, out.ctypes.data_as(C.POINTER(C.c_int32)), out.size))
		return out

# ... 842 lines not shown
```

Measured before the change: 164,900.

## Defer the last Lanczos step's update pass until beta_deg is requested

Splits each Lanczos step into front (alpha/dots) and tail (update + beta finalize) parts. When a run reaches the last step and the tail stores nothing useful, only the front is launched. The tail is recorded as pending and flushed when tridiag, the Radau quadrature or the omega diagnostics need beta_deg, or dropped when probes change. The finalize kernels now also write the step count when they close a run. This removes one full update sweep per run whenever the caller never asks for the last beta, at the cost of extra state tracking and the risk of stale or missing flushes.

```diff
diff --git a/include/slq.h b/include/slq.h
--- a/include/slq.h
+++ b/include/slq.h
@@ -126,6 +126,7 @@
 int slq_plan_run_steps(slq_plan *plan, double rtol, int upto);
 int slq_plan_steps_done(const slq_plan *plan, int *cur);
 int slq_plan_get_tridiag(slq_plan *plan, void *alpha, void *beta, int32_t *steps);
+int slq_plan_closing_state(slq_plan *plan, int *lazy, int *pending);
 int slq_plan_quadrature(slq_plan *plan, int fun_id, const double *fun_params, double *quad,
                         double *nodes, double *weights);
 int slq_plan_quadrature_at(slq_plan *plan, int m, int rule, double endpoint, int fun_id, const double *fun_params,
@@ -273,6 +274,7 @@
 int slq_debug_plan_poke_ring_flag(slq_plan *plan, int value);
 int slq_debug_plan_mark_stale(slq_plan *plan, int nstale);
 int slq_debug_step_shape(const int *facts, int nfacts, int j, int prev_xt, int *out, int nout);
+int slq_debug_lazy_tail(const int *facts, int nfacts, int lazy_close, int values_fixed, int *out);
 int slq_debug_cheb_step_shape(const int *facts, int nfacts, int j, int *out, int nout);
 int slq_debug_cheb_action_schedule(int nsteps, int *t0, int *nc, int cap, int *npieces, int *ring_slots, int *acc_cols);
 int slq_debug_csr_layout(int64_t n, int64_t nnz, const int32_t *rowptr, const int32_t *colind, int plain, int32_t *perm_out,
diff --git a/primate_amd/_capi.py b/primate_amd/_capi.py
--- a/primate_amd/_capi.py
+++ b/primate_amd/_capi.py
@@ -180,6 +180,8 @@
 	"slq_debug_plan_poke_ring_flag": (C.c_int, [_P, C.c_int]),
 	"slq_debug_step_shape": (C.c_int, [C.POINTER(C.c_int), C.c_int, C.c_int, C.c_int, C.POINTER(C.c_int), C.c_int]),
 	"slq_debug_cheb_step_shape": (C.c_int, [C.POINTER(C.c_int), C.c_int, C.c_int, C.POINTER(C.c_int), C.c_int]),
+	"slq_debug_lazy_tail": (C.c_int, [C.POINTER(C.c_int), C.c_int, C.c_int, C.c_int, C.POINTER(C.c_int)]),
+	"slq_plan_closing_state": (C.c_int, [_P, C.POINTER(C.c_int), C.POINTER(C.c_int)]),
 	"slq_debug_csr_layout": (C.c_int, [C.c_int64, C.c_int64, _P, _P, C.c_int, _P, _P, C.c_int64, _P, _P]),
 	"slq_debug_plan_shape": (C.c_int, [C.POINTER(C.c_double), C.c_int, C.POINTER(C.c_double), C.c_int]),
 	"slq_debug_plan_shape_of": (C.c_int, [_P, C.POINTER(C.c_double), C.c_int, C.POINTER(C.c_double), C.c_int]),
diff --git a/primate_amd/csrc/slq.hip b/primate_amd/csrc/slq.hip
--- a/primate_amd/csrc/slq.hip
+++ b/primate_amd/csrc/slq.hip
@@ -148,6 +148,12 @@
   int cur = 0;
   double run_rtol = 0.0;
   bool prev_xt = false;
+  struct ClosingTail {
+    bool pending = false;
+    int j = 0;
+    double rtol = 0.0;
+    seq::StepShape shape;
+  } closing;
   double *at_d = nullptr;
   int *at_flags = nullptr;
   PlanSwitches sw;
@@ -205,6 +211,9 @@
   return SLQ_OK;
 }
 
+static int flush_closing_tail(slq_plan *p);
+static void drop_closing_tail(slq_plan *p) { p->closing.pending = false; }
+
 static_assert(OperatorSwitches{}.tiles == 2 && OperatorSwitches{}.tile_rows == kTileRows && OperatorSwitches{}.tile_cols == kTileCols, "slq_switches.hpp: tile defaults");
 static_assert(seq::kMaxFusedR == kFusedMaxR && seq::kMaxRingR == kRingMaxR, "slq_sequence.hpp: the constants of slq_common.hpp");
 static_assert(PlanSwitches{}.debug_pass == PASS_ADOTS, "slq_switches.hpp: SLQ_DEBUG_PASS");
@@ -1443,6 +1452,7 @@
 extern "C" int slq_plan_destroy(slq_plan *p) {
   if (!p) return SLQ_OK;
   hipSetDevice(p->ctx->device);
+  drop_closing_tail(p);
   hipStreamSynchronize(p->ctx->stream);
   for (auto &ev : p->events) { hipEventDestroy(ev.a); hipEventDestroy(ev.b); }
   for (auto &ev : p->pool) { hipEventDestroy(ev.a); hipEventDestroy(ev.b); }
@@ -1722,6 +1732,7 @@
   for (int k = 0; k < 5; ++k) out[k] = 0;
   if (!p->omega_on) return SLQ_OK;
   HIP_TRY(hipSetDevice(p->ctx->device));
+  SLQ_TRY(flush_closing_tail(p));
   unsigned long long h[8] = {0, 0, 0, 0, 0, 0, 0, 0};
   HIP_TRY(hipMemcpyAsync(h, p->om_cnt, sizeof(h), hipMemcpyDeviceToHost, p->ctx->stream));
   if (reset) HIP_TRY(hipMemsetAsync(p->om_cnt, 0, sizeof(h), p->ctx->stream));
@@ -1738,6 +1749,7 @@
   memset(rescue, 0, (size_t)words * sizeof(int32_t));
   if (!p->omega_on) return SLQ_OK;
   HIP_TRY(hipSetDevice(p->ctx->device));
+  SLQ_TRY(flush_closing_tail(p));
   HIP_TRY(hipMemcpyAsync(read, p->om_flags, (size_t)words * sizeof(int), hipMemcpyDeviceToHost, p->ctx->stream));
   HIP_TRY(hipMemcpyAsync(rescue, p->om_flags + words, (size_t)words * sizeof(int), hipMemcpyDeviceToHost, p->ctx->stream));
   HIP_TRY(hipStreamSynchronize(p->ctx->stream));
@@ -1750,6 +1762,7 @@
   if (!p->om_census) return fail(SLQ_EINVAL, "the plan keeps no census (ring-fed Gram sequence created under SLQ_OMEGA=2)");
   if (len != words) return fail(SLQ_EINVAL, "census buffer: %lld words expected", (long long)words);
   HIP_TRY(hipSetDevice(p->ctx->device));
+  SLQ_TRY(flush_closing_tail(p));
   HIP_TRY(hipMemcpyAsync(out, p->om_census, (size_t)words * sizeof(int), hipMemcpyDeviceToHost, p->ctx->stream));
   HIP_TRY(hipStreamSynchronize(p->ctx->stream));
   return SLQ_OK;
@@ -1762,6 +1775,7 @@
   out[0] = 0.0, out[1] = std::numeric_limits<double>::infinity(), out[2] = kOmegaC, out[3] = kOmegaKappa, out[4] = p->om_norm;
   if (!p->omega_on) return SLQ_OK;
   HIP_TRY(hipSetDevice(p->ctx->device));
+  SLQ_TRY(flush_closing_tail(p));
   unsigned long long h[8];
   HIP_TRY(hipMemcpyAsync(h, p->om_cnt, sizeof(h), hipMemcpyDeviceToHost, p->ctx->stream));
   HIP_TRY(hipStreamSynchronize(p->ctx->stream));
@@ -1832,6 +1846,7 @@
   p->probes_ready = true;
   p->ran = false;
   p->cur = 0;
+  p->closing.pending = false;
   return SLQ_OK;
 }
 
@@ -1864,6 +1879,7 @@
   const bool use_pin = pinned && ensure_pinned(ctx, (size_t)cc * col_bytes);
   if (!use_pin) cc = stage_chunk_cols(p);
   SLQ_TRY(ensure_stage(p, cc));
+  drop_closing_tail(p);
   if (p->nprobes < p->bpad)
     HIP_TRY(hipMemsetAsync(slot_ptr(p, 0), 0, (size_t)p->slot_stride * p->esz, st));
   int buf = 0;
@@ -1902,6 +1918,7 @@
   if (!p) return fail(SLQ_EINVAL, "plan is NULL");
   if (pdf < 0 || pdf > 2) return fail(SLQ_EINVAL, "Invalid distribution id %d supplied.", pdf);
   HIP_TRY(hipSetDevice(p->ctx->device));
+  drop_closing_tail(p);
   hipStream_t st = p->ctx->stream;
   const int RPW = 64 / p->LPR;
   const int items = (p->n + (pdf == 0 ? 127 : 1)) / (pdf == 0 ? 128 : 2);
@@ -2366,11 +2383,11 @@
 #undef CSR_PASS
 #undef CSR_PASS_RC
 
-static int launch_gram_ring(const RunFrame &c, const seq::StepShape &s, int j) {
+static int launch_gram_ring(const RunFrame &c, const seq::StepShape &s, int j, int part) {
   slq_plan *p = c.p;
   hipStream_t st = c.st;
   const int bp = p->bpad, r = s.r, S = p->S;
-  PROFILED(p, SLQ_K_SPMM, SLQ_TRY(launch_fused_pass<PASS_ALPHA>(c, s, j, 0, c.lds_alpha(s), s.xt_alpha)));
+  if (part & seq::STEP_FRONT) PROFILED(p, SLQ_K_SPMM, SLQ_TRY(launch_fused_pass<PASS_ALPHA>(c, s, j, 0, c.lds_alpha(s), s.xt_alpha)));
   OmegaState om = c.om_off;
   om.census = p->om_census, om.PW = p->PW, om.NP = p->NP;
   if (s.omega) {
@@ -2384,53 +2401,64 @@
     om.theta = kOmegaC * om.eps_norm;
     om.tol_k = c.orth_tol / kOmegaKappa;
   }
-  PROFILED(p, SLQ_K_FINALIZE,
-           hipLaunchKernelGGL(k_fin_gram, dim3((bp + 63) / 64, r), dim3(kFinThreads), 0, st, p->st, p->part, c.blocks(s.blk_alpha), j, r, c.orth_tol, om));
-  if (om.mode == 1 && om.est_prev) {
+  if (part & seq::STEP_FRONT)
+    PROFILED(p, SLQ_K_FINALIZE,
+             hipLaunchKernelGGL(k_fin_gram, dim3((bp + 63) / 64, r), dim3(kFinThreads), 0, st, p->st, p->part, c.blocks(s.blk_alpha), j, r, c.orth_tol, om, (int)(part == seq::STEP_FRONT)));
+  if ((part & seq::STEP_FRONT) && om.mode == 1 && om.est_prev) {
     double *part_r = p->part + (size_t)p->part_maxblk * bp;
     PROFILED(p, SLQ_K_FINALIZE,
              DISPATCH(p->dtype, p->LPR, (k_omega_rescue_dot<F, L><<<c.gS, dim3(kBlock), 0, st>>>(p->n, (const F *)p->ring, p->slot_stride, S, j, r, part_r, p->om_ticket, p->st, c.orth_tol, om))));
   }
+  if (!(part & seq::STEP_TAIL)) return SLQ_OK;
   PROFILED(p, SLQ_K_REORTH_UPD, SLQ_TRY(launch_ring_gen(p, PASS_UPDATEG, r, c.gT, st, j, s.xt_update, false, om.mode == 1 ? om.read + (size_t)j * p->NP : nullptr)));
   PROFILED(p, SLQ_K_FINALIZE,
            hipLaunchKernelGGL(k_fin_beta_gram, dim3((bp + 63) / 64, r + 1), dim3(kFinThreads), 0, st, p->st, p->part, c.blocks(s.blk_beta), j, r, c.residual_tol, om));
   return SLQ_OK;
 }
 
-static int launch_gram_csr(const RunFrame &c, const seq::StepShape &s, int j) {
+static int launch_gram_csr(const RunFrame &c, const seq::StepShape &s, int j, int part) {
   slq_plan *p = c.p;
   hipStream_t st = c.st;
   const int bp = p->bpad, r = s.r;
-  PROFILED(p, SLQ_K_SPMM, SLQ_TRY(launch_fused_pass<PASS_ALPHA>(c, s, j, 0, c.lds_alpha(s), s.xt_alpha)));
-  PROFILED(p, SLQ_K_FINALIZE,
-           hipLaunchKernelGGL(k_fin_gram, dim3((bp + 63) / 64, r), dim3(kFinThreads), 0, st, p->st, p->part, c.blocks(s.blk_alpha), j, r, c.orth_tol, c.om_off));
+  if (part & seq::STEP_FRONT) {
+    PROFILED(p, SLQ_K_SPMM, SLQ_TRY(launch_fused_pass<PASS_ALPHA>(c, s, j, 0, c.lds_alpha(s), s.xt_alpha)));
+    PROFILED(p, SLQ_K_FINALIZE,
+             hipLaunchKernelGGL(k_fin_gram, dim3((bp + 63) / 64, r), dim3(kFinThreads), 0, st, p->st, p->part, c.blocks(s.blk_alpha), j, r, c.orth_tol, c.om_off, (int)(part == seq::STEP_FRONT)));
+  }
+  if (!(part & seq::STEP_TAIL)) return SLQ_OK;
   PROFILED(p, SLQ_K_REORTH_UPD, DISPATCH(p->dtype, p->LPR, (launch_csr_updateg<F, L>(p, r, s.pipe_on != 0, c.gU, c.lds_fused(s), st, j, s.xt_update))));
   PROFILED(p, SLQ_K_FINALIZE,
            hipLaunchKernelGGL(k_fin_beta_gram, dim3((bp + 63) / 64, r + 1), dim3(kFinThreads), 0, st, p->st, p->part, c.blocks(s.blk_beta), j, r, c.residual_tol, c.om_off));
   return SLQ_OK;
 }
 
-static int launch_merged(const RunFrame &c, const seq::StepShape &s, int j) {
+static int launch_merged(const RunFrame &c, const seq::StepShape &s, int j, int part) {
   slq_plan *p = c.p;
   const int bp = p->bpad, r = s.r;
-  PROFILED(p, SLQ_K_REORTH_DOT, SLQ_TRY(launch_fused_pass<PASS_ADOTS>(c, s, j, r, c.lds_fused(s), s.xt_dots)));
-  PROFILED(p, SLQ_K_FINALIZE,
-           hipLaunchKernelGGL(k_fin_adots, dim3((bp + 63) / 64, r), dim3(kFinThreads), 0, c.st, p->st, p->part, c.blocks(s.blk_dots), j, r, c.orth_tol));
+  if (part & seq::STEP_FRONT) {
+    PROFILED(p, SLQ_K_REORTH_DOT, SLQ_TRY(launch_fused_pass<PASS_ADOTS>(c, s, j, r, c.lds_fused(s), s.xt_dots)));
+    PROFILED(p, SLQ_K_FINALIZE,
+             hipLaunchKernelGGL(k_fin_adots, dim3((bp + 63) / 64, r), dim3(kFinThreads), 0, c.st, p->st, p->part, c.blocks(s.blk_dots), j, r, c.orth_tol, (int)(part == seq::STEP_FRONT)));
+  }
+  if (!(part & seq::STEP_TAIL)) return SLQ_OK;
   PROFILED(p, SLQ_K_REORTH_UPD, SLQ_TRY(launch_fused_pass<PASS_UPDATE>(c, s, j, r, c.lds_fused(s), s.xt_update)));
   return SLQ_OK;
 }
 
-static int launch_separate(const RunFrame &c, const seq::StepShape &s, int j) {
+static int launch_separate(const RunFrame &c, const seq::StepShape &s, int j, int part) {
   slq_plan *p = c.p;
   const int bp = p->bpad, r = s.r;
-  PROFILED(p, SLQ_K_SPMM, SLQ_TRY(launch_fused_pass<PASS_ALPHA>(c, s, j, 0, c.lds_alpha(s), s.xt_alpha)));
-  PROFILED(p, SLQ_K_FINALIZE,
-           hipLaunchKernelGGL(k_fin_alpha, c.gF, dim3(kFinThreads), 0, c.st, p->st, p->part, c.blocks(s.blk_alpha), j, s.xt_alpha & 1));
-  if (r > 0) {
+  if (part & seq::STEP_FRONT) {
+    PROFILED(p, SLQ_K_SPMM, SLQ_TRY(launch_fused_pass<PASS_ALPHA>(c, s, j, 0, c.lds_alpha(s), s.xt_alpha)));
+    PROFILED(p, SLQ_K_FINALIZE,
+             hipLaunchKernelGGL(k_fin_alpha, c.gF, dim3(kFinThreads), 0, c.st, p->st, p->part, c.blocks(s.blk_alpha), j, s.xt_alpha & 1, (int)(part == seq::STEP_FRONT)));
+  }
+  if ((part & seq::STEP_FRONT) && r > 0) {
     PROFILED(p, SLQ_K_REORTH_DOT, SLQ_TRY(launch_fused_pass<PASS_DOTS>(c, s, j, r, c.lds_fused(s), s.xt_dots)));
     PROFILED(p, SLQ_K_FINALIZE,
              hipLaunchKernelGGL(k_fin_gamma, dim3((bp + 63) / 64, r), dim3(kFinThreads), 0, c.st, p->st, p->part, c.blocks(s.blk_dots), j, 0, c.orth_tol));
   }
+  if (!(part & seq::STEP_TAIL)) return SLQ_OK;
   PROFILED(p, (r == 0 ? SLQ_K_AXPY_NORM : SLQ_K_REORTH_UPD), SLQ_TRY(launch_fused_pass<PASS_UPDATE>(c, s, j, r, c.lds_fused(s), s.xt_update)));
   return SLQ_OK;
 }
@@ -2489,7 +2517,7 @@
       break;
   }
   if (cheb) return SLQ_OK;
-  PROFILED(p, SLQ_K_FINALIZE, hipLaunchKernelGGL(k_fin_alpha, c.gF, dim3(kFinThreads), 0, st, p->st, p->part, nblk, j, 0));
+  PROFILED(p, SLQ_K_FINALIZE, hipLaunchKernelGGL(k_fin_alpha, c.gF, dim3(kFinThreads), 0, st, p->st, p->part, nblk, j, 0, 0));
   return SLQ_OK;
 }
 
@@ -2537,7 +2565,28 @@
   return c;
 }
 
-static int enqueue_run(slq_plan *p, double rtol, int j0, int j1) {
+static int launch_step(const RunFrame &c, const seq::StepShape &s, int j, int part) {
+  slq_plan *p = c.p;
+  switch (s.seq) {
+    case seq::SEQ_GRAM_RING: return launch_gram_ring(c, s, j, part);
+    case seq::SEQ_GRAM_CSR: return launch_gram_csr(c, s, j, part);
+    case seq::SEQ_MERGED:
+    case seq::SEQ_STORED_U: SLQ_TRY(launch_merged(c, s, j, part)); break;
+    case seq::SEQ_SEPARATE: SLQ_TRY(launch_separate(c, s, j, part)); break;
+    default:
+      if (part != seq::STEP_WHOLE) return fail(SLQ_EINVAL, "internal: a step of the store-and-revisit sweeps has no closing tail");
+      SLQ_TRY(launch_sweeps(c, s, j));
+      break;
+  }
+  if (part & seq::STEP_TAIL)
+    PROFILED(p, SLQ_K_FINALIZE,
+             hipLaunchKernelGGL(k_fin_beta, c.gF, dim3(kFinThreads), 0, c.st, p->st, p->part, c.blocks(s.blk_beta), j, c.residual_tol, s.prev_xt ? 1 : 0));
+  return SLQ_OK;
+}
+
+static bool plan_lazy_tail(const slq_plan *p) { return !p->cheb && seq::has_lazy_tail(sequence_facts(p), p->sw.last_store != 2, !p->facts.affine); }
+
+static int enqueue_run(slq_plan *p, double rtol, int j0, int j1, bool lazy_tail = false) {
   hipStream_t st = p->ctx->stream;
   const int bp = p->bpad, deg = p->deg;
   const RunFrame c = run_frame(p, rtol);
@@ -2556,16 +2605,7 @@
   for (int j = j0; j < j1; ++j) {
     const seq::StepShape s = seq::step_shape(facts, j, prev_xt);
     prev_xt = s.prev_xt != 0;
-    switch (s.seq) {
-      case seq::SEQ_GRAM_RING: SLQ_TRY(launch_gram_ring(c, s, j)); continue;
-      case seq::SEQ_GRAM_CSR: SLQ_TRY(launch_gram_csr(c, s, j)); continue;
-      case seq::SEQ_MERGED:
-      case seq::SEQ_STORED_U: SLQ_TRY(launch_merged(c, s, j)); break;
-      case seq::SEQ_SEPARATE: SLQ_TRY(launch_separate(c, s, j)); break;
-      default: SLQ_TRY(launch_sweeps(c, s, j)); break;
-    }
-    PROFILED(p, SLQ_K_FINALIZE,
-             hipLaunchKernelGGL(k_fin_beta, c.gF, dim3(kFinThreads), 0, st, p->st, p->part, c.blocks(s.blk_beta), j, c.residual_tol, prev_xt ? 1 : 0));
+    SLQ_TRY(launch_step(c, s, j, (lazy_tail && j == deg - 1) ? seq::STEP_FRONT : seq::STEP_WHOLE));
   }
   p->prev_xt = prev_xt;
   HIP_TRY(hipGetLastError());
@@ -2802,8 +2842,9 @@
   HIP_TRY(hipSetDevice(p->ctx->device));
   hipStream_t st = p->ctx->stream;
   const bool graph_ok = p->sw.graph && !p->prof && p->op->kind != OP_CALLBACK && p->op->kind != OP_DEVICE_CALLBACK;
+  const bool lazy_tail = j1 == p->deg && plan_lazy_tail(p);
   if (!graph_ok) {
-    SLQ_TRY(enqueue_run(p, rtol, j0, j1));
+    SLQ_TRY(enqueue_run(p, rtol, j0, j1, lazy_tail));
   } else {
     const unsigned variant = (unsigned)p->nstale;
     size_t gi = 0;
@@ -2827,7 +2868,7 @@
       hipGraph_t graph = nullptr;
       const bool xt_in = p->prev_xt;
       HIP_TRY(hipStreamBeginCapture(st, hipStreamCaptureModeThreadLocal));
-      const int rc = enqueue_run(p, rtol, j0, j1);
+      const int rc = enqueue_run(p, rtol, j0, j1, lazy_tail);
       hipError_t ce = hipStreamEndCapture(st, &graph);
       if (rc != SLQ_OK) {
         if (graph) hipGraphDestroy(graph);
@@ -2853,6 +2894,40 @@
   p->cur = j1;
   p->run_rtol = rtol;
   p->rule_src = 0;
+  if (lazy_tail) {
+    p->closing.pending = true;
+    p->closing.j = p->deg - 1;
+    p->closing.rtol = rtol;
+    p->closing.shape = seq::step_shape(sequence_facts(p), p->deg - 1, false);
+  }
+  return SLQ_OK;
+}
+
+static int flush_closing_tail(slq_plan *p) {
+  if (!p->closing.pending) return SLQ_OK;
+  HIP_TRY(hipSetDevice(p->ctx->device));
+  const RunFrame c = run_frame(p, p->closing.rtol);
+  const int rc = launch_step(c, p->closing.shape, p->closing.j, seq::STEP_TAIL);
+  if (rc != SLQ_OK) return rc;
+  HIP_TRY(hipGetLastError());
+  if (p->launch_error) {
+    p->launch_error = false;
+    return fail(SLQ_EINVAL, "internal: a pass of the launch sequence had no kernel for this plan's tiles");
+  }
+  p->closing.pending = false;
+  return SLQ_OK;
+}
+
+extern "C" int slq_plan_closing_state(slq_plan *p, int *lazy, int *pending) {
+  if (!p) return fail(SLQ_EINVAL, "plan is NULL");
+  if (lazy) *lazy = plan_lazy_tail(p) ? 1 : 0;
+  if (pending) *pending = p->closing.pending ? 1 : 0;
+  return SLQ_OK;
+}
+
+extern "C" int slq_debug_lazy_tail(const int *facts, int nfacts, int lazy_close, int values_fixed, int *out) {
+  if (!facts || !out || nfacts != seq::kNumFacts) return fail(SLQ_EINVAL, "slq_debug_lazy_tail: %d facts in, one value out", seq::kNumFacts);
+  *out = seq::has_lazy_tail(seq::facts_from_array(facts), lazy_close, values_fixed) ? 1 : 0;
   return SLQ_OK;
 }
 
@@ -2868,6 +2943,7 @@
   SLQ_TRY(need_lanczos(p, "slq_plan_get_tridiag"));
   if (!p->ran) return fail(SLQ_EINVAL, "slq_plan_get_tridiag: no completed run");
   HIP_TRY(hipSetDevice(p->ctx->device));
+  SLQ_TRY(flush_closing_tail(p));
   hipStream_t st = p->ctx->stream;
   const int bp = p->bpad, deg = p->deg, P = p->nprobes;
   std::vector<double> ha((size_t)(deg + 1) * bp), hn((size_t)(deg + 1) * bp);
@@ -2965,6 +3041,7 @@
     HIP_TRY(hipFuncSetAttribute((const void *)k_quadrature_at, hipFuncAttributeMaxDynamicSharedMemorySize, 160 * 1024));
   HIP_TRY(hipMemsetAsync(p->at_flags, 0, 2 * sizeof(int), st));
   const double residual_tol = std::sqrt((double)p->n) * p->run_rtol;
+  if (rule == 1 && m == deg) SLQ_TRY(flush_closing_tail(p));
   PROFILED(p, SLQ_K_QUADRATURE,
            hipLaunchKernelGGL(k_quadrature_at, dim3((P + lanes - 1) / lanes), dim3(64), lds, st, p->st, m, rule, endpoint, residual_tol, lanes,
                               fun_id, p0, p1, quad_d, gauss_d, nodes_d, weights_d, p->at_flags));
@@ -4712,6 +4789,7 @@
   HIP_TRY(hipSetDevice(p->ctx->device));
   hipStream_t st = p->ctx->stream;
   if (ldx != p->n) return fail(SLQ_EINVAL, "device probes must be contiguous columns (ldx == n)");
+  drop_closing_tail(p);
   if (p->nprobes < p->bpad) HIP_TRY(hipMemsetAsync(slot_ptr(p, 0), 0, (size_t)p->slot_stride * p->esz, st));
   dim3 g((p->n + 63) / 64, (p->nprobes + 63) / 64);
   PROFILED(p, SLQ_K_PROBES, {
diff --git a/primate_amd/csrc/slq_kernels.hpp b/primate_amd/csrc/slq_kernels.hpp
--- a/primate_amd/csrc/slq_kernels.hpp
+++ b/primate_amd/csrc/slq_kernels.hpp
@@ -1615,7 +1615,7 @@
 }
 
 __global__ __launch_bounds__(kFinThreads) void k_fin_alpha(StepState st, const double *__restrict__ partA,
-                                                   int nblk, int j, int xt) {
+                                                   int nblk, int j, int xt, int closing) {
   __shared__ double red4[kFinThreads];
   const int col = blockIdx.x * 64 + (threadIdx.x & 63);
   double a = sum_partials(partA, nblk, st.bpad, col, red4);
@@ -1624,6 +1624,7 @@
     if (xt) a -= st.coefA[col] * st.coefA[st.bpad + col] * st.cross[col];
     if (act) st.alpha[(int64_t)j * st.bpad + col] = a;
     st.coefB[col] = act ? a / st.nu[(int64_t)j * st.bpad + col] : 0.0;
+    if (closing && act) st.steps[col] = j + 1;
   }
 }
 
@@ -1655,7 +1656,7 @@
 }
 
 __global__ __launch_bounds__(kFinThreads) void k_fin_adots(StepState st, const double *__restrict__ part, int nblk,
-                                                   int j, int RC, double orth_tol) {
+                                                   int j, int RC, double orth_tol, int closing) {
   __shared__ double red4[kFinThreads];
   const int i = blockIdx.y;
   const int col = blockIdx.x * 64 + (threadIdx.x & 63);
@@ -1674,6 +1675,7 @@
       if (act) st.alpha[(int64_t)j * st.bpad + col] = a;
       st.coefB[col] = cb;
       st.gamma[col] = 0.0;
+      if (closing && act) st.steps[col] = j + 1;
     } else {
       const double nu = st.nu[(int64_t)(j - i) * st.bpad + col];
       double gm = 0.0;
@@ -1774,7 +1776,7 @@
   return gm;
 }
 
-__global__ __launch_bounds__(kFinThreads) void k_fin_gram(StepState st, const double *__restrict__ part, int nblk, int j, int RC, double orth_tol, OmegaState om) {
+__global__ __launch_bounds__(kFinThreads) void k_fin_gram(StepState st, const double *__restrict__ part, int nblk, int j, int RC, double orth_tol, OmegaState om, int closing) {
   __shared__ double red4[kFinThreads];
   const int i = blockIdx.y;
   const int col = blockIdx.x * 64 + (threadIdx.x & 63);
@@ -1792,6 +1794,7 @@
       if (act) st.alpha[(int64_t)j * bp + col] = a;
       st.coefB[col] = cb;
       st.gamma[col] = 0.0;
+      if (closing && act) st.steps[col] = j + 1;
     } else if (om.mode != 0 && i == RC - 1) {
       const double gm = omega_edge(st, om, j, i, col, cb, orth_tol, false);
       st.gamma[(int64_t)i * bp + col] = gm;
diff --git a/primate_amd/csrc/slq_plan_shape.hpp b/primate_amd/csrc/slq_plan_shape.hpp
--- a/primate_amd/csrc/slq_plan_shape.hpp
+++ b/primate_amd/csrc/slq_plan_shape.hpp
@@ -311,7 +311,7 @@
     q.dense_class = s.dense_class, q.pipelined = s.pipelined;
     q.fused = sw.fused, q.merged = sw.merged, q.mgs = sw.mgs, q.stored_u = sw.stored_u, q.nt = sw.nt, q.cross = sw.cross, q.sw_gram = sw.gram;
     q.sw_gram_csr = sw.gram_csr, q.sw_ring_gen = sw.ring_gen, q.sw_ring_deep = sw.ring_deep;
-    q.last_store = (sw.last_store || action) ? 1 : 0;
+    q.last_store = (sw.last_store == 1 || action) ? 1 : 0;
     q.ring_alpha = sw.ring_alpha, q.ring_rev = sw.ring_rev;
     seq::derive_plan_flags(q);
     s.omega_on = q.gram && sw.omega != 0 && orth == 3 && s.S >= 4 && !f.affine && s.PW >= 32;
diff --git a/primate_amd/csrc/slq_sequence.hpp b/primate_amd/csrc/slq_sequence.hpp
--- a/primate_amd/csrc/slq_sequence.hpp
+++ b/primate_amd/csrc/slq_sequence.hpp
@@ -151,6 +151,12 @@
   }
 }
 
+enum StepPart { STEP_FRONT = 1, STEP_TAIL = 2, STEP_WHOLE = 3 };
+inline bool has_lazy_tail(const SequenceFacts &f, int lazy_close, int values_fixed) {
+  if (!lazy_close || !values_fixed || f.deg < 1 || f.basis_mode != 0) return false;
+  return (step_shape(f, f.deg - 1, false).xt_update & 16) != 0;
+}
+
 struct ChebStepShape {
   int sweeps = 1;
   int tiled = 0;
diff --git a/primate_amd/csrc/slq_switches.hpp b/primate_amd/csrc/slq_switches.hpp
--- a/primate_amd/csrc/slq_switches.hpp
+++ b/primate_amd/csrc/slq_switches.hpp
@@ -36,7 +36,7 @@
   PLAN(ring_alpha, "SLQ_RING_ALPHA", 2, "alpha-only pass of a tiled symmetric operator: 2 ring over the upper-triangle stream, 1 over full rows, 0 generic") \
   PLAN(ring_alpha_max_x100, "SLQ_RING_ALPHA_MAX_X100", 260, "... takes the upper-triangle stream up to this many (x100) landed rows per row")        \
   PLAN(ring_rev, "SLQ_RING_REV", 1, "the ring-fed update pass sweeps panels and tiles in reverse")                                                   \
-  PLAN(last_store, "SLQ_LAST_STORE", 0, "1: the update pass of a run's last step stores W_deg although it is never read")                            \
+  PLAN(last_store, "SLQ_LAST_STORE", 0, "the update pass of a run's last step: 0 stores nothing and is launched when beta_deg is first asked for, 1 stores W_deg although it is never read, 2 stores nothing, launched with the run") \
   PLAN(sweep_skip, "SLQ_SWEEP_SKIP", 1, "the update sweep skips ring columns whose coefficient is zero for the whole panel")                         \
   PLAN(acc_skip, "SLQ_ACC_SKIP", 1, "the accumulation of a recompute plan's replay skips such columns")                                              \
   PLAN(defer_axpy, "SLQ_DEFER_AXPY", 1, "block-CGS sweeps: the dots sweeps are read-only, the update sweep applies the three-term axpy")             \
diff --git a/primate_amd/engine.py b/primate_amd/engine.py
--- a/primate_amd/engine.py
+++ b/primate_amd/engine.py
@@ -452,6 +452,11 @@
 			quad = np.array([np.sum(fun(nodes[i]) * weights[i]) for i in range(self.nprobes)]) * vn2
 		out = (quad,) + ((nodes, weights) if return_rule else ()) + ((stage,) if return_stage else ())
 		return out[0] if len(out) == 1 else out
+
+	def closing(self) -> dict:
+		lazy, pending = C.c_int(), C.c_int()
+		check(_capi.lib().slq_plan_closing_state(self._h, C.byref(lazy), C.byref(pending)))
+		return {"lazy": bool(lazy.value), "pending": bool(pending.value)}
 
 	def tridiag(self) -> tuple:
 		a = np.zeros((self.nprobes, self.deg + 1), dtype=self.op.dtype)
```

New measurement: 167,900, median of 6. +1.8%, better.
